# cvYouTian/Dedark-YOLO

Measured on AMD Instinct MI355X. Metric: training img/s at 640x640, higher is better.
Workload: dtype bf16

## Files before the change

dedark_yolo_amd/_C.py:

```python
import ctypes as C
import os

_HERE = os.path.dirname(os.path.abspath(__file__))
LIB_PATH = os.path.join(os.environ.get("DY_LIB_DIR") or os.path.join(_HERE, "lib"), "libdedark_yolo.so")

DY_F32, DY_BF16, DY_F16 = 0, 1, 2
ACT_NONE, ACT_SILU, ACT_LEAKY = 0, 1, 2
OPT_RULES = dict(Adam=0, Adamax=1, NAdam=2, RAdam=3, RMSProp=4)
STATS_REPLICAS = 64
BN_BWD_REPLICAS = 8

vp, i32, i64, f32, f64 = C.c_void_p, C.c_int, C.c_int64, C.c_float, C.c_double


class ConvDesc(C.Structure):
    _fields_ = [("src", vp), ("src_ld", i64), ("N", i32), ("Hs", i32), ("Ws", i32), ("Cs", i32), ("w", vp), ("dst", vp),
                ("dst_ld", i64), ("Hd", i32), ("Wd", i32), ("Cd", i32), ("KH", i32), ("KW", i32), ("stride", i32),
                ("pad", i32), ("dil", i32), ("scale", vp), ("shift", vp), ("act", i32), ("stats", vp), ("accumulate", i32),
                ("dtype", i32), ("dst_row_stride", i64), ("dst_img_stride", i64), ("KHf", i32), ("KWf", i32), ("kh0", i32),
                ("kh_step", i32), ("kw0", i32), ("kw_step", i32), ("dst_valid_channels", i32), ("dst_planar", vp),
                ("add_src", vp), ("add_src_ld", i64)]


class PackItem(C.Structure):
    _fields_ = [("w", vp), ("packed", vp), ("Cout", i32), ("Cout_pad", i32), ("Cin", i32), ("Cin_pad", i32), ("KH", i32),
                ("KW", i32), ("transposed", i32), ("dtype", i32), ("first_block", i64)]


class DetMaps(C.Structure):
    _fields_ = [("map", vp * 3), ("map_ld", i64 * 3), ("h", i32 * 3), ("w", i32 * 3), ("stride", f32 * 3), ("B", i32),
                ("nc", i32), ("n_levels", i32), ("dtype", i32)]


class DetMaps4(DetMaps):
    _fields_ = [("map3", vp), ("map_ld3", i64), ("h3", i32), ("w3", i32), ("stride3", f32)]


class AugSample(C.Structure):
    _fields_ = [("src", vp * 4), ("sh", i32 * 4), ("sw", i32 * 4), ("pitch", i64 * 4), ("rect", (i32 * 6) * 4), ("n_src", i32),
                ("canvas_h", i32), ("canvas_w", i32), ("hsv", i32), ("flipud", i32), ("fliplr", i32), ("minv", C.c_double * 6),
                ("lut", (C.c_uint8 * 256) * 3)]


class AugMixSample(C.Structure):
    _fields_ = [("a", AugSample), ("b", AugSample), ("r", C.c_double), ("r1", C.c_double), ("mix", i32)]


class SegDesc(C.Structure):
    _fields_ = [("mc", vp), ("mc_ld", i64), ("proto", vp), ("proto_ld", i64), ("B", i32), ("A", i32), ("nm", i32), ("mh", i32),
                ("mw", i32), ("target_gt_idx", vp), ("fg_mask", vp), ("target_box", vp), ("masks", vp), ("mask_dtype", i32),
                ("mask_h", i32), ("mask_w", i32), ("overlap", i32), ("gt_rows", vp), ("n_max", i32), ("img_h", f32), ("img_w", f32),
                ("pos", vp), ("npos", vp), ("dtype", i32)]


BIAS_GRAD_CHUNKS = 2048

POSE_MAX_LEVELS = 4


class PoseDesc(C.Structure):
    _fields_ = [("kpt", vp * POSE_MAX_LEVELS), ("kpt_ld", i64 * POSE_MAX_LEVELS), ("h", i32 * POSE_MAX_LEVELS), ("w", i32 * POSE_MAX_LEVELS),
                ("stride", f32 * POSE_MAX_LEVELS), ("n_levels", i32), ("B", i32), ("A", i32), ("K", i32), ("ndim", i32), ("dtype", i32),
                ("target_gt_idx", vp), ("fg_mask", vp), ("target_box", vp), ("keypoints", vp), ("n_targets", i32), ("gt_rows", vp),
                ("n_max", i32), ("img_h", f32), ("img_w", f32), ("sigma", vp), ("pos", vp), ("npos", vp)]


_SIGS = {
    "dy_version": [],
    "dy_frontend_init": [],
    "dy_conv2d_fwd": [C.POINTER(ConvDesc), vp],
    "dy_conv2d_dgrad": [C.POINTER(ConvDesc), vp],
    "dy_conv2d_wgrad": [vp, i64, i32, i32, i32, i32, vp, i64, i32, i32, i32, i32, i32, i32, i32, i32, i32, i32, vp, i64, vp,
                        i32, vp],
    "dy_conv2d_wgrad_forked": [vp, vp, i64, i32, i32, i32, i32, vp, i64, i32, i32, i32, i32, i32, i32, i32, i32, i32, i32, vp, i64,
                               vp, i32, vp],
    "dy_conv2d_bn_act_fwd": [C.POINTER(ConvDesc), i64, vp, vp, vp, vp, f32, f32, vp, i32, vp, i64, vp, i64, vp],
    "dy_bn_act_bwd": [vp, i64, vp, i64, vp, vp, i32, vp, vp, i64, vp, vp, i64, i32, i32, vp],
    "dy_conv2d_bn_act_fwd_valid": [C.POINTER(ConvDesc), i64, vp, vp, vp, vp, f32, f32, vp, i32, vp, i64, vp, i64, i32, vp],
    "dy_bn_act_bwd_valid": [vp, i64, vp, i64, vp, vp, i32, vp, vp, i64, vp, vp, i64, i32, i32, i32, vp],
    "dy_pack_weight": [vp, vp, i32, i32, i32, i32, i32, i32, i32, i32, vp],
    "dy_pack_item_blocks": [i32, i32, i32, i32],
    "dy_pack_weights_multi": [vp, i32, i64, vp],
    "dy_unpack_wgrad": [vp, vp, i32, i32, i32, i32, i32, vp],
    "dy_bn_finalize": [vp, i64, vp, vp, vp, vp, f32, f32, vp, vp, vp, vp, i32, vp],
    "dy_bn_fold_eval": [vp, vp, vp, vp, f32, vp, vp, i32, vp],
    "dy_bn_finalize_valid": [vp, i64, vp, vp, vp, vp, f32, f32, vp, vp, vp, vp, i32, i32, vp],
    "dy_bn_fold_eval_valid": [vp, vp, vp, vp, f32, vp, vp, i32, i32, vp],
    "dy_bn_act_fwd": [vp, i64, vp, vp, i32, vp, i64, vp, i64, i64, i32, i32, vp],
    "dy_bn_act_bwd_reduce": [vp, i64, vp, i64, vp, vp, vp, vp, i32, i32, vp, i64, i32, i32, vp],
    "dy_bn_act_bwd_apply": [vp, i64, vp, i64, vp, vp, vp, vp, vp, i32, i32, vp, vp, i64, vp, vp, i64, i32, i32, vp],
    "dy_bn_act_bwd_apply_valid": [vp, i64, vp, i64, vp, vp, vp, vp, vp, i32, i32, vp, vp, i64, vp, vp, i64, i32, i32, i32, vp],
    "dy_maxpool_fwd": [vp, i64, vp, i64, vp, i32, i32, i32, i32, i32, i32, i32, i32, i32, i32, vp],
    "dy_maxpool_bwd": [vp, i64, vp, vp, i64, i32, i32, i32, i32, i32, i32, i32, i32, i32, i32, i32, vp],
    "dy_upsample_nearest_fwd": [vp, i64, vp, i64, i32, i32, i32, i32, i32, i32, vp],
    "dy_upsample_nearest_bwd": [vp, i64, vp, i64, i32, i32, i32, i32, i32, i32, i32, vp],
    "dy_copy2d": [vp, i64, vp, i64, i64, i32, i32, i32, vp],
    "dy_cast": [vp, i32, vp, i32, i64, vp],
    "dy_pconv_pack": [vp, vp, i32, i32, i32, vp],
    "dy_pconv_fwd": [vp, i64, vp, i64, vp, vp, i32, i32, i32, i32, i32, i32, vp],
    "dy_pconv_dgrad": [vp, i64, vp, i64, vp, vp, i32, i32, i32, i32, i32, i32, vp, i64, i32, vp],
    "dy_pconv_wgrad": [vp, i64, vp, i64, vp, i32, i32, i32, i32, vp, i64, i32, vp],
    "dy_asff_fuse_fwd": [vp, i64, vp, i64, vp, i64, vp, i64, vp, i64, i64, i32, i32, vp],
    "dy_asff_fuse_bwd": [vp, i64, vp, i64, vp, i64, vp, i64, vp, i64, vp, i64, vp, i64, vp, i64, vp, i64, i64, i32, i32, i32,
                         i32, i32, vp],
    "dy_image_to_nhwc8": [vp, i32, i32, i32, vp, i32, i32, i32, vp],
    "dy_resize_bwd": [vp, i32, i32, i32, i32, i32, i32, vp, vp],
    "dy_filter_params_fwd": [vp, i32, vp, i32, vp],
    "dy_filter_params_bwd": [vp, i32, vp, vp, i32, vp],
    "dy_filters_pointwise_fwd": [vp, vp, vp, vp, vp, i32, i32, i32, i32, vp],
    "dy_filters_pointwise_bwd": [vp, vp, vp, vp, vp, vp, vp, i32, i32, i32, i32, i32, vp],
    "dy_usm_fwd": [vp, vp, vp, vp, vp, i32, i32, i32, i32, vp],
    "dy_usm_bwd": [vp, vp, i32, vp, vp, vp, vp, i32, i32, i32, i32, vp],
    "dy_loss_prepare_targets": [vp, vp, vp, i32, i32, i32, f32, f32, vp, vp, vp],
    "dy_loss_decode": [C.POINTER(DetMaps), vp, vp],
    "dy_tal_assign": [C.POINTER(DetMaps), vp, vp, vp, i32, vp, vp, vp, vp, vp, vp, vp, vp, vp],
    "dy_tal_assign_decoded": [vp, vp, vp, vp, vp, i32, i32, i32, i32, vp, vp, vp, vp, vp, vp, vp, vp, vp],
    "dy_chan_moments": [vp, i64, i32, i64, i32, vp, i32, vp],
    "dy_sru_fwd": [vp, i64, vp, i64, i32, i64, i32, i32, vp, vp, vp, f32, i32, vp],
    "dy_sru_bwd": [vp, i64, vp, i64, vp, i64, i32, i64, i32, i32, vp, vp, vp, f32, vp, i32, vp],
    "dy_cru_fuse_fwd": [vp, i64, vp, i64, i32, i64, i32, vp, i32, vp],
    "dy_cru_fuse_bwd": [vp, i64, vp, i64, vp, i64, i32, i64, i32, vp, vp, i32, vp],
    "dy_bbox_ciou": [vp, vp, i64, vp, vp, vp],
    "dy_bbox_iou": [vp, vp, i64, i32, i32, f32, vp, vp, vp],
    "dy_aug_resize_u8": [vp, i32, i32, i64, vp, i32, i32, i64, vp],
    "dy_aug_letterbox": [vp, i32, i32, i64, i32, i32, i32, i32, i32, i32, vp, vp],
    "dy_aug_mosaic_warp": [vp, i32, i32, i32, vp, vp],
    "dy_aug_mosaic_warp_mix": [vp, i32, i32, i32, vp, vp],
    "dy_dark_channel_prior": [vp, i32, i32, i32, vp, vp, vp],
    "dy_dfl_loss": [vp, vp, i64, vp, vp, vp],
    "dy_loss_fwd": [C.POINTER(DetMaps), vp, vp, vp, vp, vp, vp, vp],
    "dy_loss_finish": [vp, vp, f32, f32, f32, f32, i32, vp, vp, vp],
    "dy_loss_bwd": [C.POINTER(DetMaps), C.POINTER(vp), C.POINTER(i64), vp, vp, vp, vp, vp, vp, vp, f32, f32, f32, vp],
    "dy_detect_decode": [C.POINTER(DetMaps), vp, vp],
    "dy_detect_decode_rows": [C.POINTER(DetMaps), vp, i32, vp],
    "dy_detect_decode_tta": [C.POINTER(DetMaps), vp, i64, i32, i32, i32, f32, i32, f32, f32, vp],
    "dy_tta_scale_img": [vp, i32, i32, i32, i32, i32, i32, i32, i32, i32, vp, vp],
    "dy_nms_candidates": [vp, i32, i32, i32, f32, i32, vp, vp, i64, vp],
    "dy_nms_sort": [vp, vp, vp, i32, i64, vp, vp, vp],
    "dy_nms_greedy": [vp, vp, vp, i32, i32, i32, i64, C.c_double, i32, i32, f32, i32, vp, vp, vp, vp, vp, vp],
    "dy_preprocess_batch": [vp, vp, vp, f32, i32, i32, vp, i64, vp],
    "dy_sumsq": [vp, i64, vp, vp],
    "dy_sgd_step": [vp, vp, vp, vp, vp, f32, f32, f32, f32, f32, f32, f32, i32, f32, vp, f32, f32, i64, vp],
    "dy_sgd_step_scaled": [vp, vp, vp, vp, vp, f32, f32, f32, f32, f32, f32, f32, i32, f32, vp, f32, f32, vp, i64, vp],
    "dy_adamw_step_scaled": [vp, vp, vp, vp, vp, vp, f32, f32, f32, f32, f32, f32, f32, f32, f32, i32, f32, vp, f32, f32, vp, i64, vp],
    "dy_loss_scale_update": [vp, vp, f32, f32, i32, vp],
    "dy_optim_step": [i32, vp, vp, vp, vp, vp, vp, f32, f32, f32, f32, f32, f32, f64, f64, f64, f64, f32, vp, f32, f32, vp, vp, i64, vp],
    "dy_adamw_step": [vp, vp, vp, vp, vp, vp, f32, f32, f32, f32, f32, f32, f32, f32, f32, i32, f32, vp, f32, f32, i64, vp],
    "dy_ema_lerp": [vp, vp, f32, i64, vp],
    "dy_grad_accumulate": [vp, vp, i64, vp],
    "dy_stream_fork": [vp, vp],
    "dy_seg_positives": [vp, i32, i32, vp, vp, vp],
    "dy_seg_gt_rows": [vp, i32, i32, i32, vp, vp],
    "dy_seg_loss_fwd": [C.POINTER(SegDesc), f32, vp, vp, vp, vp],
    "dy_seg_loss_bwd": [C.POINTER(SegDesc), vp, f32, vp, i64, vp, i64, vp],
# ... 80 lines not shown
```

dedark_yolo_amd/csrc/bnact.hip:

```cpp
#include <stdlib.h>
#include <type_traits>
#include "dy_host.h"
#include "../../include/dedark_yolo.h"

#ifndef DY_BN_NT_FWD_MB
#define DY_BN_NT_FWD_MB 128
#endif

namespace {

constexpr int NT = 256;
template <typename T, bool NTS> __device__ inline void ld_s(const T* p, float* out) {
  if constexpr (NTS) ldvec_nt<T>(p, out); else ldvec<T>(p, out);
}
template <typename T, bool NTS> __device__ inline void st_s(T* p, const float* in) {
  if constexpr (NTS) stvec_nt<T>(p, in); else stvec<T>(p, in);
}

__global__ __launch_bounds__(256) void bn_finalize_kernel(const double* __restrict__ stats, double count, const float* __restrict__ gamma,
                                                           const float* __restrict__ beta, float* running_mean, float* running_var,
                                                           float momentum, float eps, float* scale, float* shift, float* mean_out,
                                                           float* invstd_out, int C, int Cv) {
  static_assert(DY_STATS_REPLICAS == 64, "one replica per lane");
  const int lane = threadIdx.x & 63;
  const int c = blockIdx.x * 4 + (threadIdx.x >> 6);
  if (c >= C) return;
  if (c >= Cv) {
    if (lane == 0) scale[c] = shift[c] = mean_out[c] = invstd_out[c] = 0.f;
    return;
  }
  double s1 = stats[(long)lane * 2 * C + c];
  double s2 = stats[(long)lane * 2 * C + C + c];
#pragma unroll
  for (int o = 32; o > 0; o >>= 1) {
    s1 += __shfl_xor(s1, o, 64);
    s2 += __shfl_xor(s2, o, 64);
  }
  if (lane != 0) return;
  double m = s1 / count;
  double var = s2 / count - m * m;
  if (var < 0) var = 0;
  float invstd = (float)(1.0 / sqrt(var + (double)eps));
  float g = gamma ? gamma[c] : 1.f, b = beta ? beta[c] : 0.f;
  float sc = g * invstd;
  scale[c] = sc;
  shift[c] = b - (float)m * sc;
  mean_out[c] = (float)m;
  invstd_out[c] = invstd;
  if (running_mean) {
    double unbiased = count > 1 ? var * count / (count - 1) : var;
    running_mean[c] = (1.f - momentum) * running_mean[c] + momentum * (float)m;
    running_var[c] = (1.f - momentum) * running_var[c] + momentum * (float)unbiased;
  }
}

__global__ void bn_fold_eval_kernel(const float* gamma, const float* beta, const float* rm, const float* rv, float eps,
                                    float* scale, float* shift, int C, int Cv) {
  int c = blockIdx.x * blockDim.x + threadIdx.x;
  if (c >= C) return;
  if (c >= Cv) {
    scale[c] = 0.f;
    shift[c] = 0.f;
    return;
  }
  float sc = gamma[c] / sqrtf(rv[c] + eps);
  scale[c] = sc;
  shift[c] = beta[c] - rm[c] * sc;
}

__device__ inline float fast_sigmoid(float x) { return __builtin_amdgcn_rcpf(1.0f + __expf(-x)); }
template <typename T, int ACT> __device__ inline float act_f(float u) {
  if (sizeof(T) == 4) return dy_act(ACT, u);
  if (ACT == DY_ACT_SILU) return u * fast_sigmoid(u);
  if (ACT == DY_ACT_LEAKY) return u > 0.f ? u : 0.1f * u;
  return u;
}
template <typename T, int ACT> __device__ inline float dact_f(float u) {
  if (sizeof(T) == 4) return dy_dact(ACT, u);
  if (ACT == DY_ACT_SILU) {
    const float s = fast_sigmoid(u);
    return s * (1.0f + u * (1.0f - s));
  }
  if (ACT == DY_ACT_LEAKY) return u > 0.f ? 1.0f : 0.1f;
  return 1.0f;
}
template <typename F> __device__ inline void with_act(int act, F&& f) {
  if (act == DY_ACT_SILU) f(std::integral_constant<int, DY_ACT_SILU>{});
  else if (act == DY_ACT_LEAKY) f(std::integral_constant<int, DY_ACT_LEAKY>{});
  else f(std::integral_constant<int, DY_ACT_NONE>{});
}

struct Map {
  int c, cl;
  long first, step;
  bool active;
};

template <int VE>
__device__ inline Map make_map(int C, int cgb, int rows) {
  Map m;
  const int CG = C / VE;
  const int cg_local = threadIdx.x % cgb, prow = threadIdx.x / cgb;
  const int cg = blockIdx.y * cgb + cg_local;
  m.active = prow < rows && cg < CG;
  m.c = cg * VE;
  m.cl = cg_local * VE;
  m.first = (long)blockIdx.x * rows + prow;
  m.step = (long)gridDim.x * rows;
  return m;
}


template <typename T, int U, bool NTS>
__global__ __launch_bounds__(NT) void bn_act_fwd_kernel(const T* __restrict__ z, long z_ld, const float* __restrict__ scale,
                                                         const float* __restrict__ shift, int act, const T* __restrict__ res,
                                                         long res_ld, T* __restrict__ y, long y_ld, long pixels, int C, int cgb,
                                                         int rows) {
  constexpr int VE = DT<T>::VE;
  extern __shared__ float lds[];
  const int nch = cgb * VE, c0 = blockIdx.y * nch;
  for (int i = threadIdx.x; i < nch; i += NT) {
    const int c = c0 + i;
    lds[i] = (scale && c < C) ? scale[c] : 1.f;
    lds[nch + i] = (shift && c < C) ? shift[c] : 0.f;
  }
  __syncthreads();
  const Map m = make_map<VE>(C, cgb, rows);
  if (!m.active) return;
  float sc[VE], sh[VE];
#pragma unroll
  for (int e = 0; e < VE; ++e) {
    sc[e] = lds[m.cl + e];
    sh[e] = lds[nch + m.cl + e];
  }
  with_act(act, [&](auto actc) {
    constexpr int ACT = decltype(actc)::value;
    auto loop = [&](auto resc) {
      constexpr bool RES = decltype(resc)::value;
      for (long p0 = m.first; p0 < pixels; p0 += U * m.step) {
        float v[U][VE], r[U][VE];
#pragma unroll
        for (int k = 0; k < U; ++k) {
          const long p = p0 + k * m.step;
          if (p < pixels) {
            ld_s<T, NTS>(z + p * z_ld + m.c, v[k]);
            if (RES) ld_s<T, NTS>(res + p * res_ld + m.c, r[k]);
          }
        }
#pragma unroll
        for (int k = 0; k < U; ++k) {
          const long p = p0 + k * m.step;
          if (p < pixels) {
#pragma unroll
            for (int e = 0; e < VE; ++e) {
              const float o = act_f<T, ACT>(v[k][e] * sc[e] + sh[e]);
              v[k][e] = RES ? o + r[k][e] : o;
            }
            st_s<T, NTS>(y + p * y_ld + m.c, v[k]);
          }
        }
      }
    };
    if (res) loop(std::true_type{});
    else loop(std::false_type{});
  });
}

template <typename T, int U, bool NTS>
// ... 312 lines not shown
```

dedark_yolo_amd/csrc/conv.hip:

```cpp
#include <stdlib.h>
#include "dy_host.h"
#include "conv_epilogue.h"
#include "../../include/dedark_yolo.h"
#include "conv_route.h"

namespace {

constexpr int ROWB = 144;
constexpr int NTHREADS = 256;

struct ConvP {
  const char* src;
  long src_ld;
  int N, Hs, Ws, Cs;
  const char* w;
  char* dst;
  long dst_ld;
  int Hd, Wd, Cd;
  int KH, KW, stride, pad, dil;
  const float* scale;
  const float* shift;
  int act;
  double* stats;
  int accumulate;
// ... 730 lines not shown
  const int tiles_m = dy_cdiv(p.M, BM);
  auto blocks = [&](int bn) {
    p.tiles_n = dy_cdiv(d->Cd, bn);
    p.nblk = tiles_m * p.tiles_n;
    if (p.ncls > 1) p.nblk = dy_route::number_parity_blocks(p, BM, dy_route::CLS_SEQUENTIAL);
  };
  dy_note_kernel(d->Cd <= 32 ? "conv_igemm_kernel<BN=32>" : (d->Cd <= 64 ? "conv_igemm_kernel<BN=64>" : "conv_igemm_kernel<BN=128>"));
  if (d->Cd <= 32) {
    blocks(32);
    conv_igemm_kernel<T, BM, 32, 4, 1, MODE><<<p.nblk, NTHREADS, 0, st>>>(p);
  } else if (d->Cd <= 64) {
    blocks(64);
    conv_igemm_kernel<T, BM, 64, 2, 2, MODE><<<p.nblk, NTHREADS, 0, st>>>(p);
  } else {
    blocks(128);
    conv_igemm_kernel<T, BM, 128, 2, 2, MODE><<<p.nblk, NTHREADS, 0, st>>>(p);
  }
  DY_LAUNCH_CHECK();
  return 0;
}

bool thin_eligible(const dy_conv_desc* d, int mode, bool parity_class = false) {
  static const bool off = dy_env("DY_NO_CONV_THIN") != nullptr;
  static const bool all_shapes = getenv("DY_CONV_THIN_ALL") != nullptr;
  if (off || d->dtype != DY_BF16) return false;
  if (!all_shapes && !parity_class && !(d->Cs == 16 && d->KH * d->KW > 1)) return false;
  if (!(d->Cs == 16 || d->Cs == 32 || d->Cs == 48) || d->Cd > 32 || d->Cd % 8 != 0) return false;
  if (d->KH > 3 || d->KW > 3 || d->dil != 1 || (mode == 1 && d->stride != 1)) return false;
  if ((d->src_ld * 2) % 16 != 0 || (d->dst_ld * 2) % 16 != 0 || (long)d->N * d->Hd * d->Wd < 1024) return false;
  return true;
}

int launch_thin(const dy_conv_desc* d, int mode, hipStream_t st, const dy_conv_desc* classes = nullptr, int ncls = 0) {
  ConvP p;
  dy_route::fill_parity_classes(p, classes, ncls);
  dy_route::fill_gather(p, d);
  p.tiles_n = 1;
  p.nblk = dy_cdiv(p.M, THIN_BM);
  if (p.ncls > 1) p.nblk = dy_route::number_parity_blocks(p, THIN_BM, dy_route::CLS_SEQUENTIAL);
  dy_note_kernel("conv_thin_kernel");
#define THIN(C_, M_) conv_thin_kernel<C_, M_><<<p.nblk, NTHREADS, 0, st>>>(p)
  const int c16 = d->Cs / 16;
  if (mode == 0) { if (c16 == 1) THIN(1, 0); else if (c16 == 2) THIN(2, 0); else THIN(3, 0); }
  else { if (c16 == 1) THIN(1, 1); else if (c16 == 2) THIN(2, 1); else THIN(3, 1); }
#undef THIN
  DY_LAUNCH_CHECK();
  return 0;
}

int launch_generic(const dy_conv_desc* d, int mode, hipStream_t st, const dy_conv_desc* classes = nullptr, int ncls = 0) {
  if (mode == 0)
    return d->dtype == DY_F32 ? launch_conv<float, 0>(d, st, classes, ncls)
                              : (d->dtype == DY_F16 ? launch_conv<f16_t, 0>(d, st, classes, ncls) : launch_conv<bf16_t, 0>(d, st, classes, ncls));
  return d->dtype == DY_F32 ? launch_conv<float, 1>(d, st, classes, ncls)
                            : (d->dtype == DY_F16 ? launch_conv<f16_t, 1>(d, st, classes, ncls) : launch_conv<bf16_t, 1>(d, st, classes, ncls));
}

int check_conv(const dy_conv_desc* d, const char* who) {
  DY_CHECK(d && d->src && d->w && (d->dst || d->dst_planar), "%s: null pointer", who);
  DY_CHECK(d->dtype == DY_F32 || d->dtype == DY_BF16 || d->dtype == DY_F16, "%s: bad dtype %d", who, d->dtype);
  const int ve = d->dtype == DY_F32 ? 4 : 8, es = d->dtype == DY_F32 ? 4 : 2;
  DY_CHECK(d->Cs > 0 && d->Cs % ve == 0, "%s: Cs=%d must be a positive multiple of %d", who, d->Cs, ve);
  DY_CHECK(d->src_ld >= d->Cs && (d->src_ld * es) % 16 == 0, "%s: src_ld=%ld not 16-byte aligned", who, (long)d->src_ld);
  DY_CHECK(((uintptr_t)d->src) % 16 == 0 && ((uintptr_t)d->w) % 16 == 0, "%s: src/w pointer not 16-byte aligned", who);
  DY_CHECK(d->dst_ld >= d->Cd && d->Cd > 0, "%s: dst_ld=%ld < Cd=%d", who, (long)d->dst_ld, d->Cd);
  DY_CHECK(d->N > 0 && d->Hs > 0 && d->Ws > 0 && d->Hd > 0 && d->Wd > 0, "%s: empty geometry", who);
  DY_CHECK(d->KH > 0 && d->KW > 0 && d->stride > 0 && d->dil > 0 && d->pad >= 0, "%s: bad window", who);
  DY_CHECK(d->act >= 0 && d->act <= 2, "%s: bad act", who);
  return 0;
}

enum : unsigned {
  SITE_FWD = 1,
  SITE_DGRAD_HEAD = 2,
  SITE_DGRAD = 4,
  SITE_CLASS = 8,
};

struct Route {
  bool (*eligible)(const dy_conv_desc* d, int mode);
  int (*launch)(const dy_conv_desc* d, int mode, void* stream);
  unsigned sites;
  bool fuses_add;
};

const Route kRoutes[] = {
    {dy_dense_fwd_eligible, dy_dense_fwd_launch, SITE_FWD, false},
    {dy_conv_stem_fwd_eligible, dy_conv_stem_fwd_launch, SITE_FWD, false},
    {dy_dense_dgrad_eligible, dy_dense_dgrad_launch, SITE_DGRAD_HEAD, false},
    {dy_conv_small_dgrad_eligible, dy_conv_small_dgrad_launch, SITE_DGRAD_HEAD, false},
    {dy_conv_px_eligible, dy_conv_px_launch, SITE_FWD | SITE_DGRAD, true},
    {dy_conv_v4_eligible, dy_conv_v4_launch, SITE_FWD | SITE_DGRAD | SITE_CLASS, true},
    {dy_conv_v5_eligible, dy_conv_v5_launch, SITE_FWD | SITE_DGRAD | SITE_CLASS, true},
    {dy_conv_v3_eligible, dy_conv_v3_launch, SITE_FWD | SITE_DGRAD, false},
    {dy_conv_v2_eligible, dy_conv_v2_launch, SITE_FWD | SITE_DGRAD | SITE_CLASS, false},
    {[](const dy_conv_desc* d, int mode) { return thin_eligible(d, mode); },
     [](const dy_conv_desc* d, int mode, void* stream) { return launch_thin(d, mode, (hipStream_t)stream); }, SITE_FWD | SITE_DGRAD, false},
    {[](const dy_conv_desc*, int) { return true; },
     [](const dy_conv_desc* d, int mode, void* stream) { return launch_generic(d, mode, (hipStream_t)stream); },
     SITE_FWD | SITE_DGRAD | SITE_CLASS, false},
};

const Route* pick_route(const dy_conv_desc* d, unsigned site) {
  const int mode = (site & (SITE_DGRAD_HEAD | SITE_DGRAD)) ? 1 : 0;
  for (const Route& r : kRoutes)
    if ((r.sites & site) && r.eligible(d, mode)) return &r;
  return nullptr;
}

}

extern "C" int dy_conv2d_fwd(const dy_conv_desc* d, void* stream) {
  if (int e = check_conv(d, "dy_conv2d_fwd")) return e;
  const int ho = (d->Hs + 2 * d->pad - d->dil * (d->KH - 1) - 1) / d->stride + 1;
  const int wo = (d->Ws + 2 * d->pad - d->dil * (d->KW - 1) - 1) / d->stride + 1;
  DY_CHECK(ho == d->Hd && wo == d->Wd, "dy_conv2d_fwd: dst %dx%d does not match conv output %dx%d", d->Hd, d->Wd, ho, wo);
  return pick_route(d, SITE_FWD)->launch(d, 0, stream);
}

static int dgrad_dispatch(const dy_conv_desc* d, void* stream, bool* added) {
  if (int e = check_conv(d, "dy_conv2d_dgrad")) return e;
  const int ho = (d->Hd + 2 * d->pad - d->dil * (d->KH - 1) - 1) / d->stride + 1;
  const int wo = (d->Wd + 2 * d->pad - d->dil * (d->KW - 1) - 1) / d->stride + 1;
  DY_CHECK(ho == d->Hs && wo == d->Ws, "dy_conv2d_dgrad: dz %dx%d does not match conv output %dx%d", d->Hs, d->Ws, ho, wo);
  DY_CHECK(d->stats == nullptr, "dy_conv2d_dgrad: stats unsupported");
  DY_CHECK(d->KHf == 0 && d->dst_row_stride == 0, "dy_conv2d_dgrad: tap subsets / strided destinations are forward-only");
  if (const Route* r = pick_route(d, SITE_DGRAD_HEAD)) return r->launch(d, 1, stream);
  DY_CHECK(d->dst_planar == nullptr, "dy_conv2d_dgrad: dst_planar is only supported by the direct stem kernel (bf16, 3x3 s2 p1, Cd == 8)");
  static const bool no_parity = dy_env("DY_NO_PARITY_DGRAD") != nullptr;
  if (d->stride == 2 && d->dil == 1 && !no_parity) {
    dy_conv_desc c[4];
    int nc = 0;
    bool ok = true;
    for (int ph = 0; ph < 2 && ok; ++ph)
      for (int pw = 0; pw < 2 && ok; ++pw) {
        int geo[2][4];
        for (int ax = 0; ax < 2; ++ax) {
          const int par = ax == 0 ? ph : pw, K = ax == 0 ? d->KH : d->KW, ext = ax == 0 ? d->Hd : d->Wd;
          const int first = (par + d->pad) & 1;
          const int n = first < K ? (K - 1 - first) / 2 + 1 : 0;
          const int last = first + 2 * (n - 1);
          const int omin = (par + d->pad - last) / 2;
          geo[ax][0] = n; geo[ax][1] = last; geo[ax][2] = -omin; geo[ax][3] = (ext - par + 1) / 2;
        }
        if (geo[0][3] <= 0 || geo[1][3] <= 0) continue;
        if (geo[0][0] == 0 || geo[1][0] == 0 || geo[0][2] != geo[1][2] || geo[0][2] < 0) { ok = false; break; }
        dy_conv_desc& q = c[nc++];
        q = *d;
        const long es = d->dtype == DY_F32 ? 4 : 2;
        q.dst = (char*)d->dst + ((long)ph * d->Wd + pw) * d->dst_ld * es;
        q.dst_ld = 2 * d->dst_ld;
        q.dst_row_stride = 2L * d->Wd * d->dst_ld;
        q.dst_img_stride = (long)d->Hd * d->Wd * d->dst_ld;
        q.Hd = geo[0][3]; q.Wd = geo[1][3];
        q.KHf = d->KH; q.KWf = d->KW;
        q.KH = geo[0][0]; q.KW = geo[1][0];
        q.kh0 = geo[0][1]; q.kh_step = -2; q.kw0 = geo[1][1]; q.kw_step = -2;
        q.stride = 1; q.pad = geo[0][2];
      }
    if (ok) {
      static const bool multi = !(dy_env("DY_PARITY_MULTI") && atoi(dy_env("DY_PARITY_MULTI")) == 0);
      if (multi && nc > 1) {
        dy_conv_desc r[4];
        bool all_v2 = true, none_v2 = true;
        for (int i = 0; i < nc; ++i) {
          r[i] = c[nc - 1 - i];
          const bool e2 = dy_conv_v2_eligible(&r[i], 0);
          all_v2 = all_v2 && e2;
          none_v2 = none_v2 && !e2;
        }
        const long class_tiles = dy_cdiv((long)r[0].N * r[0].Hd * r[0].Wd, 256);
        if (dy_conv_v4_classes_eligible(r, nc)) return dy_conv_v4_launch_classes(r, nc, stream);
        if (dy_conv_v5_classes_eligible(r, nc)) return dy_conv_v5_launch_classes(r, nc, stream);
        if (all_v2 && class_tiles <= 256) return dy_conv_v2_launch_classes(r, nc, stream);
        if (none_v2) {
          bool thin = true;
          for (int i = 0; i < nc; ++i) thin = thin && thin_eligible(&r[i], 0, true);
          if (thin) return launch_thin(&r[0], 0, (hipStream_t)stream, r, nc);
          if (class_tiles <= 256) return launch_generic(&r[0], 0, (hipStream_t)stream, r, nc);
        }
      }
      for (int i = nc - 1; i >= 0; --i) {
        if (int e = pick_route(&c[i], SITE_CLASS)->launch(&c[i], 0, stream)) return e;
      }
      return 0;
    }
  }
  const Route* r = pick_route(d, SITE_DGRAD);
  *added = r->fuses_add;
  return r->launch(d, 1, stream);
}

extern "C" int dy_conv2d_dgrad(const dy_conv_desc* d, void* stream) {
  bool added = false;
  if (int e = dgrad_dispatch(d, stream, &added)) return e;
  if (d->add_src && !added) {
    DY_CHECK(d->dst && d->dst_planar == nullptr, "dy_conv2d_dgrad: add_src needs an NHWC destination");
    return dy_copy2d(d->add_src, d->add_src_ld, d->dst, d->dst_ld, (int64_t)d->N * d->Hd * d->Wd, d->Cd, 1, d->dtype, stream);
  }
  return 0;
}

namespace {
template <typename T>
int launch_wgrad(WgP p, float* scratch, long scratch_elems, float* g_oihw, int Cout_real, int Cin_real, hipStream_t st) {
  constexpr int MK = 8 * DT<T>::VE;
  int bm, bn;
  bn = p.Ktot <= 32 ? 32 : (p.Ktot <= 64 ? 64 : 128);
  if (bn == 32) bm = 128;
  else if (bn == 64) bm = p.Cout <= 64 ? 64 : 128;
  else bm = p.Cout <= 32 ? 32 : (p.Cout <= 64 ? 64 : 128);
  const int tiles_c = dy_cdiv(p.Cout, bm);
  p.tiles_k = dy_cdiv(p.Ktot, bn);
  const int tiles = tiles_c * p.tiles_k;
  p.tiles = tiles;
  static const int env_blocks = dy_env("DY_WGRAD_BLOCKS") ? atoi(dy_env("DY_WGRAD_BLOCKS")) : 0;
  static const int env_steps = dy_env("DY_WGRAD_STEPS") ? atoi(dy_env("DY_WGRAD_STEPS")) : 0;
  const int min_steps = env_steps > 0 ? env_steps : 4;
  long max_splits = (p.M + (long)min_steps * MK - 1) / ((long)min_steps * MK);
  long want = ((env_blocks > 0 ? env_blocks : 2048) + tiles - 1) / tiles;
  long splits = want < max_splits ? want : max_splits;
  const long fit = scratch_elems / ((long)tiles * bm * bn);
  DY_CHECK(fit >= 1, "dy_conv2d_wgrad: scratch too small (%ld floats, need %ld)", scratch_elems, (long)tiles * bm * bn);
  if (splits > fit) splits = fit;
  if (splits < 1) splits = 1;
  if (splits > 65535) splits = 65535;
  long chunk = (p.M + splits - 1) / splits;
  chunk = (chunk + MK - 1) / MK * MK;
  splits = (p.M + chunk - 1) / chunk;
  p.chunk = chunk;
  p.part = scratch;
  dim3 grid(tiles, (unsigned)splits);
  dy_note_kernel("conv_wgrad_kernel+wgrad_reduce_kernel");
#define WG(BM_, BN_, WM_, WN_) conv_wgrad_kernel<T, BM_, BN_, WM_, WN_><<<grid, NTHREADS, 0, st>>>(p)
  if (bm == 128 && bn == 128) WG(128, 128, 2, 2);
  else if (bm == 64 && bn == 128) WG(64, 128, 1, 4);
  else if (bm == 32 && bn == 128) WG(32, 128, 1, 4);
  else if (bm == 128 && bn == 64) WG(128, 64, 4, 1);
  else if (bm == 64 && bn == 64) WG(64, 64, 2, 2);
  else WG(128, 32, 4, 1);
#undef WG
  DY_LAUNCH_CHECK();
  wgrad_reduce_kernel<<<dim3(Cout_real, dy_cdiv(p.Ktot, 32)), 256, 0, st>>>(scratch, (int)splits, tiles, p.tiles_k, bm, bn,
                                                                            Cin_real, p.Cin, p.KH, p.KW, p.Ktot, g_oihw);
  DY_LAUNCH_CHECK();
  return 0;
}

int wgrad_generic(const DyWgradArgs& a, void* stream) {
  WgP p;
  p.x = (const char*)a.x; p.x_ld = a.x_ld; p.N = a.N; p.Hi = a.Hi; p.Wi = a.Wi; p.Cin = a.Cin_pad;
  p.dz = (const char*)a.dz; p.dz_ld = a.dz_ld; p.Ho = a.Ho; p.Wo = a.Wo; p.Cout = a.Cout_pad;
  p.KH = a.KH; p.KW = a.KW; p.stride = a.stride; p.pad = a.pad; p.dil = a.dil; p.part = a.scratch;
  p.M = (long)a.N * a.Ho * a.Wo;
  p.Ktot = a.KH * a.KW * a.Cin_pad;
  p.pointwise = (a.KH == 1 && a.KW == 1 && a.stride == 1 && a.pad == 0) ? 1 : 0;
  hipStream_t st = (hipStream_t)stream;
  return a.dtype == DY_F32 ? launch_wgrad<float>(p, a.scratch, a.scratch_elems, a.g_oihw, a.Cout, a.Cin, st)
                           : (a.dtype == DY_F16 ? launch_wgrad<f16_t>(p, a.scratch, a.scratch_elems, a.g_oihw, a.Cout, a.Cin, st)
                                                : launch_wgrad<bf16_t>(p, a.scratch, a.scratch_elems, a.g_oihw, a.Cout, a.Cin, st));
}
}

extern "C" int dy_conv2d_wgrad(const void* x, int64_t x_ld, int N, int Hi, int Wi, int Cin_pad, const void* dz, int64_t dz_ld,
                               int Ho, int Wo, int Cout_pad, int KH, int KW, int stride, int pad, int dil, int Cout, int Cin,
                               float* scratch, int64_t scratch_elems, float* g_oihw, int dtype, void* stream) {
  DY_CHECK(x && dz && scratch && g_oihw, "dy_conv2d_wgrad: null pointer");
  DY_CHECK(dtype == DY_F32 || dtype == DY_BF16 || dtype == DY_F16, "dy_conv2d_wgrad: bad dtype");
  const int ve = dtype == DY_F32 ? 4 : 8, es = dtype == DY_F32 ? 4 : 2;
  DY_CHECK(Cin_pad % ve == 0 && Cout_pad % ve == 0, "dy_conv2d_wgrad: Cin=%d / Cout=%d must be multiples of %d", Cin_pad, Cout_pad, ve);
  DY_CHECK(Cout > 0 && Cout <= Cout_pad && Cin > 0 && Cin <= Cin_pad, "dy_conv2d_wgrad: bad real channel counts");
  DY_CHECK((x_ld * es) % 16 == 0 && (dz_ld * es) % 16 == 0, "dy_conv2d_wgrad: ld not 16-byte aligned");
  DY_CHECK(((uintptr_t)x) % 16 == 0 && ((uintptr_t)dz) % 16 == 0, "dy_conv2d_wgrad: pointer not 16-byte aligned");
  const int ho = (Hi + 2 * pad - dil * (KH - 1) - 1) / stride + 1, wo = (Wi + 2 * pad - dil * (KW - 1) - 1) / stride + 1;
  DY_CHECK(ho == Ho && wo == Wo, "dy_conv2d_wgrad: dz %dx%d does not match conv output %dx%d", Ho, Wo, ho, wo);
  const DyWgradArgs a = {x, x_ld, N, Hi, Wi, Cin_pad, dz, dz_ld, Ho, Wo, Cout_pad, KH, KW, stride, pad, dil, Cout, Cin,
                         scratch, scratch_elems, g_oihw, dtype};
  if (dy_dense_wgrad_eligible(a)) return dy_dense_wgrad_launch(a, stream);
  if (dy_wgrad_v3_eligible(a)) return dy_wgrad_v3_launch(a, stream);
  if (dy_wgrad_v4_eligible(a)) return dy_wgrad_v4_launch(a, stream);
  if (dy_wgrad_v2_eligible(a)) return dy_wgrad_v2_launch(a, stream);
  return wgrad_generic(a, stream);
}
// ... 67 lines not shown
```

dedark_yolo_amd/csrc/conv_epilogue.h:

```cpp
#pragma once
#include "dy_common.h"

namespace dy_epi {

template <int BM>
constexpr int pitch() { return BM * 2 + 8; }

typedef __attribute__((ext_vector_type(4))) short s16x4;
typedef __attribute__((address_space(3))) s16x4* lds_s16x4_ptr;

template <int BM, int BN>
constexpr int image_bytes() { return BN * pitch<BM>(); }

template <typename T16 = bf16_t>
__device__ inline uint32_t pack2(float a, float b) {
  if constexpr (__is_same(T16, bf16_t)) return pack_bf16x2(a, b);
  else return (uint32_t)cvt16<T16>(a) | ((uint32_t)cvt16<T16>(b) << 16);
}

template <int BM, int BN, int NW, typename T16, typename OffFn>
__device__ inline void store_image(const char* smem, int lane, int wave, long m0, int n0, long M, int Cd, int accumulate, T16* dst,
                                   OffFn off) {
  constexpr int PT = pitch<BM>();
  constexpr int UP = BM / 16, UC = BN / 32;
  const int g = lane >> 4, li = lane & 15, tq = li >> 2, tp = li & 3;
  static_assert(UP % NW == 0, "pixel tiles per wave");
#pragma unroll 2
  for (int u = 0; u < (UP / NW) * UC; ++u) {
    const int pt = wave + NW * (u / UC), ct = u % UC;
    const int cb = ct * 32 + 8 * g;
    const char* base = smem + (cb + tq) * PT + (pt * 16 + 4 * tp) * 2;
    const s16x4 lo = __builtin_amdgcn_ds_read_tr16_b64_v4i16((lds_s16x4_ptr)(base));
    const s16x4 hi = __builtin_amdgcn_ds_read_tr16_b64_v4i16((lds_s16x4_ptr)(base + 4 * PT));
    const long m = m0 + pt * 16 + li;
    const int n = n0 + cb;
    if (m < M && n < Cd) {
      u32x4 v;
      v[0] = (uint32_t)(uint16_t)lo[0] | ((uint32_t)(uint16_t)lo[1] << 16);
      v[1] = (uint32_t)(uint16_t)lo[2] | ((uint32_t)(uint16_t)lo[3] << 16);
      v[2] = (uint32_t)(uint16_t)hi[0] | ((uint32_t)(uint16_t)hi[1] << 16);
      v[3] = (uint32_t)(uint16_t)hi[2] | ((uint32_t)(uint16_t)hi[3] << 16);
      T16* o = dst + off(m) + n;
      if (n + 8 <= Cd) {
        if (accumulate) {
          float x[8], y[8];
          ldvec<T16>(o, x);
          ldvec<T16>(reinterpret_cast<const T16*>(&v), y);
#pragma unroll
          for (int e = 0; e < 8; ++e) x[e] += y[e];
          stvec<T16>(o, x);
        } else {
          *reinterpret_cast<u32x4*>(o) = v;
        }
      } else {
        const T16* e = reinterpret_cast<const T16*>(&v);
        for (int q = 0; q < 8 && n + q < Cd; ++q) {
          if (accumulate) DT<T16>::st(o + q, DT<T16>::ld(o + q) + DT<T16>::ld(e + q));
          else o[q] = e[q];
        }
      }
    }
  }
}

template <int BN>
constexpr int row_pitch() { return BN * 2 + 8; }

template <int BM, int BN>
constexpr int row_image_bytes() { return BM * row_pitch<BN>(); }

template <int BM, int BN, int NW, typename T16, typename OffFn, int RG = 64>
__device__ inline void store_rows(const char* smem, int lane, int wave, long m0, int n0, long M, int Cd, int accumulate, T16* dst, OffFn off,
                                  const T16* __restrict__ add = nullptr, long add_ld = 0) {
  constexpr int PT = row_pitch<BN>();
  constexpr int LPP = BN >= 128 ? 16 : BN / 8;
  constexpr int PPI = 64 / LPP;
  constexpr int ITERS = BM / PPI / NW;
  constexpr int HALVES = BN >= 128 ? BN / 128 : 1;
  const int pl = lane / LPP, chunk = lane % LPP;
  const bool nt = accumulate & 2;
  accumulate &= 1;
#pragma unroll 2
  for (int u = 0; u < ITERS; ++u) {
    const int px = PPI * (wave + NW * u) + pl;
    if (RG < 64 && (px & 63) >= RG) continue;
    const long m = RG < 64 ? m0 + (px >> 6) * RG + (px & 63) : m0 + px;
#pragma unroll
    for (int h = 0; h < HALVES; ++h) {
      const int c = 128 * h + 8 * chunk;
      const uint2 lo = *reinterpret_cast<const uint2*>(smem + px * PT + c * 2);
      const uint2 hi = *reinterpret_cast<const uint2*>(smem + px * PT + c * 2 + 8);
      const int n = n0 + c;
      if (m < M && n < Cd) {
        u32x4 v = {lo.x, lo.y, hi.x, hi.y};
        T16* o = dst + off(m) + n;
        if (n + 8 <= Cd) {
          if (accumulate || add) {
            float x[8], y[8];
            ldvec<T16>(reinterpret_cast<const T16*>(&v), y);
            if (accumulate) {
              ldvec<T16>(o, x);
#pragma unroll
              for (int e = 0; e < 8; ++e) y[e] += x[e];
            }
            if (add) {
              ldvec<T16>(add + m * add_ld + n, x);
#pragma unroll
              for (int e = 0; e < 8; ++e) y[e] += x[e];
            }
            if (nt) {
              u32x4 w;
              stvec<T16>(reinterpret_cast<T16*>(&w), y);
              asm volatile("global_store_dwordx4 %0, %1, off nt" ::"v"(o), "v"(w) : "memory");
            } else {
              stvec<T16>(o, y);
            }
          } else if (nt) {
            asm volatile("global_store_dwordx4 %0, %1, off nt" ::"v"(o), "v"(v) : "memory");
          } else {
            *reinterpret_cast<u32x4*>(o) = v;
          }
        } else {
          const T16* e = reinterpret_cast<const T16*>(&v);
          for (int q = 0; q < 8 && n + q < Cd; ++q) {
            float t = DT<T16>::ld(e + q);
            if (accumulate) t += DT<T16>::ld(o + q);
            if (add) t += DT<T16>::ld(add + m * add_ld + n + q);
            DT<T16>::st(o + q, t);
          }
        }
      }
    }
  }
}

template <int BM, int BN, int WM, int WN, int TM, int TN, typename T16, typename OffFn>
__device__ inline void store_tile(char* smem, f32x16 (&acc)[TM][TN], int wm, int wn, int lane, int wave, long m0, int n0, long M, int Cd,
                                  const float* scale, const float* shift, int act, int accumulate, T16* dst, OffFn off,
                                  float (&csum)[TN], float (&csq)[TN]) {
  constexpr int PT = pitch<BM>();
  static_assert(BM / WM == 32 * TM && BN / WN == 32 * TN, "wave tiling");
  const int cl = lane & 31, hh = lane >> 5;
#pragma unroll
  for (int j = 0; j < TN; ++j) { csum[j] = 0.f; csq[j] = 0.f; }
  __builtin_amdgcn_s_barrier();
#pragma unroll
  for (int j = 0; j < TN; ++j) {
    const int col = wn * (BN / WN) + j * 32 + cl;
    const int n = n0 + col;
    const bool nok = n < Cd;
    const float sc = (nok && scale) ? scale[n] : 1.f;
    const float sf = (nok && shift) ? shift[n] : 0.f;
#pragma unroll
    for (int i = 0; i < TM; ++i) {
      const int row0 = wm * (BM / WM) + i * 32 + 4 * hh;
      const long mrem = M - (m0 + row0);
#pragma unroll
      for (int rq = 0; rq < 4; ++rq) {
        float v[4];
#pragma unroll
        for (int e = 0; e < 4; ++e) {
          const float a = acc[i][j][4 * rq + e];
          if (nok && 8 * rq + e < mrem) {
            csum[j] += a;
// ... 18 lines not shown
```

dedark_yolo_amd/csrc/conv_route.h:

```cpp
#pragma once
#include "dy_common.h"
#include "../../include/dedark_yolo.h"

namespace dy_route {

__device__ inline int xcd_remap(int bid, int nblk) {
  int q = nblk >> 3, r = nblk & 7, x = bid & 7;
  int base = (x < r) ? x * (q + 1) : r * (q + 1) + (x - r) * q;
  return base + (bid >> 3);
}

template <typename P>
__device__ inline long dst_offset(const P& p, long m) {
  if (p.dst_row == 0) return m * p.dst_ld;
  const long HWd = (long)p.Hd * p.Wd;
  const long img = m / HWd;
  const int rem = (int)(m - img * HWd);
  const int oh = rem / p.Wd, ow = rem - oh * p.Wd;
  return img * p.dst_img + (long)oh * p.dst_row + (long)ow * p.dst_ld;
}

template <typename P>
inline void fill_weight_taps(P& p, const dy_conv_desc* d) {
  if (d->KHf > 0) {
    p.kh0 = d->kh0; p.khs = d->kh_step; p.kw0 = d->kw0; p.kws = d->kw_step; p.KWf = d->KWf;
    p.w_row = (long)d->KHf * d->KWf * d->Cs;
  } else {
    p.kh0 = 0; p.khs = 1; p.kw0 = 0; p.kws = 1; p.KWf = d->KW;
    p.w_row = (long)d->KH * d->KW * d->Cs;
  }
}

template <typename P>
inline void fill_dst_strides(P& p, const dy_conv_desc* d) {
  p.dst_row = d->dst_row_stride;
  p.dst_img = d->dst_img_stride ? d->dst_img_stride : (long)d->Hd * d->dst_row_stride;
}

template <typename P>
inline void fill_gather(P& p, const dy_conv_desc* d) {
  p.src = (const char*)d->src; p.src_ld = d->src_ld; p.N = d->N; p.Hs = d->Hs; p.Ws = d->Ws; p.Cs = d->Cs;
  p.w = (const char*)d->w; p.dst = (char*)d->dst; p.dst_ld = d->dst_ld; p.Hd = d->Hd; p.Wd = d->Wd; p.Cd = d->Cd;
  p.KH = d->KH; p.KW = d->KW; p.stride = d->stride; p.pad = d->pad; p.dil = d->dil;
  p.scale = d->scale; p.shift = d->shift; p.act = d->act; p.stats = d->stats; p.accumulate = d->accumulate;
  p.M = (long)d->N * d->Hd * d->Wd;
  p.Ktot = d->KH * d->KW * d->Cs;
  static const int ablate = dy_env("DY_ABLATE") ? atoi(dy_env("DY_ABLATE")) : 0;
  p.ablate = ablate;
  fill_dst_strides(p, d);
  fill_weight_taps(p, d);
}

template <typename P>
inline void fill_taps_extents(P& p, const dy_conv_desc* d, int mode) {
  p.src = (const char*)d->src; p.w = (const char*)d->w; p.dst = (char*)d->dst;
  p.src_ld = d->src_ld; p.dst_ld = d->dst_ld;
  p.src_bytes = (unsigned)((((long)d->N * d->Hs * d->Ws - 1) * d->src_ld + d->Cs) * 2);
  p.Hs = d->Hs; p.Ws = d->Ws; p.Cs = d->Cs; p.Hd = d->Hd; p.Wd = d->Wd; p.Cd = d->Cd;
  p.KH = d->KH; p.KW = d->KW;
  if (mode == 0) {
    p.stride = d->stride; p.dh0 = -d->pad; p.dhs = d->dil; p.dw0 = -d->pad; p.dws = d->dil;
  } else {
    p.stride = 1; p.dh0 = d->pad; p.dhs = -d->dil; p.dw0 = d->pad; p.dws = -d->dil;
  }
  fill_weight_taps(p, d);
  p.w_bytes = (unsigned)((long)d->Cd * p.w_row * 2);
  {
    const int dh_lo = p.dhs < 0 ? p.dh0 + p.dhs * (p.KH - 1) : p.dh0, dw_lo = p.dws < 0 ? p.dw0 + p.dws * (p.KW - 1) : p.dw0;
    const long lo = ((long)dh_lo * p.Ws + dw_lo) * p.src_ld * 2;
    p.a_min = lo < 0 ? (int)lo : 0;
  }
  p.scale = d->scale; p.shift = d->shift; p.act = d->act; p.stats = d->stats; p.accumulate = d->accumulate;
  if ((long)d->N * d->Hd * d->Wd * d->Cd * 2 > (128L << 20)) p.accumulate |= 2;
  p.M = (long)d->N * d->Hd * d->Wd;
  p.add_src = mode == 1 ? (const char*)d->add_src : nullptr; p.add_src_ld = d->add_src_ld;
  fill_dst_strides(p, d);
}

template <typename P>
inline void fill_parity_classes(P& p, const dy_conv_desc* classes, int ncls) {
  p.ncls = ncls > 1 ? ncls : 0;
  for (int c = 0; c < p.ncls; ++c) {
    const dy_conv_desc& q = classes[c];
    DyParityCls& k = p.cls[c];
    k.dst = (char*)q.dst; k.M = (long)q.N * q.Hd * q.Wd; k.Hd = q.Hd; k.Wd = q.Wd; k.KH = q.KH; k.KW = q.KW; k.pad = q.pad;
    k.kh0 = q.kh0; k.kw0 = q.kw0; k.Ktot = q.KH * q.KW * q.Cs; k.blk0 = 0; k._r = 0;
  }
}

enum ClsOrder { CLS_SEQUENTIAL, CLS_XCD_SLOTS };
template <typename P>
inline int number_parity_blocks(P& p, int bm, ClsOrder order) {
  int next = 0;
  for (int c = 0; c < p.ncls; ++c) {
    DyParityCls& k = p.cls[c];
    const int tiles = dy_cdiv(k.M, bm) * p.tiles_n;
    k.blk0 = next;
    k._r = order == CLS_XCD_SLOTS ? dy_cdiv(tiles, 8) : 0;
    next += order == CLS_XCD_SLOTS ? k._r : tiles;
  }
  return order == CLS_XCD_SLOTS ? 8 * next : next;
}

inline bool dma_extents_ok(const dy_conv_desc* d, int KH, int KW, int dil) {
  const long src_bytes = (((long)d->N * d->Hs * d->Ws - 1) * d->src_ld + d->Cs) * 2;
  const long w_row = d->KHf > 0 ? (long)d->KHf * d->KWf * d->Cs : (long)d->KH * d->KW * d->Cs;
  const long w_bytes = (long)d->Cd * w_row * 2;
  const long halo = ((long)KH * dil * d->Ws + (long)KW * dil) * d->src_ld * 2;
  return src_bytes + halo <= 0x7fffffffL && w_bytes <= 0x3fffffffL;
}

inline bool parity_classes_uniform(const dy_conv_desc* c, int ncls) {
  const dy_conv_desc* d = &c[0];
  for (int i = 0; i < ncls; ++i) {
    const dy_conv_desc& q = c[i];
    if (q.src != d->src || q.w != d->w || q.Cs != d->Cs || q.Cd != d->Cd || q.dtype != d->dtype || q.stride != 1 || q.dil != 1 || q.KHf != d->KHf ||
        q.KWf != d->KWf || q.kh_step != d->kh_step || q.kw_step != d->kw_step || q.dst_ld != d->dst_ld || q.dst_row_stride != d->dst_row_stride ||
        q.dst_img_stride != d->dst_img_stride || q.src_ld != d->src_ld || q.accumulate != d->accumulate || q.scale || q.shift || q.stats ||
        q.act != DY_ACT_NONE)
      return false;
    if ((q.dst_ld * 2) % 16 != 0 || ((uintptr_t)q.dst) % 16 != 0 || (q.src_ld * 2) % 16 != 0) return false;
  }
  return true;
}

}

bool dy_dense_fwd_eligible(const dy_conv_desc* d, int mode);
int dy_dense_fwd_launch(const dy_conv_desc* d, int mode, void* stream);
bool dy_dense_dgrad_eligible(const dy_conv_desc* d, int mode);
int dy_dense_dgrad_launch(const dy_conv_desc* d, int mode, void* stream);
bool dy_conv_stem_fwd_eligible(const dy_conv_desc* d, int mode);
int dy_conv_stem_fwd_launch(const dy_conv_desc* d, int mode, void* stream);
bool dy_conv_small_dgrad_eligible(const dy_conv_desc* d, int mode);
int dy_conv_small_dgrad_launch(const dy_conv_desc* d, int mode, void* stream);
bool dy_conv_px_eligible(const dy_conv_desc* d, int mode);
int dy_conv_px_launch(const dy_conv_desc* d, int mode, void* stream);
bool dy_conv_v4_eligible(const dy_conv_desc* d, int mode);
int dy_conv_v4_launch(const dy_conv_desc* d, int mode, void* stream);
bool dy_conv_v4_classes_eligible(const dy_conv_desc* classes, int ncls);
int dy_conv_v4_launch_classes(const dy_conv_desc* classes, int ncls, void* stream);
bool dy_conv_v5_eligible(const dy_conv_desc* d, int mode);
int dy_conv_v5_launch(const dy_conv_desc* d, int mode, void* stream);
bool dy_conv_v5_classes_eligible(const dy_conv_desc* classes, int ncls);
int dy_conv_v5_launch_classes(const dy_conv_desc* classes, int ncls, void* stream);
bool dy_conv_v3_eligible(const dy_conv_desc* d, int mode);
int dy_conv_v3_launch(const dy_conv_desc* d, int mode, void* stream);
bool dy_conv_v2_eligible(const dy_conv_desc* d, int mode);
int dy_conv_v2_launch(const dy_conv_desc* d, int mode, void* stream);
int dy_conv_v2_launch_classes(const dy_conv_desc* classes, int ncls, void* stream);
bool dy_conv_prefers_256(const dy_conv_desc* d);

struct DyWgradArgs {
  const void* x;
  long x_ld;
  int N, Hi, Wi, Cin_pad;
  const void* dz;
  long dz_ld;
  int Ho, Wo, Cout_pad, KH, KW, stride, pad, dil, Cout, Cin;
  float* scratch;
  long scratch_elems;
  float* g_oihw;
  int dtype;
};
bool dy_dense_wgrad_eligible(const DyWgradArgs& a);
int dy_dense_wgrad_launch(const DyWgradArgs& a, void* stream);
bool dy_wgrad_v3_eligible(const DyWgradArgs& a);
int dy_wgrad_v3_launch(const DyWgradArgs& a, void* stream);
bool dy_wgrad_v4_eligible(const DyWgradArgs& a);
int dy_wgrad_v4_launch(const DyWgradArgs& a, void* stream);
bool dy_wgrad_v2_eligible(const DyWgradArgs& a);
int dy_wgrad_v2_launch(const DyWgradArgs& a, void* stream);
```

dedark_yolo_amd/csrc/conv_v4.hip:

```cpp
#include <stdlib.h>
#include <type_traits>
#include "dy_common.h"
#include "conv_epilogue.h"
#include "../../include/dedark_yolo.h"
#include "conv_route.h"

namespace v4 {

constexpr int BM = 256, BN = 256, BK = 64;
constexpr int HALF = 128 * 128;
constexpr int OFF_A0 = 0, OFF_A1 = HALF, OFF_B0 = 2 * HALF, OFF_B1 = 3 * HALF, BUF = 4 * HALF;
constexpr unsigned B_ROW_OOB = 0x40000000u;

typedef __attribute__((address_space(3))) void* lds_ptr_t;
typedef __attribute__((ext_vector_type(8))) __bf16 bf16x8;

struct P {
  const char* src;
  const char* w;
  char* dst;
  unsigned src_bytes, w_bytes;
  long src_ld, dst_ld, dst_row, dst_img;
  int Hs, Ws, Cs, Hd, Wd, Cd;
  int stride;
  int KH, KW;
  int dh0, dhs, dw0, dws;
  int kh0, khs, kw0, kws, KWf;
  long w_row;
  const float* scale;
  const float* shift;
  int act;
  double* stats;
  int accumulate;
  long M;
  int a_min;
  int nk;
  int tiles_n, nblk;
  int n_full, rb_tail;
  const char* add_src;
  long add_src_ld;
  int ncls;
  DyParityCls cls[4];
};

using dy_route::xcd_remap;
using dy_route::dst_offset;

template <int ABL, typename T, int RB>
__device__ __forceinline__ void conv_tile(const P& p, char* smem, const long m0, const int n0, const int tile_m) {
  constexpr int RG = 16 * RB;
  const int tid = threadIdx.x, lane = tid & 63;
  const int wave = __builtin_amdgcn_readfirstlane(tid >> 6);
  const int wr = wave >> 2, wc = wave & 3;

  unsigned nrec_a = p.src_bytes - p.a_min, nrec_b = p.w_bytes;

  const int lrow = lane >> 3, slot = lane & 7;
  const int chunk = slot ^ ((4 * wave + (lane >> 4)) & 7);
  unsigned a_off[4], a_pad[4], b_off[4];
  {
    const DyTileWalk walk(m0, p.Hd, p.Wd);
#pragma unroll
    for (int i = 0; i < 4; ++i) {
      const int rl = 128 * (i >> 1) + 8 * (wave + 8 * (i & 1)) + lrow;
      const int r = RB == 4 ? rl : (rl >> 6) * RG + (rl & 63);
      const bool ok = (RB == 4 || (rl & 63) < RG) && m0 + r < p.M;
      int img, oh, ow;
      walk.at(r, img, oh, ow);
      const int sh0 = oh * p.stride, sw0 = ow * p.stride;
      a_off[i] = (unsigned)((((long)img * p.Hs + sh0) * p.Ws + sw0) * p.src_ld * 2 + chunk * 16);
      unsigned wb = 0, mk = 0;
      for (int tw = 0; tw < p.KW; ++tw) {
        const int sw = sw0 + p.dw0 + p.dws * tw;
        if (sw >= 0 && sw < p.Ws) wb |= 1u << tw;
      }
      for (int th = 0; th < p.KH; ++th) {
        const int sh = sh0 + p.dh0 + p.dhs * th;
        if (ok && sh >= 0 && sh < p.Hs) mk |= wb << (th * p.KW);
      }
      a_pad[i] = __builtin_amdgcn_alignbit(~mk, ~mk, 1);
      const int n = n0 + 128 * (i >> 1) + 8 * (wave + 8 * (i & 1)) + lrow;
      b_off[i] = n < p.Cd ? (unsigned)((long)n * p.w_row * 2 + chunk * 16) : B_ROW_OOB;
    }
  }
  const int ntaps = p.KH * p.KW;
  int vtap_a, vtap_b;
  {
    const int t = lane < ntaps ? lane : 0;
    const int th = t / p.KW, tw = t - th * p.KW;
    vtap_a = ((p.dh0 + p.dhs * th) * p.Ws + p.dw0 + p.dws * tw) * (int)p.src_ld * 2 - p.a_min;
    vtap_b = (int)((((long)((p.kh0 + p.khs * th) * p.KWf + p.kw0 + p.kws * tw)) * p.Cs) * 2);
  }
  int sk = 0, s_tap = 0, s_ci2 = 0;
  int a_koff = __builtin_amdgcn_readlane(vtap_a, 0);
  int b_koff = __builtin_amdgcn_readlane(vtap_b, 0);
  auto advance = [&]() {
    ++sk;
    const bool wrap = s_tap + 1 == ntaps;
    s_tap = wrap ? 0 : s_tap + 1;
    s_ci2 += wrap ? 2 * BK : 0;
    a_koff = __builtin_amdgcn_readlane(vtap_a, s_tap) + s_ci2;
    b_koff = __builtin_amdgcn_readlane(vtap_b, s_tap) + s_ci2;
    const int rot = wrap ? (33 - ntaps) & 31 : 1;
#pragma unroll
    for (int i = 0; i < 4; ++i) a_pad[i] = __builtin_amdgcn_alignbit(a_pad[i], a_pad[i], rot);
    if (sk >= p.nk) { nrec_a = 0; nrec_b = 0; a_koff = 0; b_koff = 0; }
  };
  if (p.nk < 1) { nrec_a = 0; nrec_b = 0; a_koff = 0; b_koff = 0; }
  bool in_loop = false;
  auto stage_a = [&](int buf, int h) {
    if ((ABL & 1) && in_loop) return;
    if (ABL & 16) return;
    const __amdgpu_buffer_rsrc_t rs = __builtin_amdgcn_make_buffer_rsrc((void*)(p.src + p.a_min), 0, nrec_a, 0x00020000);
#pragma unroll
    for (int j = 0; j < 2; ++j) {
      const int i = 2 * h + j;
      const unsigned v = (a_pad[i] & 0x80000000u) | a_off[i];
      __builtin_amdgcn_raw_ptr_buffer_load_lds(rs, (lds_ptr_t)(smem + buf * BUF + (h ? OFF_A1 : OFF_A0) + (wave + 8 * j) * 1024), 16,
                                               (int)v, a_koff, 0, 0);
    }
  };
  auto stage_b = [&](int buf, int h) {
    if ((ABL & 1) && in_loop) return;
    if (ABL & 32) return;
    const __amdgpu_buffer_rsrc_t rs = __builtin_amdgcn_make_buffer_rsrc((void*)p.w, 0, nrec_b, 0x00020000);
#pragma unroll
    for (int j = 0; j < 2; ++j) {
      const int i = 2 * h + j;
      __builtin_amdgcn_raw_ptr_buffer_load_lds(rs, (lds_ptr_t)(smem + buf * BUF + (h ? OFF_B1 : OFF_B0) + (wave + 8 * j) * 1024), 16,
                                               (int)b_off[i], b_koff, 0, 0);
    }
// ... 111 lines not shown
    read_a(b, 1);
    __builtin_amdgcn_sched_barrier(0);
    stage_a(b, 0);
    __builtin_amdgcn_sched_barrier(0);
    asm volatile("s_waitcnt vmcnt(10)" ::: "memory");
    __builtin_amdgcn_s_barrier();
    stamp(2, 0);
    mma(1, 1, b ^ 1, nothing);
    stamp(2, 1);
    if (!(ABL & 2048)) __builtin_amdgcn_s_barrier();
    stamp(2, 2);
    read_b(b ^ 1, 0, b ^ 1);
    __builtin_amdgcn_sched_barrier(0);
    stage_b(b, 1);
    __builtin_amdgcn_sched_barrier(0);
    asm volatile("s_waitcnt vmcnt(6)" ::: "memory");
    if (!(ABL & 2048)) __builtin_amdgcn_s_barrier();
    stamp(3, 0);
    mma(1, 0, b, nothing);
    stamp(3, 1);
    __builtin_amdgcn_s_barrier();
  };

  stamp(0, -1);
  for (int kt = 0; kt < p.nk; kt += 2) {
    kstep(std::integral_constant<int, 0>{});
    if (kt + 1 < p.nk) kstep(std::integral_constant<int, 1>{});
  }
  if ((ABL & 512) && blockIdx.x == 0 && lane == 0 && (wave == 0 || wave == 4)) {
    unsigned long long* o = reinterpret_cast<unsigned long long*>(p.stats) + (wave ? 12 : 0);
    for (int i = 0; i < 4; ++i)
      for (int j = 0; j < 3; ++j) o[3 * i + j] = t_sum[i][j];
  }
  if (!(ABL & 8) && wr == 0) __builtin_amdgcn_s_barrier();
  asm volatile("s_waitcnt vmcnt(0)" ::: "memory");
  __builtin_amdgcn_s_barrier();

  constexpr int PT = dy_epi::row_pitch<BN>();
  const int cl = lane & 15, g = lane >> 4;
  const bool plain = !p.scale && !p.shift && p.act == DY_ACT_NONE;
#pragma unroll
  for (int bh = 0; bh < 2; ++bh)
#pragma unroll
    for (int j = 0; j < 2; ++j) {
      const int c0 = 128 * bh + 32 * wc + 16 * j + 4 * g;
      if (plain) {
#pragma unroll
        for (int ah = 0; ah < 2; ++ah)
#pragma unroll
          for (int i = 0; i < RB; ++i) {
            const int px = 128 * ah + 64 * wr + 16 * i + cl;
            uint2 w2 = {dy_epi::pack2<T>(acc[ah][bh][i][j][0], acc[ah][bh][i][j][1]), dy_epi::pack2<T>(acc[ah][bh][i][j][2], acc[ah][bh][i][j][3])};
            *reinterpret_cast<uint2*>(smem + px * PT + c0 * 2) = w2;
          }
      } else {
        float sc[4], sf[4];
#pragma unroll
        for (int e = 0; e < 4; ++e) {
          const int n = n0 + c0 + e;
          const bool nok = n < p.Cd;
          sc[e] = (nok && p.scale) ? p.scale[n] : 1.f;
          sf[e] = (nok && p.shift) ? p.shift[n] : 0.f;
        }
#pragma unroll
        for (int ah = 0; ah < 2; ++ah)
#pragma unroll
          for (int i = 0; i < RB; ++i) {
            const int px = 128 * ah + 64 * wr + 16 * i + cl;
            float v[4];
#pragma unroll
            for (int e = 0; e < 4; ++e) {
              float u = acc[ah][bh][i][j][e] * sc[e] + sf[e];
              if (p.act == DY_ACT_SILU) u = u * dy_sigmoid(u);
              else if (p.act == DY_ACT_LEAKY) u = u > 0.f ? u : 0.1f * u;
              v[e] = u;
            }
            uint2 w2 = {dy_epi::pack2<T>(v[0], v[1]), dy_epi::pack2<T>(v[2], v[3])};
            *reinterpret_cast<uint2*>(smem + px * PT + c0 * 2) = w2;
          }
      }
    }
  __syncthreads();
  auto off_fn = [&](long m) { return dst_offset(p, m); };
  if (!(ABL & 64))
    dy_epi::store_rows<BM, BN, 8, T, decltype(off_fn), RG>(smem, lane, wave, m0, n0, p.M, p.Cd, p.accumulate, reinterpret_cast<T*>(p.dst), off_fn,
                                                           reinterpret_cast<const T*>(p.add_src), p.add_src_ld);
  if (p.stats && !(ABL & 512)) {
    __syncthreads();
    float* red = reinterpret_cast<float*>(smem);
#pragma unroll
    for (int bh = 0; bh < 2; ++bh)
#pragma unroll
      for (int j = 0; j < 2; ++j)
#pragma unroll
        for (int e = 0; e < 4; ++e) {
          float s1 = 0.f, s2 = 0.f;
#pragma unroll
          for (int ah = 0; ah < 2; ++ah)
#pragma unroll
            for (int i = 0; i < RB; ++i) {
              const float a = acc[ah][bh][i][j][e];
              s1 += a;
              s2 += a * a;
            }
          s1 = row16_sum(s1);
          s2 = row16_sum(s2);
          if (cl == 0) {
            const int col = 128 * bh + 32 * wc + 16 * j + 4 * g + e;
            red[(wr * BN + col) * 2] = s1;
            red[(wr * BN + col) * 2 + 1] = s2;
          }
        }
    __syncthreads();
    if (tid < BN) {
      const int n = n0 + tid;
      if (n < p.Cd) {
        const float s1 = red[tid * 2] + red[(BN + tid) * 2];
        const float s2 = red[tid * 2 + 1] + red[(BN + tid) * 2 + 1];
        double* st = p.stats + (long)(tile_m % DY_STATS_REPLICAS) * 2 * p.Cd;
        atomic_add_f64(st + n, (double)s1);
        atomic_add_f64(st + p.Cd + n, (double)s2);
      }
    }
  }
}

template <int ABL, typename T = bf16_t>
__global__ __launch_bounds__(512) void conv_kernel(const P p) {
  extern __shared__ __attribute__((aligned(16))) char smem[];
  if (p.ncls > 1) {
    const int x = blockIdx.x & 7, i = (int)blockIdx.x >> 3;
    int c = 0;
#pragma unroll
    for (int k = 1; k < 4; ++k)
      if (k < p.ncls && i >= p.cls[k].blk0) c = k;
    const DyParityCls& k = p.cls[c];
    const int tile = x * k._r + (i - k.blk0);
    const int tiles = (int)((k.M + BM - 1) / BM) * p.tiles_n;
    if (tile >= tiles) return;
    P q = p;
    q.dst = k.dst; q.M = k.M; q.Hd = k.Hd; q.Wd = k.Wd; q.KH = k.KH; q.KW = k.KW;
    q.dh0 = -k.pad; q.dw0 = -k.pad; q.kh0 = k.kh0; q.kw0 = k.kw0;
    q.nk = k.Ktot / BK;
    q.a_min = -(k.pad * p.Ws + k.pad) * (int)p.src_ld * 2;
    const int tile_m = tile / p.tiles_n, tile_n = tile - tile_m * p.tiles_n;
    conv_tile<ABL, T, 4>(q, smem, (long)tile_m * BM, tile_n * BN, tile_m);
    return;
  }
  const bool tail = (int)blockIdx.x >= p.n_full;
  const int bid = tail ? p.n_full + xcd_remap(blockIdx.x - p.n_full, p.nblk - p.n_full) : xcd_remap(blockIdx.x, p.n_full);
  const int tile_m = bid / p.tiles_n, tile_n = bid - tile_m * p.tiles_n;
  const int n0 = tile_n * BN;
  if (!tail) {
    conv_tile<ABL, T, 4>(p, smem, (long)tile_m * BM, n0, tile_m);
  } else {
    const int full_m = p.n_full / p.tiles_n;
    const long m0 = (long)full_m * BM + (long)(tile_m - full_m) * 64 * p.rb_tail;
    if (p.rb_tail == 3) conv_tile<ABL, T, 3>(p, smem, m0, n0, tile_m);
    else conv_tile<ABL, T, 2>(p, smem, m0, n0, tile_m);
  }
}

}

static int v4_variant(const dy_conv_desc* d, int mode) {
  if (d->dtype != DY_BF16 && d->dtype != DY_F16) return 0;
  if (!(d->Cs % 64 == 0 && d->KH * d->KW <= 25)) return 0;
  if (mode == 1 && d->stride != 1) return 0;
  if ((d->src_ld * 2) % 16 != 0 || (d->dst_ld * 2) % 16 != 0 || ((uintptr_t)d->dst) % 16 != 0) return 0;
  if (!dy_route::dma_extents_ok(d, d->KH, d->KW, d->dil)) return 0;
  const long tiles_m = ((long)d->N * d->Hd * d->Wd + 255) / 256;
  const long t256 = (d->Cd + 255) / 256;
  static const long min_k = dy_env("DY_V4_MINK") ? atol(dy_env("DY_V4_MINK")) : 512;
  if (d->Cd >= 192 && t256 * 256 * 4 <= (long)d->Cd * 5 && tiles_m * t256 >= 192 && (long)d->KH * d->KW * d->Cs >= min_k) return 256;
  return 0;
}

static int v4_cus() {
  static int n = 0;
  if (!n) {
    int dev = 0;
    if (hipGetDevice(&dev) != hipSuccess || hipDeviceGetAttribute(&n, hipDeviceAttributeMultiprocessorCount, dev) != hipSuccess || n <= 0) n = 256;
  }
  return n;
}

static void v4_split(long M, int tiles_n, int& n_full, int& rb_tail, int& nblk) {
  const int cus = v4_cus();
  const long tiles_m = (M + v4::BM - 1) / v4::BM;
  const long T = tiles_m * tiles_n;
  n_full = (int)T;
  rb_tail = 4;
  nblk = (int)T;
  static const char* force = dy_env("DY_V4_TAIL");
  if (force && atoi(force) == 0) return;
  if (T <= cus || T % cus == 0) return;
  const long full_blocks = (T / cus) * cus;
  const long full_m = full_blocks / tiles_n;
  if (full_m * tiles_n != full_blocks) return;
  const long rows_left = M - full_m * v4::BM;
  const double cost[5] = {0, 0, 0.75, 0.92, 1.0};
  double best = 1e9;
  int best_rb = 4;
  for (int rb = 4; rb >= 2; --rb) {
    if (force && atoi(force) != rb && rb != 4) continue;
    const long t = ((rows_left + 64 * rb - 1) / (64 * rb)) * tiles_n;
    const double c = (double)((t + cus - 1) / cus) * cost[rb];
    if (c < best - 1e-9) { best = c; best_rb = rb; }
  }
  if (force && atoi(force) >= 2 && atoi(force) <= 3) best_rb = atoi(force);
  if (best_rb == 4) return;
  n_full = (int)full_blocks;
  rb_tail = best_rb;
  nblk = (int)(full_blocks + ((rows_left + 64 * best_rb - 1) / (64 * best_rb)) * tiles_n);
}

template <int ABL, typename T = bf16_t>
static int v4_launch(const dy_conv_desc* d, int mode, void* stream, int force_variant = 0, const dy_conv_desc* classes = nullptr, int ncls = 0) {
  const int variant = force_variant ? force_variant : (ncls > 1 ? 256 : v4_variant(d, mode));
  DY_CHECK(variant != 0, "conv_v4: problem not eligible");
  DY_CHECK((long)d->N * d->Hd * d->Wd < (1L << 31), "conv_v4: too many output pixels");
  v4::P p;
  dy_route::fill_taps_extents(p, d, mode);
  p.nk = d->KH * d->KW * d->Cs / v4::BK;
  p.tiles_n = dy_cdiv(d->Cd, variant);
  v4_split(p.M, p.tiles_n, p.n_full, p.rb_tail, p.nblk);
  DY_CHECK(ncls <= 1 || (ncls <= 4 && mode == 0), "conv_v4: at most 4 forward-style classes");
  dy_route::fill_parity_classes(p, classes, ncls);
  if (p.ncls > 1) {
    for (int c = 0; c < p.ncls; ++c) DY_CHECK(p.cls[c].M < (1L << 31), "conv_v4: too many output pixels");
    p.nblk = dy_route::number_parity_blocks(p, v4::BM, dy_route::CLS_XCD_SLOTS);
    p.n_full = p.nblk; p.rb_tail = 4;
  }
  constexpr int EPI256 = dy_epi::row_image_bytes<256, 256>();
  constexpr int SH256 = 2 * v4::BUF > EPI256 ? 2 * v4::BUF : EPI256;
  static_assert(SH256 <= 160 * 1024, "LDS budget");
  static bool configured = false;
  if (!configured) {
    hipError_t e = hipFuncSetAttribute(reinterpret_cast<const void*>(&v4::conv_kernel<ABL, T>), hipFuncAttributeMaxDynamicSharedMemorySize, SH256);
    if (e != hipSuccess) {
      dy_set_error("conv_v4: hipFuncSetAttribute failed: %s", hipGetErrorString(e));
      return 3;
    }
    configured = true;
  }
  dy_note_kernel("v4::conv_kernel");
  v4::conv_kernel<ABL, T><<<p.nblk, 512, SH256, (hipStream_t)stream>>>(p);
  DY_LAUNCH_CHECK();
  return 0;
}

#ifndef DY_V4_DIAG_BUILD
bool dy_conv_v4_eligible(const dy_conv_desc* d, int mode) {
  static const bool off = dy_env("DY_NO_CONV_V4") != nullptr;
  return !off && v4_variant(d, mode) != 0;
}

int dy_conv_v4_launch(const dy_conv_desc* d, int mode, void* stream) {
  return d->dtype == DY_F16 ? v4_launch<0, f16_t>(d, mode, stream) : v4_launch<0, bf16_t>(d, mode, stream);
}

bool dy_conv_v4_classes_eligible(const dy_conv_desc* c, int ncls) {
  static const bool off = dy_env("DY_NO_CONV_V4") != nullptr || (dy_env("DY_V4_CLASSES") && atoi(dy_env("DY_V4_CLASSES")) == 0);
  if (off || ncls < 2 || ncls > 4) return false;
  const dy_conv_desc* d = &c[0];
  if (d->dtype != DY_BF16 && d->dtype != DY_F16) return false;
  if (!(d->Cs % 64 == 0 && d->KHf > 0 && d->KHf * d->KWf <= 25 && d->stride == 1)) return false;
  if (!dy_route::dma_extents_ok(d, d->KHf, d->KWf, 1) || !dy_route::parity_classes_uniform(c, ncls)) return false;
  const long t256 = (d->Cd + 255) / 256;
  if (!(d->Cd >= 192 && t256 * 256 * 4 <= (long)d->Cd * 5)) return false;
  long tiles = 0, kmax = 0;
  for (int i = 0; i < ncls; ++i) {
    const dy_conv_desc& q = c[i];
    tiles += (((long)q.N * q.Hd * q.Wd + 255) / 256) * t256;
    const long k = (long)q.KH * q.KW * q.Cs;
    kmax = k > kmax ? k : kmax;
  }
  return tiles >= 192 && kmax >= 512;
}

int dy_conv_v4_launch_classes(const dy_conv_desc* c, int ncls, void* stream) {
  return c[0].dtype == DY_F16 ? v4_launch<0, f16_t>(&c[0], 0, stream, 0, c, ncls) : v4_launch<0, bf16_t>(&c[0], 0, stream, 0, c, ncls);
}
#endif
```

dedark_yolo_amd/csrc/conv_v5.hip:

```cpp
#include <stdlib.h>
#include <type_traits>
#include "dy_common.h"
#include "conv_epilogue.h"
#include "../../include/dedark_yolo.h"
#include "conv_route.h"

namespace v5 {

constexpr int BM = 256, BK = 32;
constexpr int A_BYTES = BM * 64, NSTAGE = 3;
constexpr unsigned B_ROW_OOB = 0x40000000u;

typedef __attribute__((address_space(3))) void* lds_ptr_t;
typedef __attribute__((ext_vector_type(8))) __bf16 bf16x8;

__device__ unsigned long long g_stamps[16];

__device__ inline void stamp(int ablate, int nblk, int i) {
  if ((ablate & 32) && threadIdx.x == 0 && (blockIdx.x == 0 || (int)blockIdx.x == (nblk / 8) * 7)) {
    unsigned long long t;
    asm volatile("s_memtime %0\n\ts_waitcnt lgkmcnt(0)" : "=s"(t)::"memory");
    g_stamps[(blockIdx.x == 0 ? 0 : 8) + i] = t;
  }
}

struct P {
  const char* src;
  const char* w;
  char* dst;
  unsigned src_bytes, w_bytes;
  long src_ld, dst_ld, dst_row, dst_img;
  int Hs, Ws, Cs, Hd, Wd, Cd;
  int stride;
  int KH, KW;
  int dh0, dhs, dw0, dws;
  int kh0, khs, kw0, kws, KWf;
  long w_row;
  const float* scale;
  const float* shift;
  int act;
  double* stats;
  int accumulate;
  long M;
  int a_min;
  int nk;
  int tiles_n, nblk;
  const char* add_src;
  long add_src_ld;
  int ablate;
  int ncls;
  DyParityCls cls[4];
};

using dy_route::xcd_remap;
using dy_route::dst_offset;

template <int BN, typename T, int MB>
__device__ __forceinline__ void epilogue(const P& p, f32x4 (&acc)[MB][4], char* smem, int tid, int lane, int wave, int wm, int wn, long m0,
                                         int n0, int tile_m) {
  constexpr int WN = BN / 64, WM = 4 / WN;
  constexpr int PT = dy_epi::row_pitch<BN>();
  const int cl = lane & 15, g = lane >> 4;
  const bool plain = !p.scale && !p.shift && p.act == DY_ACT_NONE;
#pragma unroll
  for (int j = 0; j < 4; ++j) {
    const int c0 = 64 * wn + 16 * j + 4 * g;
    if (plain) {
#pragma unroll
      for (int i = 0; i < MB; ++i) {
        const int px = 16 * MB * wm + 16 * i + cl;
        uint2 w2 = {dy_epi::pack2<T>(acc[i][j][0], acc[i][j][1]), dy_epi::pack2<T>(acc[i][j][2], acc[i][j][3])};
        *reinterpret_cast<uint2*>(smem + px * PT + c0 * 2) = w2;
      }
    } else {
      float sc[4], sf[4];
#pragma unroll
      for (int e = 0; e < 4; ++e) {
        const int n = n0 + c0 + e;
        const bool nok = n < p.Cd;
        sc[e] = (nok && p.scale) ? p.scale[n] : 1.f;
        sf[e] = (nok && p.shift) ? p.shift[n] : 0.f;
      }
#pragma unroll
      for (int i = 0; i < MB; ++i) {
        const int px = 16 * MB * wm + 16 * i + cl;
        float v[4];
#pragma unroll
        for (int e = 0; e < 4; ++e) {
          float u = acc[i][j][e] * sc[e] + sf[e];
          if (p.act == DY_ACT_SILU) u = u * dy_sigmoid(u);
          else if (p.act == DY_ACT_LEAKY) u = u > 0.f ? u : 0.1f * u;
          v[e] = u;
        }
        uint2 w2 = {dy_epi::pack2<T>(v[0], v[1]), dy_epi::pack2<T>(v[2], v[3])};
        *reinterpret_cast<uint2*>(smem + px * PT + c0 * 2) = w2;
      }
    }
  }
  __syncthreads();
  stamp(DY_ABLATE_OF(p), p.nblk, 3);
  dy_epi::store_rows<BM, BN, 4>(smem, lane, wave, m0, n0, p.M, p.Cd, p.accumulate, reinterpret_cast<T*>(p.dst),
                                [&](long m) { return dst_offset(p, m); }, reinterpret_cast<const T*>(p.add_src), p.add_src_ld);
  stamp(DY_ABLATE_OF(p), p.nblk, 4);
  if (p.stats) {
    __syncthreads();
    float* red = reinterpret_cast<float*>(smem);
#pragma unroll
    for (int j = 0; j < 4; ++j)
#pragma unroll
      for (int e = 0; e < 4; ++e) {
        float s1 = 0.f, s2 = 0.f;
#pragma unroll
        for (int i = 0; i < MB; ++i) {
          const float a = acc[i][j][e];
          s1 += a;
          s2 += a * a;
        }
        s1 = row16_sum(s1);
        s2 = row16_sum(s2);
        if (cl == 0) {
          const int col = 64 * wn + 16 * j + 4 * g + e;
          red[(wm * BN + col) * 2] = s1;
          red[(wm * BN + col) * 2 + 1] = s2;
        }
      }
    __syncthreads();
    if (tid < BN) {
      const int n = n0 + tid;
      if (n < p.Cd) {
        float s1 = 0.f, s2 = 0.f;
#pragma unroll
        for (int w = 0; w < WM; ++w) {
          s1 += red[(w * BN + tid) * 2];
          s2 += red[(w * BN + tid) * 2 + 1];
        }
        double* st = p.stats + (long)(tile_m % DY_STATS_REPLICAS) * 2 * p.Cd;
        atomic_add_f64(st + n, (double)s1);
        atomic_add_f64(st + p.Cd + n, (double)s2);
      }
    }
  }
}

template <int BN, typename T = bf16_t, bool SLIM = false>
__global__ __launch_bounds__(256, SLIM ? 4 : 2) void conv_kernel(const P pk) {
  constexpr int WN = BN / 64, WM = 4 / WN, MB = BM / WM / 16, NB = 4, STAGE = A_BYTES + BN * 64, B_LD = BN / 64;
  extern __shared__ __attribute__((aligned(16))) char smem[];
  const int tid = threadIdx.x, lane = tid & 63;
  const int wave = __builtin_amdgcn_readfirstlane(tid >> 6);
  const int wm = wave / WN, wn = wave % WN;
  P p = pk;
  int bid;
  if (pk.ncls > 1) {
    const int x = blockIdx.x & 7, i = (int)blockIdx.x >> 3;
    int c = 0;
#pragma unroll
    for (int k = 1; k < 4; ++k)
      if (k < pk.ncls && i >= pk.cls[k].blk0) c = k;
    const DyParityCls& k = pk.cls[c];
    bid = x * k._r + (i - k.blk0);
    if (bid >= (int)((k.M + BM - 1) / BM) * pk.tiles_n) return;
    p.dst = k.dst; p.M = k.M; p.Hd = k.Hd; p.Wd = k.Wd; p.KH = k.KH; p.KW = k.KW;
    p.dh0 = -k.pad; p.dw0 = -k.pad; p.kh0 = k.kh0; p.kw0 = k.kw0;
    p.nk = k.Ktot / BK;
    p.a_min = -(k.pad * pk.Ws + k.pad) * (int)pk.src_ld * 2;
  } else {
    bid = xcd_remap(blockIdx.x, p.nblk);
  }
  stamp(DY_ABLATE_OF(p), p.nblk, 0);
  const int tile_m = bid / p.tiles_n, tile_n = bid - tile_m * p.tiles_n;
  const long m0 = (long)tile_m * BM;
  const int n0 = tile_n * BN;

  unsigned nrec_a = p.nk > 0 ? p.src_bytes - p.a_min : 0, nrec_b = p.nk > 0 ? p.w_bytes : 0;

  const int lrow = lane >> 2, slot = lane & 3;
  const int chunk = slot ^ ((lane & 32) ? 3 : 0);
  unsigned a_off[4], a_pad[4], b_off[B_LD];
  {
    const DyTileWalk walk(m0, p.Hd, p.Wd);
#pragma unroll
    for (int j = 0; j < 4; ++j) {
      const int r = 16 * (wave + 4 * j) + lrow;
      const bool ok = m0 + r < p.M;
      int img, oh, ow;
// ... 90 lines not shown
#pragma unroll
    for (int i = 0; i < MB; ++i) {
#pragma unroll
      for (int j = 0; j < NB; ++j)
        acc[i][j] = mfma_16x16x32<T>(bfr[j], afr[i], acc[i][j]);
      if (i == 0) mid();
    }
    __builtin_amdgcn_s_setprio(0);
  };
  auto nothing = []() {};
  auto walk = [&]() { advance(); };
  stamp(DY_ABLATE_OF(p), p.nblk, 1);
  if constexpr (BN >= 128) {
    issue(0);
    advance();
    issue(STAGE);
    advance();
    int cur = 0, fill = 2 * STAGE;
    for (int kt = 0; kt < p.nk; ++kt) {
      if ((DY_ABLATE_OF(p) & 64) || kt + 1 >= p.nk) asm volatile("s_waitcnt vmcnt(0)" ::: "memory");
      else
      asm volatile("s_waitcnt vmcnt(%0)" ::"n"(4 + B_LD) : "memory");
      __builtin_amdgcn_s_barrier();
      __builtin_amdgcn_sched_barrier(0);
      if (sk < p.nk) issue(fill);
      __builtin_amdgcn_sched_barrier(0);
      compute(cur, walk);
      __builtin_amdgcn_sched_barrier(0);
      cur = cur == 2 * STAGE ? 0 : cur + STAGE;
      fill = fill == 2 * STAGE ? 0 : fill + STAGE;
    }
  } else if constexpr (SLIM) {
    issue(0);
    advance();
    int cur = 0;
    for (int kt = 0; kt < p.nk; ++kt) {
      asm volatile("s_waitcnt vmcnt(0)" ::: "memory");
      __builtin_amdgcn_s_barrier();
      __builtin_amdgcn_sched_barrier(0);
      if (sk < p.nk) issue(cur ? 0 : STAGE);
      __builtin_amdgcn_sched_barrier(0);
      compute(cur, walk);
      __builtin_amdgcn_sched_barrier(0);
      cur = cur ? 0 : STAGE;
    }
  } else {
    issue(0);
    advance();
    issue(STAGE);
    advance();
    int cur = 0;
    for (int kt = 0; kt < p.nk; kt += 2) {
      asm volatile("s_waitcnt vmcnt(0)" ::: "memory");
      __builtin_amdgcn_s_barrier();
      __builtin_amdgcn_sched_barrier(0);
      const int nxt = cur ^ (2 * STAGE);
      if (sk < p.nk) {
        issue(nxt);
        advance();
        issue(nxt + STAGE);
      } else {
        advance();
      }
      __builtin_amdgcn_sched_barrier(0);
      compute(cur, walk);
      compute(cur + STAGE, nothing);
      __builtin_amdgcn_sched_barrier(0);
      cur = nxt;
    }
  }
  asm volatile("s_waitcnt vmcnt(0)" ::: "memory");
  __builtin_amdgcn_s_barrier();
  stamp(DY_ABLATE_OF(p), p.nblk, 2);

  epilogue<BN, T, MB>(p, acc, smem, tid, lane, wave, wm, wn, m0, n0, tile_m);
#ifdef DY_DIAG
  asm volatile("s_waitcnt vmcnt(0)" ::: "memory");
#endif
  stamp(DY_ABLATE_OF(p), p.nblk, 5);
}

constexpr int BAND_BYTES = 17 * 1024;

template <int BN, typename T = bf16_t, int NBAND_ = (BN == 64 ? 3 : 2)>
__global__ __launch_bounds__(256, (BN == 64 && NBAND_ == 2) ? 3 : 2) void band_kernel(const P p) {
  constexpr int WN = BN / 64, WM = 4 / WN, MB = BM / WM / 16, B_LD = BN / 64, B_BYTES = BN * 64;
  constexpr int NBAND = NBAND_, DB = 3 * (NBAND - 1), NBBUF = DB + 1;
  constexpr int OFF_B = NBAND * BAND_BYTES, OFF_ZERO = OFF_B + NBBUF * B_BYTES;
  constexpr int N0 = (DB - 1) * B_LD + 5 * (NBAND - 2), N1 = (DB - 1) * B_LD + 5 * (NBAND - 1);
  extern __shared__ __attribute__((aligned(16))) char smem[];
  const int tid = threadIdx.x, lane = tid & 63;
  const int wave = __builtin_amdgcn_readfirstlane(tid >> 6);
  const int wm = wave / WN, wn = wave % WN;
  const int bid = xcd_remap(blockIdx.x, p.nblk);
  stamp(DY_ABLATE_OF(p), p.nblk, 0);
  const int tile_m = bid / p.tiles_n, tile_n = bid - tile_m * p.tiles_n;
  const long m0 = (long)tile_m * BM;
  const int n0 = tile_n * BN;

  if (tid < 16) reinterpret_cast<unsigned*>(smem + OFF_ZERO)[tid] = 0u;

  const int lrow = lane >> 2, slot = lane & 3;
  const int chunk = slot ^ ((lane & 16) ? 2 : 0);
  const bool tail_lane = (lane >> 4) == wave;
  unsigned a_off[5], b_off[B_LD];
#pragma unroll
  for (int j = 0; j < 5; ++j) {
    const int brow = j < 4 ? 16 * (wave + 4 * j) + lrow : 256 + lrow;
    a_off[j] = (unsigned)((m0 - 1 + brow) * p.src_ld * 2 + chunk * 16);
  }
#pragma unroll
  for (int j = 0; j < B_LD; ++j) {
    const int n = n0 + 16 * (wave + 4 * j) + lrow;
    b_off[j] = n < p.Cd ? (unsigned)((long)n * p.w_row * 2 + chunk * 16) : B_ROW_OOB;
  }
  const int ng = p.nk / 3;
  int ga_n = 0, ga_th = 0, ga_ci = 0;
  auto issue_band = [&](int base) {
    const bool live = ga_n < ng && !(DY_ABLATE_OF(p) & 2);
    const unsigned koff = (unsigned)((p.dh0 + p.dhs * ga_th) * p.Ws * (int)p.src_ld * 2 + ga_ci * 2);
    const __amdgpu_buffer_rsrc_t rs = __builtin_amdgcn_make_buffer_rsrc((void*)p.src, 0, live ? p.src_bytes : 0u, 0x00020000);
#pragma unroll
    for (int j = 0; j < 4; ++j)
      __builtin_amdgcn_raw_ptr_buffer_load_lds(rs, (lds_ptr_t)(smem + base + (wave + 4 * j) * 1024), 16, (int)(a_off[j] + koff), 0, 0, 0);
    if (tail_lane)
      __builtin_amdgcn_raw_ptr_buffer_load_lds(rs, (lds_ptr_t)(smem + base + 16 * 1024), 16, (int)(a_off[4] + koff), 0, 0, 0);
    ++ga_n;
    if (++ga_th == 3) { ga_th = 0; ga_ci += BK; }
  };
  int kb = 0, kb_tp = 0, kb_ci = 0;
  auto issue_b = [&](int base) {
    const bool live = kb < p.nk && !(DY_ABLATE_OF(p) & 4);
    const int koff = live ? (int)(((long)kb_tp * p.Cs + kb_ci) * 2) : 0;
    const __amdgpu_buffer_rsrc_t rs = __builtin_amdgcn_make_buffer_rsrc((void*)p.w, 0, live ? p.w_bytes : 0u, 0x00020000);
#pragma unroll
    for (int j = 0; j < B_LD; ++j)
      __builtin_amdgcn_raw_ptr_buffer_load_lds(rs, (lds_ptr_t)(smem + base + (wave + 4 * j) * 1024), 16, (int)b_off[j], koff, 0, 0);
    ++kb;
    if (++kb_tp == 9) { kb_tp = 0; kb_ci += BK; }
  };

  const int fr = lane & 15, fq = lane >> 4;
  const int r0 = 16 * MB * wm + fr;
  int a_rd[3];
#pragma unroll
  for (int tw = 0; tw < 3; ++tw) {
    const int brow = r0 + 1 + p.dw0 + p.dws * tw;
    a_rd[tw] = brow * 64 + ((fq ^ ((brow & 4) ? 2 : 0)) * 16);
  }
  const int b_rd = (64 * wn + fr) * 64 + ((fq ^ ((fr & 4) ? 2 : 0)) * 16);
  unsigned tm[3] = {0u, 0u, 0u};
  {
    const long m = m0 + r0;
    int img, h, w;
    DyTileWalk(m0, p.Hd, p.Wd).at(r0, img, h, w);
#pragma unroll
    for (int i = 0; i < MB; ++i) {
      const bool ok = m + 16 * i < p.M;
#pragma unroll
      for (int th = 0; th < 3; ++th) {
        const bool hv = (unsigned)(h + p.dh0 + p.dhs * th) < (unsigned)p.Hs;
#pragma unroll
        for (int tw = 0; tw < 3; ++tw) {
          const bool wv = (unsigned)(w + p.dw0 + p.dws * tw) < (unsigned)p.Ws;
          if (ok && hv && wv) tm[th] |= 1u << (8 * tw + i);
        }
      }
// ... 17 lines not shown
    if (DY_ABLATE_OF(p) & 16) {
#pragma unroll
      for (int j = 0; j < 4; ++j) bfr[j] = u32x4{0x3f803f80u + (unsigned)b_base, 0x3f803f80u, 0x3f803f80u, 0x3f803f80u};
#pragma unroll
      for (int i = 0; i < MB; ++i) afr[i] = u32x4{0x3f803f80u, 0x3f803f80u + (bits & 1u), 0x3f803f80u, 0x3f803f80u};
    } else {
#pragma unroll
      for (int j = 0; j < 4; ++j) bfr[j] = *reinterpret_cast<const u32x4*>(smem + b_base + b_rd + 1024 * j);
#pragma unroll
      for (int i = 0; i < MB; ++i) {
        const int sel = ((bits >> i) & 1u) ? av : OFF_ZERO - 1024 * i;
        afr[i] = *reinterpret_cast<const u32x4*>(smem + sel + 1024 * i);
      }
    }
    if (DY_ABLATE_OF(p) & 8) {
#pragma unroll
      for (int i = 0; i < MB; ++i) acc[i][0][0] += __builtin_bit_cast(float, afr[i][0] ^ bfr[i & 3][1]);
      return;
    }
    __builtin_amdgcn_s_setprio(1);
#pragma unroll
    for (int i = 0; i < MB; ++i)
#pragma unroll
      for (int j = 0; j < 4; ++j) acc[i][j] = mfma_16x16x32<T>(bfr[j], afr[i], acc[i][j]);
    __builtin_amdgcn_s_setprio(0);
  };
  stamp(DY_ABLATE_OF(p), p.nblk, 1);

  int band_fill = 0, b_fill = 0;
#pragma unroll
  for (int s = 0; s < DB; ++s) {
    if (s % 3 == 0) {
      issue_band(band_fill);
      band_fill += BAND_BYTES;
    }
    issue_b(OFF_B + b_fill);
    b_fill += B_BYTES;
  }
  int band_cur = 0, b_cur = 0, th = 0;
  auto next_b = [&]() {
    b_cur = b_cur == DB * B_BYTES ? 0 : b_cur + B_BYTES;
    b_fill = b_fill == DB * B_BYTES ? 0 : b_fill + B_BYTES;
  };
  auto group = [&](auto tailc) {
    constexpr bool tail = decltype(tailc)::value;
    const unsigned tmc = th == 0 ? tm[0] : (th == 1 ? tm[1] : tm[2]);
    asm volatile("s_waitcnt vmcnt(%0)" ::"n"(N0) : "memory");
    __builtin_amdgcn_s_barrier();
    __builtin_amdgcn_sched_barrier(0);
    if constexpr (!tail) {
      issue_band(band_fill);
      issue_b(OFF_B + b_fill);
    }
    __builtin_amdgcn_sched_barrier(0);
    compute(band_cur, OFF_B + b_cur, tmc, a_rd[0]);
    __builtin_amdgcn_sched_barrier(0);
    next_b();
    asm volatile("s_waitcnt vmcnt(%0)" ::"n"(tail ? B_LD : N1) : "memory");
    __builtin_amdgcn_s_barrier();
    __builtin_amdgcn_sched_barrier(0);
    if constexpr (!tail) issue_b(OFF_B + b_fill);
    __builtin_amdgcn_sched_barrier(0);
    compute(band_cur, OFF_B + b_cur, tmc >> 8, a_rd[1]);
    __builtin_amdgcn_sched_barrier(0);
    next_b();
    asm volatile("s_waitcnt vmcnt(%0)" ::"n"(tail ? 0 : N1) : "memory");
    __builtin_amdgcn_s_barrier();
    __builtin_amdgcn_sched_barrier(0);
    if constexpr (!tail) issue_b(OFF_B + b_fill);
    __builtin_amdgcn_sched_barrier(0);
    compute(band_cur, OFF_B + b_cur, tmc >> 16, a_rd[2]);
    __builtin_amdgcn_sched_barrier(0);
    next_b();
    band_cur = band_cur == (NBAND - 1) * BAND_BYTES ? 0 : band_cur + BAND_BYTES;
    band_fill = band_fill == (NBAND - 1) * BAND_BYTES ? 0 : band_fill + BAND_BYTES;
    th = th == 2 ? 0 : th + 1;
  };
  constexpr bool peel = NBAND == 2;
  for (int g = 0; g < ng - (peel ? 1 : 0); ++g) group(std::false_type{});
  if (peel) group(std::true_type{});
  asm volatile("s_waitcnt vmcnt(0)" ::: "memory");
  __builtin_amdgcn_s_barrier();
  stamp(DY_ABLATE_OF(p), p.nblk, 2);
  epilogue<BN, T, MB>(p, acc, smem, tid, lane, wave, wm, wn, m0, n0, tile_m);
#ifdef DY_DIAG
  asm volatile("s_waitcnt vmcnt(0)" ::: "memory");
#endif
  stamp(DY_ABLATE_OF(p), p.nblk, 5);
}


}

extern "C" int dy_debug_conv5_stamps(unsigned long long* out) {
  return hipMemcpyFromSymbol(out, HIP_SYMBOL(v5::g_stamps), sizeof(unsigned long long) * 16) == hipSuccess ? 0 : 1;
}

bool dy_conv_v5_eligible(const dy_conv_desc* d, int mode) {
  static const bool off = dy_env("DY_NO_CONV_V5") != nullptr;
  if (off || (d->dtype != DY_BF16 && d->dtype != DY_F16)) return false;
  if (!(d->Cs % 32 == 0 && d->KH * d->KW <= 25)) return false;
  if (mode == 1 && d->stride != 1) return false;
  if ((d->src_ld * 2) % 16 != 0 || (d->dst_ld * 2) % 16 != 0 || ((uintptr_t)d->dst) % 16 != 0) return false;
  const long M = (long)d->N * d->Hd * d->Wd;
  if (!(dy_route::dma_extents_ok(d, d->KH, d->KW, d->dil) && M < (1L << 31))) return false;
  const long tiles_m = (M + 255) / 256;
  const long tn = (d->Cd + 127) / 128;
  if (d->Cd >= 96 && tn * 128 * 4 <= (long)d->Cd * 5 && tiles_m * tn >= 256) return true;
  return d->Cd >= 48 && d->Cd <= 64 && tiles_m >= 256;
}

static int v5_launch(const dy_conv_desc* d, int mode, void* stream, const dy_conv_desc* classes, int ncls);

int dy_conv_v5_launch(const dy_conv_desc* d, int mode, void* stream) { return v5_launch(d, mode, stream, nullptr, 0); }

bool dy_conv_v5_classes_eligible(const dy_conv_desc* c, int ncls) {
  static const bool off = dy_env("DY_NO_CONV_V5") != nullptr || (dy_env("DY_V5_CLASSES") && atoi(dy_env("DY_V5_CLASSES")) == 0);
  if (off || ncls < 2 || ncls > 4) return false;
  const dy_conv_desc* d = &c[0];
  if (d->dtype != DY_BF16 && d->dtype != DY_F16) return false;
  if (!(d->Cs % 32 == 0 && d->KHf > 0 && d->KHf * d->KWf <= 25 && d->stride == 1)) return false;
  if (!dy_route::dma_extents_ok(d, d->KHf, d->KWf, 1) || !dy_route::parity_classes_uniform(c, ncls)) return false;
  const long tn = (d->Cd + 127) / 128;
  const bool wide = d->Cd >= 96 && tn * 128 * 4 <= (long)d->Cd * 5, narrow = d->Cd >= 48 && d->Cd <= 64;
  if (!wide && !narrow) return false;
  long tiles = 0;
  for (int i = 0; i < ncls; ++i) {
    const dy_conv_desc& q = c[i];
    if ((long)q.N * q.Hd * q.Wd >= (1L << 31)) return false;
    tiles += (((long)q.N * q.Hd * q.Wd + 255) / 256) * (wide ? tn : 1);
  }
  return tiles >= 256;
}

int dy_conv_v5_launch_classes(const dy_conv_desc* c, int ncls, void* stream) { return v5_launch(&c[0], 0, stream, c, ncls); }

static int v5_launch(const dy_conv_desc* d, int mode, void* stream, const dy_conv_desc* classes, int ncls) {
  v5::P p;
  dy_route::fill_taps_extents(p, d, mode);
  p.nk = d->KH * d->KW * d->Cs / v5::BK;
  static const int ablate = dy_env("DY_ABLATE") ? atoi(dy_env("DY_ABLATE")) : 0;
  p.ablate = ablate;
  const int bn = d->Cd <= 64 ? 64 : 128;
  p.tiles_n = dy_cdiv(d->Cd, bn);
  p.nblk = dy_cdiv(p.M, v5::BM) * p.tiles_n;
  DY_CHECK(ncls <= 1 || (ncls <= 4 && mode == 0), "conv_v5: at most 4 forward-style classes");
  dy_route::fill_parity_classes(p, classes, ncls);
  if (p.ncls > 1) p.nblk = dy_route::number_parity_blocks(p, v5::BM, dy_route::CLS_XCD_SLOTS);
  constexpr int RING128 = v5::NSTAGE * (v5::A_BYTES + 128 * 64), EPI128 = dy_epi::row_image_bytes<v5::BM, 128>();
  constexpr int RING64 = 4 * (v5::A_BYTES + 64 * 64), EPI64 = dy_epi::row_image_bytes<v5::BM, 64>();
  constexpr int SH128 = RING128 > EPI128 ? RING128 : EPI128, SH64 = RING64 > EPI64 ? RING64 : EPI64;
  constexpr int RING64S = 2 * (v5::A_BYTES + 64 * 64), SH64S = RING64S > EPI64 ? RING64S : EPI64;
  static_assert(4 * SH64S <= 160 * 1024, "four blocks per CU");
  static const bool slim64 = !(dy_env("DY_CONV64_SLIM") && atoi(dy_env("DY_CONV64_SLIM")) == 0);
  constexpr int BAND128 = 2 * v5::BAND_BYTES + 4 * 128 * 64 + 64, BAND64 = 3 * v5::BAND_BYTES + 7 * 64 * 64 + 64;
  constexpr int SB128 = BAND128 > EPI128 ? BAND128 : EPI128, SB64 = BAND64 > EPI64 ? BAND64 : EPI64;
  constexpr int BAND64S = 2 * v5::BAND_BYTES + 4 * 64 * 64 + 64, SB64S = BAND64S > EPI64 ? BAND64S : EPI64;
  static_assert(3 * SB64S <= 160 * 1024, "three blocks per CU");
  static const int band64_nband = dy_env("DY_BAND64_NBAND") ? atoi(dy_env("DY_BAND64_NBAND")) : 2;
  static_assert(2 * SH128 <= 160 * 1024 && 2 * SH64 <= 160 * 1024 && 2 * SB128 <= 160 * 1024 && 2 * SB64 <= 160 * 1024, "two blocks per CU");
  static const bool no_band = dy_env("DY_NO_CONV_BAND") != nullptr;
  const bool band = ncls <= 1 && !no_band && d->KH == 3 && d->KW == 3 && d->stride == 1 && d->pad == 1 && d->dil == 1 && d->KHf <= 0 && d->Hs == d->Hd &&
                    d->Ws == d->Wd && d->Ws >= 16;
  static bool configured = false;
  if (!configured) {
    hipError_t e = hipFuncSetAttribute(reinterpret_cast<const void*>(&v5::conv_kernel<128, bf16_t>), hipFuncAttributeMaxDynamicSharedMemorySize, SH128);
    if (e == hipSuccess) e = hipFuncSetAttribute(reinterpret_cast<const void*>(&v5::conv_kernel<64, bf16_t>), hipFuncAttributeMaxDynamicSharedMemorySize, SH64);
    if (e == hipSuccess) e = hipFuncSetAttribute(reinterpret_cast<const void*>(&v5::conv_kernel<128, f16_t>), hipFuncAttributeMaxDynamicSharedMemorySize, SH128);
    if (e == hipSuccess) e = hipFuncSetAttribute(reinterpret_cast<const void*>(&v5::conv_kernel<64, f16_t>), hipFuncAttributeMaxDynamicSharedMemorySize, SH64);
    if (e == hipSuccess) e = hipFuncSetAttribute(reinterpret_cast<const void*>(&v5::conv_kernel<64, bf16_t, true>), hipFuncAttributeMaxDynamicSharedMemorySize, SH64S);
    if (e == hipSuccess) e = hipFuncSetAttribute(reinterpret_cast<const void*>(&v5::conv_kernel<64, f16_t, true>), hipFuncAttributeMaxDynamicSharedMemorySize, SH64S);
    if (e == hipSuccess) e = hipFuncSetAttribute(reinterpret_cast<const void*>(&v5::band_kernel<128, bf16_t>), hipFuncAttributeMaxDynamicSharedMemorySize, SB128);
    if (e == hipSuccess) e = hipFuncSetAttribute(reinterpret_cast<const void*>(&v5::band_kernel<64, bf16_t>), hipFuncAttributeMaxDynamicSharedMemorySize, SB64);
    if (e == hipSuccess) e = hipFuncSetAttribute(reinterpret_cast<const void*>(&v5::band_kernel<128, f16_t>), hipFuncAttributeMaxDynamicSharedMemorySize, SB128);
    if (e == hipSuccess) e = hipFuncSetAttribute(reinterpret_cast<const void*>(&v5::band_kernel<64, f16_t>), hipFuncAttributeMaxDynamicSharedMemorySize, SB64);
    if (e == hipSuccess) e = hipFuncSetAttribute(reinterpret_cast<const void*>(&v5::band_kernel<64, bf16_t, 2>), hipFuncAttributeMaxDynamicSharedMemorySize, SB64S);
    if (e == hipSuccess) e = hipFuncSetAttribute(reinterpret_cast<const void*>(&v5::band_kernel<64, f16_t, 2>), hipFuncAttributeMaxDynamicSharedMemorySize, SB64S);
    if (e != hipSuccess) {
      dy_set_error("conv_v5: hipFuncSetAttribute failed: %s", hipGetErrorString(e));
      return 3;
    }
    configured = true;
  }
  const bool f16 = d->dtype == DY_F16;
  if (band && bn == 128) {
    dy_note_kernel("v5::band_kernel<128>");
    if (f16) v5::band_kernel<128, f16_t><<<p.nblk, 256, SB128, (hipStream_t)stream>>>(p);
    else v5::band_kernel<128, bf16_t><<<p.nblk, 256, SB128, (hipStream_t)stream>>>(p);
  } else if (band && band64_nband == 2) {
    dy_note_kernel("v5::band_kernel<64>");
    if (f16) v5::band_kernel<64, f16_t, 2><<<p.nblk, 256, SB64S, (hipStream_t)stream>>>(p);
    else v5::band_kernel<64, bf16_t, 2><<<p.nblk, 256, SB64S, (hipStream_t)stream>>>(p);
  } else if (band) {
    dy_note_kernel("v5::band_kernel<64>");
    if (f16) v5::band_kernel<64, f16_t><<<p.nblk, 256, SB64, (hipStream_t)stream>>>(p);
    else v5::band_kernel<64, bf16_t><<<p.nblk, 256, SB64, (hipStream_t)stream>>>(p);
  } else if (bn == 128) {
    dy_note_kernel("v5::conv_kernel<128>");
    if (f16) v5::conv_kernel<128, f16_t><<<p.nblk, 256, SH128, (hipStream_t)stream>>>(p);
    else v5::conv_kernel<128, bf16_t><<<p.nblk, 256, SH128, (hipStream_t)stream>>>(p);
  } else if (slim64) {
    dy_note_kernel("v5::conv_kernel<64>");
    if (f16) v5::conv_kernel<64, f16_t, true><<<p.nblk, 256, SH64S, (hipStream_t)stream>>>(p);
    else v5::conv_kernel<64, bf16_t, true><<<p.nblk, 256, SH64S, (hipStream_t)stream>>>(p);
  } else {
    dy_note_kernel("v5::conv_kernel<64>");
    if (f16) v5::conv_kernel<64, f16_t><<<p.nblk, 256, SH64, (hipStream_t)stream>>>(p);
    else v5::conv_kernel<64, bf16_t><<<p.nblk, 256, SH64, (hipStream_t)stream>>>(p);
  }
  DY_LAUNCH_CHECK();
  return 0;
}
```

dedark_yolo_amd/csrc/dy_common.h:

```cpp
#pragma once
#include <hip/hip_runtime.h>
#include <stdint.h>
#include <stdio.h>

#define DY_F32 0
#define DY_BF16 1
#define DY_F16 2

#include <stdlib.h>
#ifdef DY_DIAG
#define DY_ABLATE_OF(p) ((p).ablate)
static inline const char* dy_env(const char* name) { return getenv(name); }
#else
#define DY_ABLATE_OF(p) 0
static inline const char* dy_env(const char*) { return nullptr; }
#endif

#define DY_ACT_NONE 0
#define DY_ACT_SILU 1
#define DY_ACT_LEAKY 2

typedef uint16_t bf16_t;
typedef _Float16 f16_t;
typedef __attribute__((ext_vector_type(4))) float f32x4;
// ... 97 lines not shown
    out[2 * i] = __builtin_bit_cast(float, v[i] << 16);
    out[2 * i + 1] = __builtin_bit_cast(float, v[i] & 0xffff0000u);
  }
}
template <> __device__ inline void ldvec<f16_t>(const f16_t* p, float* out) {
  const f16x8 v = *reinterpret_cast<const f16x8*>(p);
#pragma unroll
  for (int i = 0; i < 8; ++i) out[i] = (float)v[i];
}
template <typename T> __device__ inline void stvec(T* p, const float* in);
template <> __device__ inline void stvec<float>(float* p, const float* in) {
  f32x4 v = {in[0], in[1], in[2], in[3]};
  *reinterpret_cast<f32x4*>(p) = v;
}
__device__ inline uint32_t pack_bf16x2(float lo, float hi) {
  typedef __attribute__((ext_vector_type(2))) float f32x2_;
  typedef __attribute__((ext_vector_type(2))) __bf16 bf16x2_;
  return __builtin_bit_cast(uint32_t, __builtin_convertvector(f32x2_{lo, hi}, bf16x2_));
}
template <> __device__ inline void stvec<bf16_t>(bf16_t* p, const float* in) {
  u32x4 v;
#pragma unroll
  for (int i = 0; i < 4; ++i) v[i] = pack_bf16x2(in[2 * i], in[2 * i + 1]);
  *reinterpret_cast<u32x4*>(p) = v;
}

template <> __device__ inline void stvec<f16_t>(f16_t* p, const float* in) {
  f16x8 v;
#pragma unroll
  for (int i = 0; i < 8; ++i) v[i] = (f16_t)in[i];
  *reinterpret_cast<f16x8*>(p) = v;
}

template <typename T> __device__ inline void ldvec_nt(const T* p, float* out) {
  if constexpr (sizeof(T) == 4) {
    const f32x4 v = __builtin_nontemporal_load(reinterpret_cast<const f32x4*>(p));
    out[0] = v[0]; out[1] = v[1]; out[2] = v[2]; out[3] = v[3];
  } else {
    const u32x4 v = __builtin_nontemporal_load(reinterpret_cast<const u32x4*>(p));
    if constexpr (__is_same(T, f16_t)) {
      const f16x8 h = __builtin_bit_cast(f16x8, v);
#pragma unroll
      for (int i = 0; i < 8; ++i) out[i] = (float)h[i];
    } else {
#pragma unroll
      for (int i = 0; i < 4; ++i) {
        out[2 * i] = __builtin_bit_cast(float, v[i] << 16);
        out[2 * i + 1] = __builtin_bit_cast(float, v[i] & 0xffff0000u);
      }
    }
  }
}
template <typename T> __device__ inline void stvec_nt(T* p, const float* in) {
  if constexpr (sizeof(T) == 4) {
    const f32x4 v = {in[0], in[1], in[2], in[3]};
    __builtin_nontemporal_store(v, reinterpret_cast<f32x4*>(p));
  } else {
    u32x4 v;
    if constexpr (__is_same(T, f16_t)) {
      f16x8 h;
#pragma unroll
      for (int i = 0; i < 8; ++i) h[i] = (f16_t)in[i];
      v = __builtin_bit_cast(u32x4, h);
    } else {
#pragma unroll
      for (int i = 0; i < 4; ++i) v[i] = pack_bf16x2(in[2 * i], in[2 * i + 1]);
    }
    __builtin_nontemporal_store(v, reinterpret_cast<u32x4*>(p));
  }
}

__host__ __device__ inline float dy_sigmoid(float x) { return 1.0f / (1.0f + expf(-x)); }
__host__ __device__ inline float dy_act(int act, float u) {
  if (act == DY_ACT_SILU) return u * dy_sigmoid(u);
  if (act == DY_ACT_LEAKY) return u > 0.f ? u : 0.1f * u;
  return u;
}
__host__ __device__ inline float dy_dact(int act, float u) {
  if (act == DY_ACT_SILU) {
    float s = dy_sigmoid(u);
    return s * (1.0f + u * (1.0f - s));
  }
  if (act == DY_ACT_LEAKY) return u > 0.f ? 1.0f : 0.1f;
  return 1.0f;
}

struct DyTileWalk {
  int img0, oh0, ow0, Hd, Wd;
  float inv_h, inv_w;
  __device__ inline DyTileWalk(long m0, int Hd_, int Wd_) : Hd(Hd_), Wd(Wd_) {
    const unsigned HWd = (unsigned)(Hd_ * Wd_);
    const unsigned mm = (unsigned)m0;
    const unsigned img = mm / HWd;
    const unsigned rem = mm - img * HWd;
    const unsigned oh = rem / (unsigned)Wd_;
    img0 = (int)img;
    oh0 = (int)oh;
    ow0 = (int)(rem - oh * (unsigned)Wd_);
    inv_h = 1.0f / (float)Hd_;
    inv_w = 1.0f / (float)Wd_;
  }
  __device__ inline void at(int r, int& img, int& oh, int& ow) const {
    const int x = ow0 + r;
    const int q = (int)(((float)x + 0.5f) * inv_w);
    ow = x - q * Wd;
    const int y = oh0 + q;
    const int q2 = (int)(((float)y + 0.5f) * inv_h);
    oh = y - q2 * Hd;
    img = img0 + q2;
  }
};

__device__ inline float row16_sum(float v) {
  v += __builtin_bit_cast(float, __builtin_amdgcn_update_dpp(0, __builtin_bit_cast(int, v), 0xB1, 0xf, 0xf, true));
  v += __builtin_bit_cast(float, __builtin_amdgcn_update_dpp(0, __builtin_bit_cast(int, v), 0x4E, 0xf, 0xf, true));
  v += __builtin_bit_cast(float, __builtin_amdgcn_update_dpp(0, __builtin_bit_cast(int, v), 0x141, 0xf, 0xf, true));
  v += __builtin_bit_cast(float, __builtin_amdgcn_update_dpp(0, __builtin_bit_cast(int, v), 0x140, 0xf, 0xf, true));
  return v;
}
__device__ inline float wave_sum(float v) {
#pragma unroll
  for (int o = 32; o > 0; o >>= 1) v += __shfl_xor(v, o, 64);
  return v;
}
__device__ inline float wave_max(float v) {
#pragma unroll
  for (int o = 32; o > 0; o >>= 1) v = fmaxf(v, __shfl_xor(v, o, 64));
  return v;
}
__device__ inline float block_sum(float v, float* sm) {
  v = wave_sum(v);
  int lane = threadIdx.x & 63, w = threadIdx.x >> 6, nw = (blockDim.x + 63) >> 6;
  __syncthreads();
  if (lane == 0) sm[w] = v;
  __syncthreads();
  float r = 0.f;
  for (int i = 0; i < nw; ++i) r += sm[i];
  return r;
}

__device__ inline void atomic_add_f64(double* p, double v) { unsafeAtomicAdd(p, v); }
__device__ inline void atomic_add_f32(float* p, float v) { unsafeAtomicAdd(p, v); }
```

dedark_yolo_amd/nn/modules.py:

```python
import ctypes as C
import math
import os

import torch
import torch.nn as nn

from .. import ops
from .._C import ACT_LEAKY, ACT_NONE, ACT_SILU, call
from ..ops import as_nhwc, conv_backward, conv_forward, copy2d, empty_nhwc, ld_of, ptr, stream

__all__ = ("Conv", "Concat", "Bottleneck", "C2", "C2f", "PConv", "PconvBottleneck", "PconvBottleneck_n", "FasterC2f", "FasterC2f_N", "SPPF", "Upsample", "AsffTribeLevel", "AsffDoubLevel", "MFRU", "SCConv", "RFBblock", "DFL", "Detect",
           "AsffDetect", "Proto", "Segment", "Pose", "Classify",
           "lowlight_recovery", "ExtractParameters2", "autopad")


def autopad(k, p=None, d=1):
    if d > 1:
        k = d * (k - 1) + 1 if isinstance(k, int) else [d * (x - 1) + 1 for x in k]
    if p is None:
        p = k // 2 if isinstance(k, int) else [x // 2 for x in k]
    return p


class Tape:
# ... 22 lines not shown
        ctx.out_meta = [(outs.shape, outs.dtype, outs.device)]
        return outs

    @staticmethod
    def backward(ctx, *gouts):
        gouts = [g if g is not None else torch.zeros(m[0], dtype=m[1], device=m[2]) for g, m in zip(gouts, ctx.out_meta)]
        module, tape = ctx.module, ctx.tape
        if getattr(module, "_planar_grad_ok", False) and all(g.is_contiguous() and g.dtype == m[1] for g, m in zip(gouts, ctx.out_meta)):
            pass
        else:
            gouts = [as_nhwc(g, m[1]) for g, m in zip(gouts, ctx.out_meta)]
        gins = module._bwd(tape, *gouts, needs=list(ctx.needs_input_grad[3:3 + ctx.n_in]))
        if not isinstance(gins, (list, tuple)):
            gins = (gins,)
        assert not tape.stack, f"{type(module).__name__}: unbalanced tape"
        cb = module.__dict__.get("_dy_after_backward")
        if cb is not None:
            cb()
        pg = [tape.pgrads.get(p) for p in module._plist]
        return (None, None, None, *gins, *pg)


class DyModule(nn.Module):
    in_dtype = None

    def _params(self):
        pl = self.__dict__.get("_plist")
        if pl is None:
            pl = [p for p in self.parameters() if p.requires_grad]
            self.__dict__["_plist"] = pl
        return pl

    def forward(self, x, *extra, out=None):
        xs = list(x) if isinstance(x, (list, tuple)) else [x]
        xs = [self._adapt(t) for t in xs]
        pl = self._params()
        if torch.is_grad_enabled() and (any(t.requires_grad for t in xs) or any(p.requires_grad for p in pl)):
            return self._wrap(_ModuleFn.apply(self, len(xs), out, *xs, *pl))
        with torch.no_grad():
            return self._wrap(self._fwd(None, *xs) if out is None else self._fwd(None, *xs, out=out))

    def _adapt(self, t):
        return as_nhwc(t, self.in_dtype)

    def _wrap(self, out):
        return list(out) if isinstance(out, tuple) else out

    def train(self, mode=True):
        self.__dict__.pop("_plist", None)
        return super().train(mode)


def _act_code(act):
    if act is True or isinstance(act, nn.SiLU):
        return ACT_SILU
    if isinstance(act, nn.LeakyReLU):
        if abs(act.negative_slope - 0.1) > 1e-12:
            raise NotImplementedError("only LeakyReLU(0.1) is implemented in the HIP epilogue")
        return ACT_LEAKY
    if act is False or act is None or isinstance(act, nn.Identity):
        return ACT_NONE
    raise NotImplementedError(f"activation {act!r} has no HIP epilogue")


class Conv(DyModule):
    default_act = nn.SiLU()

    def __init__(self, c1, c2, k=1, s=1, p=None, g=1, d=1, act=True):
        super().__init__()
        if g != 1:
            raise NotImplementedError("grouped convolution is outside the Dedark-YOLO hot path")
        self.conv = nn.Conv2d(c1, c2, k, s, autopad(k, p, d), groups=g, dilation=d, bias=False)
        self.bn = nn.BatchNorm2d(c2)
        self.act = self.default_act if act is True else act if isinstance(act, nn.Module) else nn.Identity()
        self._act = _act_code(self.act)

    def _fwd(self, tape, x, out=None, residual=None):
        c = self.conv
        return conv_forward(tape, x, c.weight, None, self.bn, self._act, c.stride[0], c.padding[0], c.dilation[0],
                            self.training, out=out, residual=residual)

    _takes_into = True

    def _bwd(self, tape, dy, needs=(True,), dx_out=None, accumulate=False, add_src=None, into=None):
        if into is not None and into[0] is not None:
            conv_backward(tape, dy, need_dx=True, dx_out=into[0], accumulate=True)
            return None
        return conv_backward(tape, dy, need_dx=needs[0], dx_out=dx_out, accumulate=accumulate, add_src=add_src)


class AddConv(nn.Module):

    def __init__(self, in_ch, out_ch, ksize, stride):
        super().__init__()
        self.conv = nn.Conv2d(in_ch, out_ch, ksize, stride, (ksize - 1) // 2, bias=False)
        self.batch_norm = nn.BatchNorm2d(out_ch)
        self.leaky = nn.LeakyReLU(0.1)

    def _fwd(self, tape, x, training, out=None):
        c = self.conv
        return conv_forward(tape, x, c.weight, None, self.batch_norm, ACT_LEAKY, c.stride[0], c.padding[0], 1, training, out=out)


def plain_conv_fwd(tape, m, x, act=ACT_NONE, out=None):
    return conv_forward(tape, x, m.weight, m.bias, None, act, m.stride[0], m.padding[0], m.dilation[0], False, out=out)


class Concat(DyModule):

    def __init__(self, dimension=1):
        super().__init__()
        if dimension != 1:
            raise NotImplementedError("Concat: only channel concat is on the hot path")
        self.d = dimension

    @staticmethod
    def _in_place(xs, tot):
        t0 = xs[0]
        if ld_of(t0) != tot or t0.dim() != 4:
            return None
        es, base, o = t0.element_size(), t0.data_ptr(), 0
        for t in xs:
            if (t.dtype != t0.dtype or tuple(t.shape[2:]) != tuple(t0.shape[2:]) or t.shape[0] != t0.shape[0] or ld_of(t) != tot
                    or t.stride() != t0.stride() or t.data_ptr() != base + o * es
                    or t.untyped_storage().data_ptr() != t0.untyped_storage().data_ptr()):
                return None
            o += t.shape[1]
        return torch.as_strided(t0, (t0.shape[0], tot, t0.shape[2], t0.shape[3]), t0.stride(), t0.storage_offset())

    def _fwd(self, tape, *xs):
        B, _, H, W = xs[0].shape
        tot = sum(t.shape[1] for t in xs)
        whole = self._in_place(xs, tot)
        if whole is not None:
            if tape is not None:
                tape.push([t.shape[1] for t in xs])
            return whole
        out = empty_nhwc(B, tot, H, W, xs[0].dtype, xs[0].device)
        o = 0
        for t in xs:
            copy2d(t, out[:, o:o + t.shape[1]])
            o += t.shape[1]
        if tape is not None:
            tape.push([t.shape[1] for t in xs])
        return out

    def _bwd(self, tape, dy, needs=None):
        sizes = tape.pop()
        outs, o = [], 0
        for c in sizes:
            outs.append(dy[:, o:o + c])
            o += c
        return outs


class Upsample(DyModule):

    def __init__(self, size=None, scale_factor=None, mode="nearest"):
        super().__init__()
        if size is not None or mode != "nearest" or int(scale_factor) != scale_factor:
            raise NotImplementedError("Upsample: integer nearest-neighbour scale only")
        self.scale_factor = int(scale_factor)
        self.mode = mode

    def _fwd(self, tape, x, out=None):
        return ops.upsample_fwd(x, self.scale_factor, out=out)

    _takes_into = True

    def _bwd(self, tape, dy, needs=None, into=None):
        if into is not None and into[0] is not None:
            ops.upsample_bwd(dy, self.scale_factor, dx_out=into[0], accumulate=True)
            return None
        return ops.upsample_bwd(dy, self.scale_factor)


class Bottleneck(DyModule):

    def __init__(self, c1, c2, shortcut=True, g=1, k=(3, 3), e=0.5):
        super().__init__()
        c_ = int(c2 * e)
        self.cv1 = Conv(c1, c_, k[0], 1)
        self.cv2 = Conv(c_, c2, k[1], 1, g=g)
        self.add = shortcut and c1 == c2

    def _fwd(self, tape, x, out=None):
        t = self.cv1._fwd(tape, x)
        return self.cv2._fwd(tape, t, out=out, residual=x if self.add else None)

    def _bwd(self, tape, dy, needs=(True,), dx_out=None, accumulate=False):
        dt = self.cv2._bwd(tape, dy)
        return self.cv1._bwd(tape, dt, dx_out=dx_out, accumulate=accumulate, add_src=dy if self.add else None)


class C2(DyModule):

    def __init__(self, c1, c2, n=1, shortcut=True, g=1, e=0.5):
        super().__init__()
        self.c = int(c2 * e)
        self.cv1 = Conv(c1, 2 * self.c, 1, 1)
        self.cv2 = Conv(2 * self.c, c2, 1)
        self.m = nn.Sequential(*(Bottleneck(self.c, self.c, shortcut, g, k=((3, 3), (3, 3)), e=1.0) for _ in range(n)))

    def _fwd(self, tape, x, out=None):
        c, n = self.c, len(self.m)
        B, _, H, W = x.shape
        Y = empty_nhwc(B, 2 * c, H, W, x.dtype, x.device)
        Z = empty_nhwc(B, 2 * c, H, W, x.dtype, x.device)
        self.cv1._fwd(tape, x, out=Y)
        t = Y[:, :c]
        for i, m in enumerate(self.m):
            t = m._fwd(tape, t, out=Z[:, :c] if i == n - 1 else None)
        copy2d(Y[:, c:], Z[:, c:])
        return self.cv2._fwd(tape, Z, out=out)

    def _bwd(self, tape, dy, needs=(True,)):
        c, n = self.c, len(self.m)
        dZ = self.cv2._bwd(tape, dy)
        B, _, H, W = dZ.shape
        dY = empty_nhwc(B, 2 * c, H, W, dZ.dtype, dZ.device)
        copy2d(dZ[:, c:], dY[:, c:])
        g = dZ[:, :c]
        for i in reversed(range(n)):
            g = self.m[i]._bwd(tape, g, dx_out=dY[:, :c] if i == 0 else None)
        return self.cv1._bwd(tape, dY, needs=needs)


class C2f(DyModule):

    def __init__(self, c1, c2, n=1, shortcut=False, g=1, e=0.5):
        super().__init__()
        self.c = int(c2 * e)
        self.cv1 = Conv(c1, 2 * self.c, 1, 1)
        self.cv2 = Conv((2 + n) * self.c, c2, 1)
        self.m = nn.ModuleList(Bottleneck(self.c, self.c, shortcut, g, k=((3, 3), (3, 3)), e=1.0) for _ in range(n))

    def _fwd(self, tape, x, out=None):
        c, n = self.c, len(self.m)
        B, _, H, W = x.shape
        Y = empty_nhwc(B, (2 + n) * c, H, W, x.dtype, x.device)
        self.cv1._fwd(tape, x, out=Y[:, :2 * c])
        for i, m in enumerate(self.m):
            m._fwd(tape, Y[:, (1 + i) * c:(2 + i) * c], out=Y[:, (2 + i) * c:(3 + i) * c])
        return self.cv2._fwd(tape, Y, out=out)

    def _bwd(self, tape, dy, needs=(True,)):
        c, n = self.c, len(self.m)
        dY = self.cv2._bwd(tape, dy)
        for i in reversed(range(n)):
            self.m[i]._bwd(tape, dY[:, (2 + i) * c:(3 + i) * c], dx_out=dY[:, (1 + i) * c:(2 + i) * c], accumulate=True)
        return self.cv1._bwd(tape, dY[:, :2 * c], needs=needs)


class PConv(DyModule):

    def __init__(self, dim, n_div, forward="split_cat"):
        super().__init__()
        if forward != "split_cat":
            raise NotImplementedError("PConv: only the split_cat forward is implemented")
        self.dim_conv3 = dim // n_div
        self.dim_untouched = dim - self.dim_conv3
        self.patial_conv3 = nn.Conv2d(self.dim_conv3, self.dim_conv3, 3, 1, 1, bias=False)

    def _fwd(self, tape, x, out=None):
        return ops.pconv_forward(tape, x, self.patial_conv3.weight, out=out)

    def _bwd(self, tape, dy, needs=(True,), dx_out=None, accumulate=False, add_src=None):
        return ops.pconv_backward(tape, dy, dx_out=dx_out, accumulate=accumulate, add_src=add_src)


class _PconvBottleneckBase(DyModule):

    def _last(self):
        raise NotImplementedError

    def _fwd(self, tape, x, out=None):
        fb = self.fasterblock
        t = fb[1]._fwd(tape, fb[0]._fwd(tape, x))
        y = conv_forward(tape, t, self._last().weight, None, None, ACT_NONE, 1, 0, 1, False, out=out)
        if self.add:
            copy2d(x, y, accumulate=True)
            ops.emu_round(y)
        return y

    def _bwd(self, tape, dy, needs=(True,), dx_out=None, accumulate=False):
        fb = self.fasterblock
        du = conv_backward(tape, dy)
        dt = fb[1]._bwd(tape, du)
        return fb[0]._bwd(tape, dt, dx_out=dx_out, accumulate=accumulate, add_src=dy if self.add else None)


class PconvBottleneck(_PconvBottleneckBase):

    def __init__(self, c1, c2, shortcut=True, g=1, k=(3, 3), e=0.5):
        super().__init__()
        if g != 1:
            raise NotImplementedError("grouped convolution is outside the Dedark-YOLO hot path")
        c_ = int(c2 * e)
        self.fasterblock = nn.Sequential(PConv(dim=c1, n_div=4), Conv(c1=c1, c2=c_, k=3, s=1, p=1))
        self.conv = nn.Conv2d(c_, c2, 1, 1, autopad(1, None, 1), groups=g, bias=False)
        self.add = shortcut and c1 == c2

    def _last(self):
        return self.conv


class PconvBottleneck_n(_PconvBottleneckBase):

    def __init__(self, c1, c2, shortcut=True, g=1, k=(3, 3), e=0.5):
        super().__init__()
        if g != 1:
            raise NotImplementedError("grouped convolution is outside the Dedark-YOLO hot path")
        c_ = int(c2 * e)
        self.fasterblock = nn.Sequential(PConv(dim=c1, n_div=4), Conv(c1=c1, c2=2 * c_, k=1, s=1),
                                         nn.Conv2d(2 * c_, c2, 1, 1, autopad(1, None, 1), groups=g, bias=False))
        self.add = shortcut and c1 == c2

    def _last(self):
        return self.fasterblock[2]


class FasterC2f_N(C2f):

    def __init__(self, c1, c2, n=1, shortcut=False, g=1, e=0.5):
        super().__init__(c1, c2, n, shortcut, g, e)
        self.m = nn.ModuleList(PconvBottleneck_n(self.c, self.c, shortcut, g=g, k=((3, 3), (3, 3)), e=1.0) for _ in range(n))


class FasterC2f(C2f):

    def __init__(self, c1, c2, n=1, shortcut=False, g=1, e=0.5):
        super().__init__(c1, c2, n, shortcut, g, e)
        self.m = nn.ModuleList(PconvBottleneck(self.c, self.c, shortcut, g, k=((3, 3), (3, 3)), e=1.0) for _ in range(n))
# ... 914 lines not shown
```

dedark_yolo_amd/ops.py:

```python
import ctypes as C
import math
import os

import torch

from . import _C
from ._C import ACT_LEAKY, ACT_NONE, ACT_SILU, ConvDesc, DetMaps, DetMaps4, call

_compute_dtype = torch.float32
_pack_generation = 0
_weights_epoch = 0


def set_compute_dtype(dt):
    global _compute_dtype
    if dt not in (torch.float32, torch.bfloat16, torch.float16):
        raise ValueError(f"dedark_yolo_amd: unsupported compute dtype {dt}")
    _compute_dtype = dt


def get_compute_dtype():
    return _compute_dtype


# ... 203 lines not shown
class PackPlan:

    def __init__(self):
        self.sig = None
        self.table = None
        self.n_blocks = 0
        self.entries = []

    def _collect(self, model):
        ent = []
        _extra_pack_views[:] = [r for r in _extra_pack_views if r() is not None]
        for w in list(model.parameters()) + [r() for r in _extra_pack_views]:
            cache = w.__dict__.get("_dy_pack")
            if not cache or w.dtype != torch.float32 or not w.is_contiguous() or w.dim() != 4:
                continue
            for key, (tag, out) in cache.items():
                ent.append((w, key, out))
        return ent

    def repack(self, model):
        key = (id(model), _pack_generation)
        if key != getattr(self, "_ent_key", None):
            self._ent = self._collect(model)
            self._ent_sig = tuple((w.data_ptr(), out.data_ptr(), k) for w, k, out in self._ent)
            self._ent_key = key
        ent = self._ent
        if not ent:
            return
        sig = self._ent_sig
        if any(w.data_ptr() != sg[0] for (w, _, _), sg in zip(ent[:4], sig[:4])):
            self._ent_key = None
            return self.repack(model)
        if sig != self.sig:
            items = (_C.PackItem * len(ent))()
            blk = 0
            lib = _C.lib()
            for it, (w, (cout_pad, cin_pad, transposed, dtype), out) in zip(items, ent):
                Co, Ci, KH, KW = w.shape
                it.w, it.packed = w.data_ptr(), out.data_ptr()
                it.Cout, it.Cout_pad, it.Cin, it.Cin_pad, it.KH, it.KW = Co, cout_pad, Ci, cin_pad, KH, KW
                it.transposed, it.dtype, it.first_block = int(transposed), dt_id(dtype), blk
                blk += lib.dy_pack_item_blocks(cout_pad, cin_pad, KH, KW)
            raw = torch.frombuffer(bytearray(bytes(items)), dtype=torch.uint8)
            self.table = raw.to(ent[0][0].device)
            self.n_blocks, self.sig = blk, sig
        call("dy_pack_weights_multi", ptr(self.table), len(ent), self.n_blocks, stream())
        for w, key, out in ent:
            w.__dict__["_dy_pack"][key] = ((_weights_epoch, w._version), out)


def _padded_vec(v, n):
    if v is None:
        return None
    v = v.detach()
    if v.numel() == n and v.dtype == torch.float32:
        return v
    out = torch.zeros(n, dtype=torch.float32, device=v.device)
    out[:v.numel()] = v
    return out


def bn_fold(bn, cout_pad):
    tag = (_weights_epoch, bn.weight._version, bn.bias._version, bn.running_mean._version, bn.running_var._version,
           bn.weight.data_ptr(), bn.running_mean.data_ptr(), cout_pad)
    hit = bn.__dict__.get("_dy_fold")
    if hit is not None and hit[0] == tag:
        return hit[1]
    aff = hit[1] if (hit is not None and hit[1].shape[1] == cout_pad and hit[1].device == bn.weight.device) else \
        torch.empty((2, cout_pad), dtype=torch.float32, device=bn.weight.device)
    call("dy_bn_fold_eval_valid", ptr(bn.weight), ptr(bn.bias), ptr(bn.running_mean), ptr(bn.running_var), float(bn.eps),
         ptr(aff[0]), ptr(aff[1]), cout_pad, bn.weight.numel(), stream())
    bn.__dict__["_dy_fold"] = (tag, aff)
    return aff


def bn_fold_is_current(bn):
    hit = bn.__dict__.get("_dy_fold")
    return hit is not None and hit[0][:7] == (_weights_epoch, bn.weight._version, bn.bias._version, bn.running_mean._version,
                                               bn.running_var._version, bn.weight.data_ptr(), bn.running_mean.data_ptr())


class ConvCtx:
    __slots__ = ("x", "z", "aff", "weight", "bias", "bn", "act", "k", "stride", "pad", "dil", "cout", "cout_pad", "cin_pad",
                 "has_bn", "y", "owner", "shared")


def _conv_desc(src, w, dst, N, Hs, Ws, Cs, Hd, Wd, Cd, KH, KW, stride, pad, dil, scale, shift, act, stats, accumulate, dtype):
    if dst is not None:
        dptr, dld = dst.data_ptr(), ld_of(dst)
    else:
        dptr, dld = None, Cd
    return ConvDesc(src.data_ptr(), ld_of(src), N, Hs, Ws, Cs, w.data_ptr(), dptr, dld, Hd, Wd, Cd, KH, KW, stride, pad, dil,
                    None if scale is None else scale.data_ptr(), None if shift is None else shift.data_ptr(), act,
                    None if stats is None else stats.data_ptr(), 1 if accumulate else 0, dt_id(dtype))


_bn_pending = {}


def flush_bn_counters():
    for bn, n in _bn_pending.items():
        bn.num_batches_tracked += n
    _bn_pending.clear()


def conv_forward(tape, x, weight, bias=None, bn=None, act=ACT_NONE, stride=1, pad=0, dil=1, training=False, out=None,
                 residual=None, owner=None, shared=False):
    dtype = x.dtype
    B, Cin, H, W = x.shape
    Cout, Cw, KH, KW = weight.shape
    if Cw != Cin:
        raise RuntimeError(f"conv: weight expects {Cw} input channels, got {Cin}")
    ve = vec_elems(dtype)
    cin_pad = padded_channels(x)
    cout_pad = round_up(Cout, ve)
    Ho = (H + 2 * pad - dil * (KH - 1) - 1) // stride + 1
    Wo = (W + 2 * pad - dil * (KW - 1) - 1) // stride + 1
    wp = _pack(weight, cout_pad, cin_pad, False, dtype)
    dev = x.device
    has_bn = bn is not None
    batch_stats = has_bn and training
    ctx = None
    if tape is not None:
        ctx = ConvCtx()
        ctx.x, ctx.weight, ctx.bias, ctx.bn, ctx.act = x, weight, bias, bn, act
        ctx.owner = owner if owner is not None else weight
        ctx.shared = shared
        ctx.k, ctx.stride, ctx.pad, ctx.dil = (KH, KW), stride, pad, dil
        ctx.cout, ctx.cout_pad, ctx.cin_pad, ctx.has_bn = Cout, cout_pad, cin_pad, has_bn
    if batch_stats:
        z = empty_nhwc(B, cout_pad, Ho, Wo, dtype, dev)
        stats = arena.alloc(2 * cout_pad * _C.STATS_REPLICAS, dev)
        d = _conv_desc(x, wp, z, B, H, W, cin_pad, Ho, Wo, cout_pad, KH, KW, stride, pad, dil, None, None, ACT_NONE, stats,
                       False, dtype)
        aff = torch.empty((4, cout_pad), dtype=torch.float32, device=dev)
        pa, sa = aff.data_ptr(), 4 * cout_pad
        pixels = B * Ho * Wo
        _bn_pending[bn] = _bn_pending.get(bn, 0) + 1
        bn.__dict__.pop("_dy_fold", None)
        y = out if out is not None else empty_nhwc(B, cout_pad, Ho, Wo, dtype, dev)
        st = stream()
        rp, rld = (residual.data_ptr(), ld_of(residual)) if residual is not None else (None, 0)
        bp = bn._parameters
        if _C._prof is None and _emulate_storage is None:
            call("dy_conv2d_bn_act_fwd_valid", C.byref(d), pixels, ptr(bp["weight"]), ptr(bp["bias"]), ptr(bn.running_mean), ptr(bn.running_var),
                 float(bn.momentum), float(bn.eps), pa, act, rp, rld, y.data_ptr(), ld_of(y), Cout, st)
        else:
            _C.set_meta(kind="conv_fwd", shape=f"{Cin}->{Cout} k{KH} s{stride} in {B}x{H}x{W}", dtype=str(dtype), flops=2.0 * pixels * Cout * KH * KW * Cin,
                        bytes=float((B * H * W * Cin + pixels * Cout + Cout * KH * KW * Cin) * x.element_size()))
            call("dy_conv2d_fwd", C.byref(d), st)
            emu_round(z)
            call("dy_bn_finalize_valid", ptr(stats), pixels, ptr(bn.weight), ptr(bn.bias), ptr(bn.running_mean),
                 ptr(bn.running_var), float(bn.momentum), float(bn.eps), pa, pa + sa, pa + 2 * sa, pa + 3 * sa, cout_pad, Cout, st)
            _C.set_meta(kind="bn_act_fwd", shape=f"{cout_pad}ch {B}x{Ho}x{Wo}", dtype=str(dtype), flops=0.0,
                        bytes=float(pixels * cout_pad * x.element_size() * (3 if residual is not None else 2)))
            call("dy_bn_act_fwd", ptr(z), ld_of(z), pa, pa + sa, act, rp, rld, ptr(y), ld_of(y), pixels, cout_pad, dt_id(dtype), st)
            emu_round(y)
        if ctx is not None:
            ctx.z, ctx.aff, ctx.y = z, aff, None
    else:
        if has_bn:
            aff = bn_fold(bn, cout_pad)
            scale, shift = aff[0], aff[1]
        else:
            scale, shift = None, _padded_vec(bias, cout_pad)
        direct = residual is None
        y = out if (out is not None and direct) else empty_nhwc(B, cout_pad, Ho, Wo, dtype, dev)
        d = _conv_desc(x, wp, y, B, H, W, cin_pad, Ho, Wo, cout_pad, KH, KW, stride, pad, dil, scale, shift, act, None, False,
                       dtype)
        _C._prof is not None and _C.set_meta(kind="conv_fwd", shape=f"{Cin}->{Cout} k{KH} s{stride} in {B}x{H}x{W}", dtype=str(dtype), flops=2.0 * B * Ho * Wo * Cout * KH * KW * Cin,
                    bytes=float((B * H * W * Cin + B * Ho * Wo * Cout + Cout * KH * KW * Cin) * x.element_size()))
        call("dy_conv2d_fwd", C.byref(d), stream())
        if not direct:
            tgt = out if out is not None else y
            if tgt is not y:
                call("dy_copy2d", ptr(y), ld_of(y), ptr(tgt), ld_of(tgt), B * Ho * Wo, cout_pad, 0, dt_id(dtype), stream())
            call("dy_copy2d", ptr(residual), ld_of(residual), ptr(tgt), ld_of(tgt), B * Ho * Wo, cout_pad, 1, dt_id(dtype),
                 stream())
            y = tgt
        emu_round(y)
        if ctx is not None:
            if has_bn:
                raise RuntimeError("conv: gradients through an eval-mode BatchNorm are not supported")
            ctx.z, ctx.aff, ctx.y = None, None, y
    if tape is not None:
        tape.push(ctx)
    return y if cout_pad == Cout else y[:, :Cout]


def _add_pgrad(tape, p, g):
    if p is None or not p.requires_grad:
        return
    if p in tape.pgrads:
        tape.pgrads[p] = tape.pgrads[p] + g
    else:
        tape.pgrads[p] = g


_wg_scratch = {}


def wgrad_scratch(device, elems=32 << 20, tag=0):
    t = _wg_scratch.get((device, tag))
    if t is None or t.numel() < elems:
        t = torch.empty(elems, dtype=torch.float32, device=device)
        _wg_scratch[(device, tag)] = t
    return t


class _WgradSide:
    GROUP = 8

# ... 6 lines not shown
        self.free_events = []
        self.cb_queued = False


_wg_side = _WgradSide()


def enable_wgrad_stream(on=True):
    _wg_side.on = bool(on) and os.environ.get("DY_WGRAD_STREAM", "1") != "0"


def wgrad_stream_enabled():
    return bool(_wg_side.on)


def wgrad_side_stream(device=None):
    s = _wg_side
    if not s.on:
        return None
    if s.stream is None:
        prio = int(os.environ.get("DY_WGRAD_PRIO", "0"))
        s.stream = torch.cuda.Stream(device=device, priority=prio)
        s.raw = s.stream.cuda_stream
    return s.stream


def _side_wait_main(side=None):
    call("dy_stream_fork", stream(), _wg_side.raw)


def _wg_track(x, dz):
    s = _wg_side
    s.cur.append((x, dz))
    if len(s.cur) < s.GROUP or torch.cuda.is_current_stream_capturing():
        return
    ev = s.free_events.pop() if s.free_events else torch.cuda.Event()
    ev.record(s.stream)
    s.groups.append((ev, s.cur))
    s.cur = []
    while s.groups and s.groups[0][0].query():
        s.free_events.append(s.groups.pop(0)[0])


def wgrad_pending():
    return bool(_wg_side.cur or _wg_side.groups)


def wgrad_join():
    s = _wg_side
    if s.cur or s.groups:
        call("dy_stream_fork", s.raw, stream())
        s.free_events.extend(g[0] for g in s.groups)
        s.groups.clear()
        s.cur = []
    s.cb_queued = False


_branch = {"on": False, "streams": [], "by_device": {}}


def enable_branch_streams(on=True):
    _branch["on"] = bool(on) and os.environ.get("DY_BRANCH_STREAMS", "1") != "0"


def branch_streams(n, device):
    if not _branch["on"] or n <= 0:
        return None
    dev = torch.device(device)
    key = dev.index if dev.index is not None else torch.cuda.current_device()
    mine = _branch["by_device"].setdefault(key, [])
    while len(mine) < n:
        s = torch.cuda.Stream(device=device)
        mine.append(s)
        _branch["streams"].append(s)
    return mine[:n]


def _grad_dst(p):
    if p is not None and p.requires_grad and getattr(p, "_dy_direct", False) and p.grad is not None:
        return p.grad
    return None


def conv_backward(tape, dy, need_dx=True, dx_out=None, accumulate=False, add_src=None):
    ctx = tape.pop()
    x = ctx.x
    dtype = x.dtype
    dev = x.device
    B, Cin, H, W = x.shape
    KH, KW = ctx.k
    Cout, cout_pad, cin_pad = ctx.cout, ctx.cout_pad, ctx.cin_pad
    Ho, Wo = dy.shape[2], dy.shape[3]
    if cout_pad != Cout:
        if padded_channels(dy) != cout_pad:
            raise RuntimeError("conv_backward: gradient view lacks zero padding")
    pixels = B * Ho * Wo
    did = dt_id(dtype)
    st = stream()
    _grad_dst = (lambda p: None) if getattr(ctx, "shared", False) else globals()["_grad_dst"]
    if ctx.has_bn:
        aff, z, bn = ctx.aff, ctx.z, ctx.bn
        sums = arena.alloc(2 * cout_pad * _C.BN_BWD_REPLICAS, dev)
        pa, sa = aff.data_ptr(), 4 * cout_pad
        dz = empty_nhwc(B, cout_pad, Ho, Wo, dtype, dev)
        gw_, gb_ = _grad_dst(bn.weight), _grad_dst(bn.bias)
        direct = gw_ is not None and gb_ is not None
        if not direct:
            dgb = torch.empty((2, Cout), dtype=torch.float32, device=dev)
            gw_, gb_ = dgb[0], dgb[1]
        if _C._prof is None or _emulate_storage is not None:
            call("dy_bn_act_bwd_valid", dy.data_ptr(), ld_of(dy), z.data_ptr(), ld_of(z), pa, ptr(bn._parameters["weight"]), ctx.act,
                 sums.data_ptr(), dz.data_ptr(), ld_of(dz), gw_.data_ptr(), gb_.data_ptr(), pixels, cout_pad, Cout, did, st)
        else:
            _C.set_meta(kind="bn_act_bwd_reduce", shape=f"{cout_pad}ch {pixels}px", dtype=str(dtype), flops=0.0, bytes=float(pixels * cout_pad * x.element_size() * 2))
            call("dy_bn_act_bwd_reduce", ptr(dy), ld_of(dy), ptr(z), ld_of(z), pa, pa + sa, pa + 2 * sa, pa + 3 * sa,
                 ctx.act, 1, ptr(sums), pixels, cout_pad, did, st)
            _C.set_meta(kind="bn_act_bwd_apply", shape=f"{cout_pad}ch {pixels}px", dtype=str(dtype), flops=0.0, bytes=float(pixels * cout_pad * x.element_size() * 3))
            call("dy_bn_act_bwd_apply_valid", ptr(dy), ld_of(dy), ptr(z), ld_of(z), pa, pa + sa, pa + 2 * sa, pa + 3 * sa,
                 ptr(bn.weight), ctx.act, 1, ptr(sums), ptr(dz), ld_of(dz), ptr(gw_), ptr(gb_), pixels, cout_pad, Cout, did, st)
        emu_round(dz)
        if not direct:
            _add_pgrad(tape, bn.weight, gw_)
            _add_pgrad(tape, bn.bias, gb_)
    else:
        y = ctx.y
        need_bias = ctx.bias is not None and ctx.bias.requires_grad
        if ctx.act == ACT_NONE and not need_bias:
            dz = dy
        else:
            sums = arena.alloc(2 * cout_pad * _C.BN_BWD_REPLICAS, dev)
            call("dy_bn_act_bwd_reduce", ptr(dy), ld_of(dy), ptr(y), ld_of(y), None, None, None, None, ctx.act, 0, ptr(sums),
                 pixels, cout_pad, did, st)
            gb_ = _grad_dst(ctx.bias) if (need_bias and cout_pad == Cout) else None
            db = gb_ if gb_ is not None else torch.empty(cout_pad, dtype=torch.float32, device=dev)
            if ctx.act == ACT_NONE:
                dz = dy
                call("dy_bn_act_bwd_apply_valid", ptr(dy), ld_of(dy), ptr(y), ld_of(y), None, None, None, None, None, ctx.act, 0,
                     ptr(sums), ptr(dy), ld_of(dy), None, ptr(db), 0, cout_pad, Cout, did, st)
            else:
                dz = empty_nhwc(B, cout_pad, Ho, Wo, dtype, dev)
                call("dy_bn_act_bwd_apply_valid", ptr(dy), ld_of(dy), ptr(y), ld_of(y), None, None, None, None, None, ctx.act, 0,
                     ptr(sums), ptr(dz), ld_of(dz), None, ptr(db), pixels, cout_pad, Cout, did, st)
                emu_round(dz)
            if need_bias and gb_ is None:
                gd = _grad_dst(ctx.bias)
                if gd is not None:
                    gd.copy_(db[:Cout])
                else:
                    _add_pgrad(tape, ctx.bias, db[:Cout])
    if ctx.owner.requires_grad:
        gd = _grad_dst(ctx.owner)
        gw = gd if gd is not None else torch.empty(ctx.weight.shape, dtype=torch.float32, device=dev)
        side = wgrad_side_stream(dev) if gd is not None else None
        st_w = st
        if side is not None:
            if _C._prof is not None:
                _side_wait_main()
            if not _wg_side.cb_queued:
                try:
                    torch.autograd.Variable._execution_engine.queue_callback(wgrad_join)
                    _wg_side.cb_queued = True
                except RuntimeError:
                    pass
            st_w = side.cuda_stream
        scratch = wgrad_scratch(dev, tag=st_w)
        _C._prof is not None and _C.set_meta(kind="conv_wgrad", shape=f"{Cin}->{Cout} k{KH} s{ctx.stride} in {B}x{H}x{W}", dtype=str(dtype), flops=2.0 * pixels * Cout * KH * KW * Cin,
                    bytes=float((B * H * W * Cin + pixels * Cout) * x.element_size() + Cout * KH * KW * Cin * 4))
        wargs = (ptr(x), ld_of(x), B, H, W, cin_pad, ptr(dz), ld_of(dz), Ho, Wo, cout_pad, KH, KW, ctx.stride, ctx.pad, ctx.dil, Cout, Cin,
                 ptr(scratch), scratch.numel(), ptr(gw), did)
        if side is not None and _C._prof is not None:
            with torch.cuda.stream(side):
                call("dy_conv2d_wgrad", *wargs, st_w)
        elif side is not None:
            call("dy_conv2d_wgrad_forked", st, *wargs, st_w)
        else:
            call("dy_conv2d_wgrad", *wargs, st_w)
        if side is not None:
            _wg_track(x, dz)
        if gd is None:
            _add_pgrad(tape, ctx.owner, gw.view(ctx.owner.shape))
    if not need_dx:
        return None
    wt = _pack(ctx.weight, cout_pad, cin_pad, True, dtype)
    planar = (dx_out is None and add_src is None and dtype in (torch.bfloat16, torch.float16) and cin_pad == 8 and Cin <= 4 and (KH, KW) == (3, 3) and ctx.stride == 2
              and ctx.pad == 1 and ctx.dil == 1 and cout_pad in (16, 32, 64) and os.environ.get("DY_NO_CONV_SMALL") is None)
    if planar:
        dxp = torch.empty((B, Cin, H, W), dtype=dtype, device=dev)
        d = _conv_desc(dz, wt, None, B, Ho, Wo, cout_pad, H, W, cin_pad, KH, KW, ctx.stride, ctx.pad, ctx.dil, None, None, ACT_NONE,
                       None, False, dtype)
        d.dst_valid_channels = Cin
        d.dst_planar = dxp.data_ptr()
        _C._prof is not None and _C.set_meta(kind="conv_dgrad", shape=f"{Cin}->{Cout} k{KH} s{ctx.stride} in {B}x{H}x{W} (planar)", dtype=str(dtype),
                    flops=2.0 * pixels * Cout * KH * KW * Cin, bytes=float((B * H * W * Cin + pixels * Cout) * x.element_size()))
        call("dy_conv2d_dgrad", C.byref(d), st)
        return dxp
    if dx_out is None:
        dxb = empty_nhwc(B, cin_pad, H, W, dtype, dev)
        accumulate = False
    else:
        dxb = dx_out
        if padded_channels(dxb) != cin_pad:
            raise RuntimeError("conv_backward: dx_out view too narrow")
    d = _conv_desc(dz, wt, dxb, B, Ho, Wo, cout_pad, H, W, cin_pad, KH, KW, ctx.stride, ctx.pad, ctx.dil, None, None, ACT_NONE,
                   None, accumulate, dtype)
    d.dst_valid_channels = Cin
    if add_src is not None:
        if tuple(add_src.shape) != (B, Cin, H, W) or add_src.dtype != dtype or padded_channels(add_src) != cin_pad:
            raise RuntimeError("conv_backward: add_src must be an NHWC view of dx's shape and dtype")
        d.add_src, d.add_src_ld = add_src.data_ptr(), ld_of(add_src)
    _C._prof is not None and _C.set_meta(kind="conv_dgrad", shape=f"{Cin}->{Cout} k{KH} s{ctx.stride} in {B}x{H}x{W}", dtype=str(dtype), flops=2.0 * pixels * Cout * KH * KW * Cin,
                bytes=float((B * H * W * Cin * (2 if accumulate else 1) + pixels * Cout + Cout * KH * KW * Cin) * x.element_size()))
    call("dy_conv2d_dgrad", C.byref(d), st)
    emu_round(dxb)
    if dx_out is not None:
        return dx_out
    return dxb if cin_pad == Cin else dxb[:, :Cin]


def _nhwc_like(B, Cc, H, W, dtype, device):
    Cp = round_up(Cc, vec_elems(dtype))
    if Cp == Cc:
        return empty_nhwc(B, Cc, H, W, dtype, device)
    return zeros_nhwc(B, Cp, H, W, dtype, device)[:, :Cc]


def _pconv_packed(weight, w32, transposed, dtype):
    c3 = weight.shape[0]
    if dtype == torch.float32 or c3 < 16:
        return None
    cache = weight.__dict__.setdefault("_dy_pconv_pack", {})
    key, tag = (bool(transposed), dtype), (_weights_epoch, weight._version, weight.data_ptr())
    hit = cache.get(key)
    if hit is not None and hit[0] == tag:
        return hit[1]
    out = hit[1] if hit is not None else torch.empty(9 * ((c3 + 31) // 32) * ((c3 + 15) // 16) * 512, dtype=dtype, device=weight.device)
    call("dy_pconv_pack", ptr(w32), ptr(out), c3, 1 if transposed else 0, dt_id(dtype), stream())
    cache[key] = (tag, out)
    return out


def pconv_forward(tape, x, weight, out=None):
    B, Cc, H, W = x.shape
    c3 = weight.shape[0]
    if tuple(weight.shape) != (c3, c3, 3, 3) or c3 > Cc:
        raise RuntimeError(f"pconv: weight {tuple(weight.shape)} does not fit {Cc} channels")
    y = out if out is not None else _nhwc_like(B, Cc, H, W, x.dtype, x.device)
    w32 = weight.detach()
    if w32.dtype != torch.float32 or not w32.is_contiguous():
        w32 = w32.float().contiguous()
    es = x.element_size()
    _C._prof is not None and _C.set_meta(kind="pconv_fwd", shape=f"{c3}/{Cc} k3 in {B}x{H}x{W}", dtype=str(x.dtype),
                                         flops=2.0 * B * H * W * c3 * 9 * c3, bytes=float(2 * B * H * W * Cc * es + 9 * c3 * c3 * 4))
    wp = _pconv_packed(weight, w32, False, x.dtype)
    call("dy_pconv_fwd", ptr(x), ld_of(x), ptr(y), ld_of(y), ptr(w32), ptr(wp), B, H, W, Cc, c3, dt_id(x.dtype), stream())
    emu_round(y)
    if tape is not None:
        tape.push((x, weight))
    return y


def pconv_backward(tape, dy, dx_out=None, accumulate=False, add_src=None):
    x, weight = tape.pop()
    B, Cc, H, W = x.shape
    c3 = weight.shape[0]
    dtype, dev, st = x.dtype, x.device, stream()
    es = x.element_size()
    if tuple(dy.shape) != (B, Cc, H, W) or dy.dtype != dtype:
        raise RuntimeError("pconv_backward: gradient does not match the forward's output")
    if weight.requires_grad:
        gd = _grad_dst(weight)
        gw = gd if gd is not None else torch.empty(weight.shape, dtype=torch.float32, device=dev)
        scratch = wgrad_scratch(dev, tag=st)
        _C._prof is not None and _C.set_meta(kind="pconv_wgrad", shape=f"{c3}/{Cc} k3 in {B}x{H}x{W}", dtype=str(dtype),
                                             flops=2.0 * B * H * W * c3 * 9 * c3, bytes=float(2 * B * H * W * c3 * es + 9 * c3 * c3 * 4))
        call("dy_pconv_wgrad", ptr(x), ld_of(x), ptr(dy), ld_of(dy), ptr(gw), B, H, W, c3, ptr(scratch), scratch.numel(), dt_id(dtype), st)
        if gd is None:
            _add_pgrad(tape, weight, gw)
    if dx_out is None:
        dx, accumulate = _nhwc_like(B, Cc, H, W, dtype, dev), False
    else:
        dx = dx_out
    if add_src is not None and (tuple(add_src.shape) != (B, Cc, H, W) or add_src.dtype != dtype):
        raise RuntimeError("pconv_backward: add_src must be an NHWC view of dx's shape and dtype")
    w32 = weight.detach()
    if w32.dtype != torch.float32 or not w32.is_contiguous():
        w32 = w32.float().contiguous()
    n_rw = 2 + (1 if accumulate else 0) + (1 if add_src is not None else 0)
    _C._prof is not None and _C.set_meta(kind="pconv_dgrad", shape=f"{c3}/{Cc} k3 in {B}x{H}x{W}", dtype=str(dtype),
                                         flops=2.0 * B * H * W * c3 * 9 * c3, bytes=float(n_rw * B * H * W * Cc * es + 9 * c3 * c3 * 4))
    wp = _pconv_packed(weight, w32, True, dtype)
    call("dy_pconv_dgrad", ptr(dy), ld_of(dy), ptr(dx), ld_of(dx), ptr(w32), ptr(wp), B, H, W, Cc, c3, 1 if accumulate else 0,
         ptr(add_src), 0 if add_src is None else ld_of(add_src), dt_id(dtype), st)
    emu_round(dx)
    return dx

# ... 256 lines not shown
```

include/dedark_yolo.h:

```cpp
#ifndef DEDARK_YOLO_H
#define DEDARK_YOLO_H
#include <stddef.h>
#include <stdint.h>
#ifdef __cplusplus
extern "C" {
#endif

#define DY_F32 0
#define DY_BF16 1
#define DY_F16 2
#define DY_ACT_NONE 0
#define DY_ACT_SILU 1
#define DY_ACT_LEAKY 2
#define DY_STATS_REPLICAS 64
#define DY_BN_BWD_REPLICAS 8

const char* dy_last_error(void);
int dy_version(void);
const char* dy_last_kernel(void);
void dy_clear_last_kernel(void);

typedef struct {
  const void* src;
  int64_t src_ld;
  int N, Hs, Ws, Cs;
  const void* w;
  void* dst;
  int64_t dst_ld;
  int Hd, Wd, Cd;
  int KH, KW, stride, pad, dil;
  const float* scale;
  const float* shift;
  int act;
  double* stats;
  int accumulate;
  int dtype;
  int64_t dst_row_stride;
  int64_t dst_img_stride;
  int KHf, KWf;
  int kh0, kh_step;
  int kw0, kw_step;
  int dst_valid_channels;
  void* dst_planar;
  const void* add_src;
  int64_t add_src_ld;
} dy_conv_desc;

int dy_conv2d_fwd(const dy_conv_desc* d, void* stream);
int dy_conv2d_dgrad(const dy_conv_desc* d, void* stream);
int dy_conv2d_wgrad(const void* x, int64_t x_ld, int N, int Hi, int Wi, int Cin_pad, const void* dz, int64_t dz_ld, int Ho,
                    int Wo, int Cout_pad, int KH, int KW, int stride, int pad, int dil, int Cout, int Cin, float* scratch,
                    int64_t scratch_elems, float* g_oihw, int dtype, void* stream);
int dy_pack_weight(const float* w_oihw, void* packed, int Cout, int Cout_pad, int Cin, int Cin_pad, int KH, int KW,
                   int transposed, int dtype, void* stream);
typedef struct {
  const float* w;
  void* packed;
  int Cout, Cout_pad, Cin, Cin_pad, KH, KW, transposed, dtype;
  int64_t first_block;
} dy_pack_item;
int64_t dy_pack_item_blocks(int Cout_pad, int Cin_pad, int KH, int KW);
int dy_pack_weights_multi(const dy_pack_item* items_dev, int n_items, int64_t n_blocks, void* stream);
int dy_unpack_wgrad(const float* dw_packed, float* g_oihw, int Cout, int Cin, int Cin_pad, int KH, int KW, void* stream);

int dy_bn_finalize(const double* stats, int64_t count, const float* gamma, const float* beta, float* running_mean,
                   float* running_var, float momentum, float eps, float* scale, float* shift, float* mean, float* invstd,
                   int C, void* stream);
int dy_bn_fold_eval(const float* gamma, const float* beta, const float* running_mean, const float* running_var, float eps,
                    float* scale, float* shift, int C, void* stream);
int dy_bn_finalize_valid(const double* stats, int64_t count, const float* gamma, const float* beta, float* running_mean,
                         float* running_var, float momentum, float eps, float* scale, float* shift, float* mean, float* invstd,
                         int C, int C_valid, void* stream);
int dy_bn_fold_eval_valid(const float* gamma, const float* beta, const float* running_mean, const float* running_var, float eps,
                          float* scale, float* shift, int C, int C_valid, void* stream);
int dy_bn_act_fwd(const void* z, int64_t z_ld, const float* scale, const float* shift, int act, const void* residual,
                  int64_t res_ld, void* y, int64_t y_ld, int64_t pixels, int C, int dtype, void* stream);
int dy_bn_act_bwd_reduce(const void* dy, int64_t dy_ld, const void* z, int64_t z_ld, const float* scale,
                         const float* shift, const float* mean, const float* invstd, int act, int has_bn, double* sums,
                         int64_t pixels, int C, int dtype, void* stream);
int dy_bn_act_bwd_apply(const void* dy, int64_t dy_ld, const void* z, int64_t z_ld, const float* scale, const float* shift,
                        const float* mean, const float* invstd, const float* gamma, int act, int has_bn,
                        const double* sums, void* dz, int64_t dz_ld, float* dgamma, float* dbeta, int64_t pixels, int C,
                        int dtype, void* stream);
int dy_bn_act_bwd_apply_valid(const void* dy, int64_t dy_ld, const void* z, int64_t z_ld, const float* scale, const float* shift,
                              const float* mean, const float* invstd, const float* gamma, int act, int has_bn,
                              const double* sums, void* dz, int64_t dz_ld, float* dgamma, float* dbeta, int64_t pixels, int C,
                              int C_valid, int dtype, void* stream);

int dy_maxpool_fwd(const void* x, int64_t x_ld, void* y, int64_t y_ld, uint8_t* argmax, int N, int H, int W, int C, int k,
                   int stride, int pad, int Ho, int Wo, int dtype, void* stream);
int dy_maxpool_bwd(const void* dy, int64_t dy_ld, const uint8_t* argmax, void* dx, int64_t dx_ld, int N, int H, int W, int C,
                   int k, int stride, int pad, int Ho, int Wo, int accumulate, int dtype, void* stream);
int dy_upsample_nearest_fwd(const void* x, int64_t x_ld, void* y, int64_t y_ld, int N, int H, int W, int C, int scale,
                            int dtype, void* stream);
int dy_upsample_nearest_bwd(const void* dy, int64_t dy_ld, void* dx, int64_t dx_ld, int N, int H, int W, int C, int scale,
                            int accumulate, int dtype, void* stream);
int dy_copy2d(const void* src, int64_t src_ld, void* dst, int64_t dst_ld, int64_t pixels, int C, int accumulate, int dtype,
              void* stream);
int dy_cast(const void* src, int src_dtype, void* dst, int dst_dtype, int64_t n, void* stream);

int dy_pconv_pack(const float* w, void* wp, int c3, int transposed, int dtype, void* stream);
int dy_pconv_fwd(const void* x, int64_t x_ld, void* y, int64_t y_ld, const float* w, const void* wp, int N, int H, int W, int C, int c3,
                 int dtype, void* stream);
int dy_pconv_dgrad(const void* dy, int64_t dy_ld, void* dx, int64_t dx_ld, const float* w, const void* wp, int N, int H, int W, int C,
                   int c3, int accumulate, const void* add_src, int64_t add_ld, int dtype, void* stream);
int dy_pconv_wgrad(const void* x, int64_t x_ld, const void* dy, int64_t dy_ld, float* dw, int N, int H, int W, int c3, float* scratch,
                   int64_t scratch_elems, int dtype, void* stream);
int dy_asff_fuse_fwd(const void* x0, int64_t ld0, const void* x1, int64_t ld1, const void* x2, int64_t ld2,
                     const void* logits, int64_t ldl, void* out, int64_t ldo, int64_t pixels, int C, int dtype, void* stream);
int dy_asff_fuse_bwd(const void* dout, int64_t lddo, const void* x0, int64_t ld0, const void* x1, int64_t ld1,
                     const void* x2, int64_t ld2, const void* logits, int64_t ldl, void* dx0, int64_t ldd0, void* dx1,
                     int64_t ldd1, void* dx2, int64_t ldd2, void* dlogits, int64_t lddl, int64_t pixels, int C,
                     int acc0, int acc1, int acc2, int dtype, void* stream);

int dy_image_to_nhwc8(const float* x, int B, int H, int W, void* y, int Ho, int Wo, int dtype, void* stream);
int dy_resize_bwd(const float* dy_nhwc, int dy_ld, int B, int H, int W, int Ho, int Wo, float* dx, void* stream);
int dy_filter_params_fwd(const float* feat, int feat_ld, float* params, int B, void* stream);
int dy_filter_params_bwd(const float* feat, int feat_ld, const double* dparams, float* dfeat, int B, void* stream);
int dy_filters_pointwise_fwd(const float* x, const float* params, const float* A, const float* IcA, float* s4, int B,
                             int H, int W, int fast_math, void* stream);
int dy_usm_fwd(const float* s4, const float* params, float* out_nchw, void* out_nhwc8, float* hp, int B, int H, int W,
               int dtype, void* stream);
int dy_usm_bwd(const float* dout_nchw, const void* dout_nhwc, int dout_ld, const float* hp, const float* params, float* ds4,
               double* dparams, int B, int H, int W, int dtype, void* stream);
int dy_filters_pointwise_bwd(const float* x, const float* params, const float* A, const float* IcA, const float* ds4,
                             float* dx, double* dparams, int B, int H, int W, int accumulate, int fast_math, void* stream);

typedef struct {
  const void* map[3];
  int64_t map_ld[3];
  int h[3], w[3];
  float stride[3];
// ... 210 lines not shown
```

Baseline: 1017.

## Fuse next layer's BatchNorm backward reduction into conv dgrad epilogue

Adds a conv dgrad entry point that, when the producing layer has BatchNorm, computes the BN-backward per-channel sums (sum of dy*dact and sum of dy*dact*xhat) inside the v4/v5 conv epilogue while the gradient tile is still in registers. The results are accumulated into replicated double sums with atomics, and the later BN backward uses an apply-only kernel. This removes one full read pass over dx and z for the separate reduction kernel in bottleneck and C2f blocks. In exchange the epilogue carries more registers and LDS, adds atomics, and needs extra kernel instantiations.

```diff
diff --git a/dedark_yolo_amd/_C.py b/dedark_yolo_amd/_C.py
--- a/dedark_yolo_amd/_C.py
+++ b/dedark_yolo_amd/_C.py
@@ -22,6 +22,10 @@
                 ("add_src", vp), ("add_src_ld", i64)]
 
 
+class BnReduce(C.Structure):
+    _fields_ = [("z", vp), ("z_ld", i64), ("aff", vp), ("act", i32), ("sums", vp)]
+
+
 class PackItem(C.Structure):
     _fields_ = [("w", vp), ("packed", vp), ("Cout", i32), ("Cout_pad", i32), ("Cin", i32), ("Cin_pad", i32), ("KH", i32),
                 ("KW", i32), ("transposed", i32), ("dtype", i32), ("first_block", i64)]
@@ -70,6 +74,7 @@
     "dy_frontend_init": [],
     "dy_conv2d_fwd": [C.POINTER(ConvDesc), vp],
     "dy_conv2d_dgrad": [C.POINTER(ConvDesc), vp],
+    "dy_conv2d_dgrad_bnreduce": [C.POINTER(ConvDesc), C.POINTER(BnReduce), vp],
     "dy_conv2d_wgrad": [vp, i64, i32, i32, i32, i32, vp, i64, i32, i32, i32, i32, i32, i32, i32, i32, i32, i32, vp, i64, vp,
                         i32, vp],
     "dy_conv2d_wgrad_forked": [vp, vp, i64, i32, i32, i32, i32, vp, i64, i32, i32, i32, i32, i32, i32, i32, i32, i32, i32, vp, i64,
diff --git a/dedark_yolo_amd/csrc/bnact.hip b/dedark_yolo_amd/csrc/bnact.hip
--- a/dedark_yolo_amd/csrc/bnact.hip
+++ b/dedark_yolo_amd/csrc/bnact.hip
@@ -68,22 +68,6 @@
   shift[c] = beta[c] - rm[c] * sc;
 }
 
-__device__ inline float fast_sigmoid(float x) { return __builtin_amdgcn_rcpf(1.0f + __expf(-x)); }
-template <typename T, int ACT> __device__ inline float act_f(float u) {
-  if (sizeof(T) == 4) return dy_act(ACT, u);
-  if (ACT == DY_ACT_SILU) return u * fast_sigmoid(u);
-  if (ACT == DY_ACT_LEAKY) return u > 0.f ? u : 0.1f * u;
-  return u;
-}
-template <typename T, int ACT> __device__ inline float dact_f(float u) {
-  if (sizeof(T) == 4) return dy_dact(ACT, u);
-  if (ACT == DY_ACT_SILU) {
-    const float s = fast_sigmoid(u);
-    return s * (1.0f + u * (1.0f - s));
-  }
-  if (ACT == DY_ACT_LEAKY) return u > 0.f ? 1.0f : 0.1f;
-  return 1.0f;
-}
 template <typename F> __device__ inline void with_act(int act, F&& f) {
   if (act == DY_ACT_SILU) f(std::integral_constant<int, DY_ACT_SILU>{});
   else if (act == DY_ACT_LEAKY) f(std::integral_constant<int, DY_ACT_LEAKY>{});
diff --git a/dedark_yolo_amd/csrc/conv.hip b/dedark_yolo_amd/csrc/conv.hip
--- a/dedark_yolo_amd/csrc/conv.hip
+++ b/dedark_yolo_amd/csrc/conv.hip
@@ -836,6 +836,7 @@
   int (*launch)(const dy_conv_desc* d, int mode, void* stream);
   unsigned sites;
   bool fuses_add;
+  bool (*fuses_bnr)(const dy_conv_desc* d);
 };
 
 const Route kRoutes[] = {
@@ -844,8 +845,8 @@
     {dy_dense_dgrad_eligible, dy_dense_dgrad_launch, SITE_DGRAD_HEAD, false},
     {dy_conv_small_dgrad_eligible, dy_conv_small_dgrad_launch, SITE_DGRAD_HEAD, false},
     {dy_conv_px_eligible, dy_conv_px_launch, SITE_FWD | SITE_DGRAD, true},
-    {dy_conv_v4_eligible, dy_conv_v4_launch, SITE_FWD | SITE_DGRAD | SITE_CLASS, true},
-    {dy_conv_v5_eligible, dy_conv_v5_launch, SITE_FWD | SITE_DGRAD | SITE_CLASS, true},
+    {dy_conv_v4_eligible, dy_conv_v4_launch, SITE_FWD | SITE_DGRAD | SITE_CLASS, true, dy_conv_v4_fuses_bnr},
+    {dy_conv_v5_eligible, dy_conv_v5_launch, SITE_FWD | SITE_DGRAD | SITE_CLASS, true, dy_conv_v5_fuses_bnr},
     {dy_conv_v3_eligible, dy_conv_v3_launch, SITE_FWD | SITE_DGRAD, false},
     {dy_conv_v2_eligible, dy_conv_v2_launch, SITE_FWD | SITE_DGRAD | SITE_CLASS, false},
     {[](const dy_conv_desc* d, int mode) { return thin_eligible(d, mode); },
@@ -953,6 +954,33 @@
     return dy_copy2d(d->add_src, d->add_src_ld, d->dst, d->dst_ld, (int64_t)d->N * d->Hd * d->Wd, d->Cd, 1, d->dtype, stream);
   }
   return 0;
+}
+
+thread_local const dy_bn_reduce* dy_bnr_pending = nullptr;
+
+extern "C" int dy_conv2d_dgrad_bnreduce(const dy_conv_desc* d, const dy_bn_reduce* r, void* stream) {
+  if (int e = check_conv(d, "dy_conv2d_dgrad_bnreduce")) return e;
+  DY_CHECK(r && r->z && r->aff && r->sums, "dy_conv2d_dgrad_bnreduce: null pointer");
+  DY_CHECK(d->dst && d->dst_planar == nullptr && d->stats == nullptr, "dy_conv2d_dgrad_bnreduce: needs an NHWC destination and no statistics");
+  DY_CHECK(r->act >= 0 && r->act <= 2, "dy_conv2d_dgrad_bnreduce: bad act");
+  if (int e = dy_check_view("dy_conv2d_dgrad_bnreduce(z)", r->z, r->z_ld, d->Cd, d->dtype)) return e;
+  static const bool off = dy_env("DY_NO_BN_FUSE") != nullptr;
+  bool fuse = !off && d->dtype != DY_F32 && d->stride == 1 && d->KHf == 0 && d->dst_row_stride == 0 && pick_route(d, SITE_DGRAD_HEAD) == nullptr;
+  if (fuse) {
+    const Route* rt = pick_route(d, SITE_DGRAD);
+    fuse = rt->fuses_bnr && rt->fuses_bnr(d);
+  }
+  if (fuse) {
+    dy_bnr_pending = r;
+    const int e = dy_conv2d_dgrad(d, stream);
+    dy_bnr_pending = nullptr;
+    return e;
+  }
+  if (int e = dy_conv2d_dgrad(d, stream)) return e;
+  const float* a = r->aff;
+  const long C = d->Cd;
+  return dy_bn_act_bwd_reduce(d->dst, d->dst_ld, r->z, r->z_ld, a, a + C, a + 2 * C, a + 3 * C, r->act, 1, r->sums, (int64_t)d->N * d->Hd * d->Wd,
+                              d->Cd, d->dtype, stream);
 }
 
 namespace {
diff --git a/dedark_yolo_amd/csrc/conv_epilogue.h b/dedark_yolo_amd/csrc/conv_epilogue.h
--- a/dedark_yolo_amd/csrc/conv_epilogue.h
+++ b/dedark_yolo_amd/csrc/conv_epilogue.h
@@ -1,5 +1,7 @@
 #pragma once
+#include <type_traits>
 #include "dy_common.h"
+#include "../../include/dedark_yolo.h"
 
 namespace dy_epi {
 
@@ -69,17 +71,155 @@
 template <int BM, int BN>
 constexpr int row_image_bytes() { return BM * row_pitch<BN>(); }
 
-template <int BM, int BN, int NW, typename T16, typename OffFn, int RG = 64>
+struct BnReduce {
+  const char* z;
+  long z_ld;
+  const float* aff;
+  int act;
+  double* sums;
+};
+
+template <int BN>
+constexpr int bnr_halves() { return BN >= 128 ? BN / 128 : 1; }
+template <int BN, int NW>
+constexpr int bnr_lds_bytes() { return NW * BN * 2 * 4; }
+
+template <int BM, int BN, int NW, typename T16, typename OffFn, int RG = 64, bool BNR = false>
 __device__ inline void store_rows(const char* smem, int lane, int wave, long m0, int n0, long M, int Cd, int accumulate, T16* dst, OffFn off,
-                                  const T16* __restrict__ add = nullptr, long add_ld = 0) {
+                                  const T16* __restrict__ add = nullptr, long add_ld = 0, const BnReduce* bnr = nullptr, int tile_m = 0) {
   constexpr int PT = row_pitch<BN>();
   constexpr int LPP = BN >= 128 ? 16 : BN / 8;
   constexpr int PPI = 64 / LPP;
   constexpr int ITERS = BM / PPI / NW;
-  constexpr int HALVES = BN >= 128 ? BN / 128 : 1;
+  constexpr int HALVES = bnr_halves<BN>();
   const int pl = lane / LPP, chunk = lane % LPP;
   const bool nt = accumulate & 2;
   accumulate &= 1;
+  if constexpr (BNR) {
+    float sc[HALVES][8], sh[HALVES][8], mu[HALVES][8], is[HALVES][8], s1[HALVES][8], s2[HALVES][8];
+#pragma unroll
+    for (int h = 0; h < HALVES; ++h) {
+      const int n = n0 + 128 * h + 8 * chunk;
+      const bool nok = n < Cd;
+#pragma unroll
+      for (int e = 0; e < 8; ++e) {
+        sc[h][e] = nok ? bnr->aff[n + e] : 0.f;
+        sh[h][e] = nok ? bnr->aff[Cd + n + e] : 0.f;
+        mu[h][e] = nok ? bnr->aff[2 * Cd + n + e] : 0.f;
+        is[h][e] = nok ? bnr->aff[3 * Cd + n + e] : 0.f;
+        s1[h][e] = 0.f;
+        s2[h][e] = 0.f;
+      }
+    }
+    const T16* zp = reinterpret_cast<const T16*>(bnr->z);
+    constexpr bool PRE = HALVES == 1;
+    constexpr int UNR = PRE ? ITERS : 1;
+    u32x4 zraw[PRE ? ITERS : 1][HALVES];
+#pragma unroll
+    for (int u = 0; u < (PRE ? ITERS : 0); ++u) {
+      const int px = PPI * (wave + NW * u) + pl;
+      const long m = RG < 64 ? m0 + (px >> 6) * RG + (px & 63) : m0 + px;
+      const bool rok = !(RG < 64 && (px & 63) >= RG) && m < M;
+#pragma unroll
+      for (int h = 0; h < HALVES; ++h) {
+        const int n = n0 + 128 * h + 8 * chunk;
+        zraw[u][h] = (rok && n < Cd) ? *reinterpret_cast<const u32x4*>(zp + m * bnr->z_ld + n) : u32x4{0u, 0u, 0u, 0u};
+      }
+    }
+    auto rows = [&](auto actc) {
+      constexpr int ACT = decltype(actc)::value;
+#pragma unroll UNR
+      for (int u = 0; u < ITERS; ++u) {
+        const int px = PPI * (wave + NW * u) + pl;
+        if (RG < 64 && (px & 63) >= RG) continue;
+        const long m = RG < 64 ? m0 + (px >> 6) * RG + (px & 63) : m0 + px;
+        if (m >= M) continue;
+        const long o0 = off(m);
+        float zz[HALVES][8], xa[HALVES][8], xb[HALVES][8];
+        bool ok[HALVES];
+#pragma unroll
+        for (int h = 0; h < HALVES; ++h) {
+          const int n = n0 + 128 * h + 8 * chunk;
+          ok[h] = n < Cd;
+          if (ok[h]) {
+            if (accumulate) ldvec<T16>(dst + o0 + n, xa[h]);
+            if (add) ldvec<T16>(add + m * add_ld + n, xb[h]);
+          }
+          if constexpr (PRE) ldvec<T16>(reinterpret_cast<const T16*>(&zraw[u][h]), zz[h]);
+          else if (ok[h]) ldvec<T16>(zp + m * bnr->z_ld + n, zz[h]);
+        }
+#pragma unroll
+        for (int h = 0; h < HALVES; ++h) {
+          if (!ok[h]) continue;
+          const int c = 128 * h + 8 * chunk;
+          const uint2 lo = *reinterpret_cast<const uint2*>(smem + px * PT + c * 2);
+          const uint2 hi = *reinterpret_cast<const uint2*>(smem + px * PT + c * 2 + 8);
+          u32x4 v = {lo.x, lo.y, hi.x, hi.y};
+          T16* o = dst + o0 + n0 + c;
+          float g[8];
+          ldvec<T16>(reinterpret_cast<const T16*>(&v), g);
+          if (accumulate || add) {
+            if (accumulate) {
+#pragma unroll
+              for (int e = 0; e < 8; ++e) g[e] += xa[h][e];
+            }
+            if (add) {
+#pragma unroll
+              for (int e = 0; e < 8; ++e) g[e] += xb[h][e];
+            }
+            stvec<T16>(reinterpret_cast<T16*>(&v), g);
+            ldvec<T16>(reinterpret_cast<const T16*>(&v), g);
+          }
+          if (nt) asm volatile("global_store_dwordx4 %0, %1, off nt" ::"v"(o), "v"(v) : "memory");
+          else *reinterpret_cast<u32x4*>(o) = v;
+#pragma unroll
+          for (int e = 0; e < 8; ++e) {
+            const float ge = g[e] * dact_f<T16, ACT>(zz[h][e] * sc[h][e] + sh[h][e]);
+            s1[h][e] += ge;
+            s2[h][e] += ge * ((zz[h][e] - mu[h][e]) * is[h][e]);
+          }
+        }
+      }
+    };
+    if (bnr->act == DY_ACT_SILU) rows(std::integral_constant<int, DY_ACT_SILU>{});
+    else if (bnr->act == DY_ACT_LEAKY) rows(std::integral_constant<int, DY_ACT_LEAKY>{});
+    else rows(std::integral_constant<int, DY_ACT_NONE>{});
+#pragma unroll
+    for (int h = 0; h < HALVES; ++h)
+#pragma unroll
+      for (int e = 0; e < 8; ++e) {
+#pragma unroll
+        for (int o = 32; o >= LPP; o >>= 1) {
+          s1[h][e] += __shfl_xor(s1[h][e], o, 64);
+          s2[h][e] += __shfl_xor(s2[h][e], o, 64);
+        }
+      }
+    float* red = reinterpret_cast<float*>(const_cast<char*>(smem) + row_image_bytes<BM, BN>());
+    if (pl == 0) {
+#pragma unroll
+      for (int h = 0; h < HALVES; ++h)
+#pragma unroll
+        for (int e = 0; e < 8; ++e) {
+          const int c = 128 * h + 8 * chunk + e;
+          red[(wave * BN + c) * 2] = s1[h][e];
+          red[(wave * BN + c) * 2 + 1] = s2[h][e];
+        }
+    }
+    __syncthreads();
+    const int tid = wave * 64 + lane;
+    if (tid < BN && n0 + tid < Cd) {
+      float t1 = 0.f, t2 = 0.f;
+#pragma unroll
+      for (int w = 0; w < NW; ++w) {
+        t1 += red[(w * BN + tid) * 2];
+        t2 += red[(w * BN + tid) * 2 + 1];
+      }
+      double* st = bnr->sums + (long)(tile_m % DY_BN_BWD_REPLICAS) * 2 * Cd;
+      atomic_add_f64(st + n0 + tid, (double)t1);
+      atomic_add_f64(st + Cd + n0 + tid, (double)t2);
+    }
+    return;
+  }
 #pragma unroll 2
   for (int u = 0; u < ITERS; ++u) {
     const int px = PPI * (wave + NW * u) + pl;
diff --git a/dedark_yolo_amd/csrc/conv_route.h b/dedark_yolo_amd/csrc/conv_route.h
--- a/dedark_yolo_amd/csrc/conv_route.h
+++ b/dedark_yolo_amd/csrc/conv_route.h
@@ -1,6 +1,8 @@
 #pragma once
 #include "dy_common.h"
 #include "../../include/dedark_yolo.h"
+
+extern thread_local const dy_bn_reduce* dy_bnr_pending;
 
 namespace dy_route {
 
@@ -74,6 +76,11 @@
   if ((long)d->N * d->Hd * d->Wd * d->Cd * 2 > (128L << 20)) p.accumulate |= 2;
   p.M = (long)d->N * d->Hd * d->Wd;
   p.add_src = mode == 1 ? (const char*)d->add_src : nullptr; p.add_src_ld = d->add_src_ld;
+  p.bnr.z = nullptr; p.bnr.z_ld = 0; p.bnr.aff = nullptr; p.bnr.act = 0; p.bnr.sums = nullptr;
+  if (mode == 1 && dy_bnr_pending) {
+    const dy_bn_reduce* r = dy_bnr_pending;
+    p.bnr.z = (const char*)r->z; p.bnr.z_ld = r->z_ld; p.bnr.aff = r->aff; p.bnr.act = r->act; p.bnr.sums = r->sums;
+  }
   fill_dst_strides(p, d);
 }
 
@@ -137,10 +144,12 @@
 bool dy_conv_px_eligible(const dy_conv_desc* d, int mode);
 int dy_conv_px_launch(const dy_conv_desc* d, int mode, void* stream);
 bool dy_conv_v4_eligible(const dy_conv_desc* d, int mode);
+bool dy_conv_v4_fuses_bnr(const dy_conv_desc* d);
 int dy_conv_v4_launch(const dy_conv_desc* d, int mode, void* stream);
 bool dy_conv_v4_classes_eligible(const dy_conv_desc* classes, int ncls);
 int dy_conv_v4_launch_classes(const dy_conv_desc* classes, int ncls, void* stream);
 bool dy_conv_v5_eligible(const dy_conv_desc* d, int mode);
+bool dy_conv_v5_fuses_bnr(const dy_conv_desc* d);
 int dy_conv_v5_launch(const dy_conv_desc* d, int mode, void* stream);
 bool dy_conv_v5_classes_eligible(const dy_conv_desc* classes, int ncls);
 int dy_conv_v5_launch_classes(const dy_conv_desc* classes, int ncls, void* stream);
diff --git a/dedark_yolo_amd/csrc/conv_v4.hip b/dedark_yolo_amd/csrc/conv_v4.hip
--- a/dedark_yolo_amd/csrc/conv_v4.hip
+++ b/dedark_yolo_amd/csrc/conv_v4.hip
@@ -41,12 +41,13 @@
   long add_src_ld;
   int ncls;
   DyParityCls cls[4];
+  dy_epi::BnReduce bnr;
 };
 
 using dy_route::xcd_remap;
 using dy_route::dst_offset;
 
-template <int ABL, typename T, int RB>
+template <int ABL, typename T, int RB, bool BNR = false>
 __device__ __forceinline__ void conv_tile(const P& p, char* smem, const long m0, const int n0, const int tile_m) {
   constexpr int RG = 16 * RB;
   const int tid = threadIdx.x, lane = tid & 63;
@@ -324,6 +325,11 @@
     }
   __syncthreads();
   auto off_fn = [&](long m) { return dst_offset(p, m); };
+  if constexpr (BNR) {
+    dy_epi::store_rows<BM, BN, 8, T, decltype(off_fn), RG, true>(smem, lane, wave, m0, n0, p.M, p.Cd, p.accumulate, reinterpret_cast<T*>(p.dst),
+                                                                 off_fn, reinterpret_cast<const T*>(p.add_src), p.add_src_ld, &p.bnr, tile_m);
+    return;
+  }
   if (!(ABL & 64))
     dy_epi::store_rows<BM, BN, 8, T, decltype(off_fn), RG>(smem, lane, wave, m0, n0, p.M, p.Cd, p.accumulate, reinterpret_cast<T*>(p.dst), off_fn,
                                                            reinterpret_cast<const T*>(p.add_src), p.add_src_ld);
@@ -367,10 +373,10 @@
   }
 }
 
-template <int ABL, typename T = bf16_t>
+template <int ABL, typename T = bf16_t, bool BNR = false>
 __global__ __launch_bounds__(512) void conv_kernel(const P p) {
   extern __shared__ __attribute__((aligned(16))) char smem[];
-  if (p.ncls > 1) {
+  if (!BNR && p.ncls > 1) {
     const int x = blockIdx.x & 7, i = (int)blockIdx.x >> 3;
     int c = 0;
 #pragma unroll
@@ -394,12 +400,12 @@
   const int tile_m = bid / p.tiles_n, tile_n = bid - tile_m * p.tiles_n;
   const int n0 = tile_n * BN;
   if (!tail) {
-    conv_tile<ABL, T, 4>(p, smem, (long)tile_m * BM, n0, tile_m);
+    conv_tile<ABL, T, 4, BNR>(p, smem, (long)tile_m * BM, n0, tile_m);
   } else {
     const int full_m = p.n_full / p.tiles_n;
     const long m0 = (long)full_m * BM + (long)(tile_m - full_m) * 64 * p.rb_tail;
-    if (p.rb_tail == 3) conv_tile<ABL, T, 3>(p, smem, m0, n0, tile_m);
-    else conv_tile<ABL, T, 2>(p, smem, m0, n0, tile_m);
+    if (p.rb_tail == 3) conv_tile<ABL, T, 3, BNR>(p, smem, m0, n0, tile_m);
+    else conv_tile<ABL, T, 2, BNR>(p, smem, m0, n0, tile_m);
   }
 }
 
@@ -477,14 +483,25 @@
   constexpr int EPI256 = dy_epi::row_image_bytes<256, 256>();
   constexpr int SH256 = 2 * v4::BUF > EPI256 ? 2 * v4::BUF : EPI256;
   static_assert(SH256 <= 160 * 1024, "LDS budget");
+  constexpr int SHBNR = EPI256 + dy_epi::bnr_lds_bytes<256, 8>() > SH256 ? EPI256 + dy_epi::bnr_lds_bytes<256, 8>() : SH256;
+  static_assert(SHBNR <= 160 * 1024, "LDS budget");
   static bool configured = false;
   if (!configured) {
     hipError_t e = hipFuncSetAttribute(reinterpret_cast<const void*>(&v4::conv_kernel<ABL, T>), hipFuncAttributeMaxDynamicSharedMemorySize, SH256);
+    if (e == hipSuccess && ABL == 0)
+      e = hipFuncSetAttribute(reinterpret_cast<const void*>(&v4::conv_kernel<0, T, true>), hipFuncAttributeMaxDynamicSharedMemorySize, SHBNR);
     if (e != hipSuccess) {
       dy_set_error("conv_v4: hipFuncSetAttribute failed: %s", hipGetErrorString(e));
       return 3;
     }
     configured = true;
+  }
+  if (p.bnr.sums) {
+    DY_CHECK(ABL == 0 && mode == 1 && ncls <= 1 && d->Cd % 8 == 0, "conv_v4: the BatchNorm-reduce epilogue serves whole data gradients");
+    dy_note_kernel("v4::conv_kernel<bnr>");
+    v4::conv_kernel<0, T, true><<<p.nblk, 512, SHBNR, (hipStream_t)stream>>>(p);
+    DY_LAUNCH_CHECK();
+    return 0;
   }
   dy_note_kernel("v4::conv_kernel");
   v4::conv_kernel<ABL, T><<<p.nblk, 512, SH256, (hipStream_t)stream>>>(p);
@@ -493,6 +510,7 @@
 }
 
 #ifndef DY_V4_DIAG_BUILD
+bool dy_conv_v4_fuses_bnr(const dy_conv_desc* d) { return d->Cd % 8 == 0; }
 bool dy_conv_v4_eligible(const dy_conv_desc* d, int mode) {
   static const bool off = dy_env("DY_NO_CONV_V4") != nullptr;
   return !off && v4_variant(d, mode) != 0;
diff --git a/dedark_yolo_amd/csrc/conv_v5.hip b/dedark_yolo_amd/csrc/conv_v5.hip
--- a/dedark_yolo_amd/csrc/conv_v5.hip
+++ b/dedark_yolo_amd/csrc/conv_v5.hip
@@ -50,12 +50,13 @@
   int ablate;
   int ncls;
   DyParityCls cls[4];
+  dy_epi::BnReduce bnr;
 };
 
 using dy_route::xcd_remap;
 using dy_route::dst_offset;
 
-template <int BN, typename T, int MB>
+template <int BN, typename T, int MB, bool BNR = false>
 __device__ __forceinline__ void epilogue(const P& p, f32x4 (&acc)[MB][4], char* smem, int tid, int lane, int wave, int wm, int wn, long m0,
                                          int n0, int tile_m) {
   constexpr int WN = BN / 64, WM = 4 / WN;
@@ -99,8 +100,14 @@
   }
   __syncthreads();
   stamp(DY_ABLATE_OF(p), p.nblk, 3);
-  dy_epi::store_rows<BM, BN, 4>(smem, lane, wave, m0, n0, p.M, p.Cd, p.accumulate, reinterpret_cast<T*>(p.dst),
-                                [&](long m) { return dst_offset(p, m); }, reinterpret_cast<const T*>(p.add_src), p.add_src_ld);
+  auto off_fn = [&](long m) { return dst_offset(p, m); };
+  if constexpr (BNR) {
+    dy_epi::store_rows<BM, BN, 4, T, decltype(off_fn), 64, true>(smem, lane, wave, m0, n0, p.M, p.Cd, p.accumulate, reinterpret_cast<T*>(p.dst),
+                                                                 off_fn, reinterpret_cast<const T*>(p.add_src), p.add_src_ld, &p.bnr, tile_m);
+    return;
+  }
+  dy_epi::store_rows<BM, BN, 4>(smem, lane, wave, m0, n0, p.M, p.Cd, p.accumulate, reinterpret_cast<T*>(p.dst), off_fn,
+                                reinterpret_cast<const T*>(p.add_src), p.add_src_ld);
   stamp(DY_ABLATE_OF(p), p.nblk, 4);
   if (p.stats) {
     __syncthreads();
@@ -357,7 +364,7 @@
 
 constexpr int BAND_BYTES = 17 * 1024;
 
-template <int BN, typename T = bf16_t, int NBAND_ = (BN == 64 ? 3 : 2)>
+template <int BN, typename T = bf16_t, int NBAND_ = (BN == 64 ? 3 : 2), bool BNR = false>
 __global__ __launch_bounds__(256, (BN == 64 && NBAND_ == 2) ? 3 : 2) void band_kernel(const P p) {
   constexpr int WN = BN / 64, WM = 4 / WN, MB = BM / WM / 16, B_LD = BN / 64, B_BYTES = BN * 64;
   constexpr int NBAND = NBAND_, DB = 3 * (NBAND - 1), NBBUF = DB + 1;
@@ -541,7 +548,7 @@
   asm volatile("s_waitcnt vmcnt(0)" ::: "memory");
   __builtin_amdgcn_s_barrier();
   stamp(DY_ABLATE_OF(p), p.nblk, 2);
-  epilogue<BN, T, MB>(p, acc, smem, tid, lane, wave, wm, wn, m0, n0, tile_m);
+  epilogue<BN, T, MB, BNR>(p, acc, smem, tid, lane, wave, wm, wn, m0, n0, tile_m);
 #ifdef DY_DIAG
   asm volatile("s_waitcnt vmcnt(0)" ::: "memory");
 #endif
@@ -570,6 +577,17 @@
 }
 
 static int v5_launch(const dy_conv_desc* d, int mode, void* stream, const dy_conv_desc* classes, int ncls);
+
+static bool v5_band(const dy_conv_desc* d) {
+  static const bool no_band = dy_env("DY_NO_CONV_BAND") != nullptr;
+  return !no_band && d->KH == 3 && d->KW == 3 && d->stride == 1 && d->pad == 1 && d->dil == 1 && d->KHf <= 0 && d->Hs == d->Hd && d->Ws == d->Wd &&
+         d->Ws >= 16;
+}
+static int v5_band64_nband() {
+  static const int n = dy_env("DY_BAND64_NBAND") ? atoi(dy_env("DY_BAND64_NBAND")) : 2;
+  return n;
+}
+bool dy_conv_v5_fuses_bnr(const dy_conv_desc* d) { return v5_band(d) && d->Cd % 8 == 0 && (d->Cd > 64 || v5_band64_nband() == 2); }
 
 int dy_conv_v5_launch(const dy_conv_desc* d, int mode, void* stream) { return v5_launch(d, mode, stream, nullptr, 0); }
 
@@ -616,11 +634,12 @@
   constexpr int SB128 = BAND128 > EPI128 ? BAND128 : EPI128, SB64 = BAND64 > EPI64 ? BAND64 : EPI64;
   constexpr int BAND64S = 2 * v5::BAND_BYTES + 4 * 64 * 64 + 64, SB64S = BAND64S > EPI64 ? BAND64S : EPI64;
   static_assert(3 * SB64S <= 160 * 1024, "three blocks per CU");
-  static const int band64_nband = dy_env("DY_BAND64_NBAND") ? atoi(dy_env("DY_BAND64_NBAND")) : 2;
+  const int band64_nband = v5_band64_nband();
   static_assert(2 * SH128 <= 160 * 1024 && 2 * SH64 <= 160 * 1024 && 2 * SB128 <= 160 * 1024 && 2 * SB64 <= 160 * 1024, "two blocks per CU");
-  static const bool no_band = dy_env("DY_NO_CONV_BAND") != nullptr;
-  const bool band = ncls <= 1 && !no_band && d->KH == 3 && d->KW == 3 && d->stride == 1 && d->pad == 1 && d->dil == 1 && d->KHf <= 0 && d->Hs == d->Hd &&
-                    d->Ws == d->Wd && d->Ws >= 16;
+  const bool band = ncls <= 1 && v5_band(d);
+  constexpr int SBR128 = EPI128 + dy_epi::bnr_lds_bytes<128, 4>() > SB128 ? EPI128 + dy_epi::bnr_lds_bytes<128, 4>() : SB128;
+  constexpr int SBR64S = EPI64 + dy_epi::bnr_lds_bytes<64, 4>() > SB64S ? EPI64 + dy_epi::bnr_lds_bytes<64, 4>() : SB64S;
+  static_assert(2 * SBR128 <= 160 * 1024 && 3 * SBR64S <= 160 * 1024, "blocks per CU of the BNR band kernels");
   static bool configured = false;
   if (!configured) {
     hipError_t e = hipFuncSetAttribute(reinterpret_cast<const void*>(&v5::conv_kernel<128, bf16_t>), hipFuncAttributeMaxDynamicSharedMemorySize, SH128);
@@ -635,6 +654,10 @@
     if (e == hipSuccess) e = hipFuncSetAttribute(reinterpret_cast<const void*>(&v5::band_kernel<64, f16_t>), hipFuncAttributeMaxDynamicSharedMemorySize, SB64);
     if (e == hipSuccess) e = hipFuncSetAttribute(reinterpret_cast<const void*>(&v5::band_kernel<64, bf16_t, 2>), hipFuncAttributeMaxDynamicSharedMemorySize, SB64S);
     if (e == hipSuccess) e = hipFuncSetAttribute(reinterpret_cast<const void*>(&v5::band_kernel<64, f16_t, 2>), hipFuncAttributeMaxDynamicSharedMemorySize, SB64S);
+    if (e == hipSuccess) e = hipFuncSetAttribute(reinterpret_cast<const void*>(&v5::band_kernel<128, bf16_t, 2, true>), hipFuncAttributeMaxDynamicSharedMemorySize, SBR128);
+    if (e == hipSuccess) e = hipFuncSetAttribute(reinterpret_cast<const void*>(&v5::band_kernel<128, f16_t, 2, true>), hipFuncAttributeMaxDynamicSharedMemorySize, SBR128);
+    if (e == hipSuccess) e = hipFuncSetAttribute(reinterpret_cast<const void*>(&v5::band_kernel<64, bf16_t, 2, true>), hipFuncAttributeMaxDynamicSharedMemorySize, SBR64S);
+    if (e == hipSuccess) e = hipFuncSetAttribute(reinterpret_cast<const void*>(&v5::band_kernel<64, f16_t, 2, true>), hipFuncAttributeMaxDynamicSharedMemorySize, SBR64S);
     if (e != hipSuccess) {
       dy_set_error("conv_v5: hipFuncSetAttribute failed: %s", hipGetErrorString(e));
       return 3;
@@ -642,6 +665,20 @@
     configured = true;
   }
   const bool f16 = d->dtype == DY_F16;
+  if (p.bnr.sums) {
+    DY_CHECK(mode == 1 && dy_conv_v5_fuses_bnr(d), "conv_v5: the BatchNorm-reduce epilogue serves the band kernels' data gradients");
+    if (bn == 128) {
+      dy_note_kernel("v5::band_kernel<128,bnr>");
+      if (f16) v5::band_kernel<128, f16_t, 2, true><<<p.nblk, 256, SBR128, (hipStream_t)stream>>>(p);
+      else v5::band_kernel<128, bf16_t, 2, true><<<p.nblk, 256, SBR128, (hipStream_t)stream>>>(p);
+    } else {
+      dy_note_kernel("v5::band_kernel<64,bnr>");
+      if (f16) v5::band_kernel<64, f16_t, 2, true><<<p.nblk, 256, SBR64S, (hipStream_t)stream>>>(p);
+      else v5::band_kernel<64, bf16_t, 2, true><<<p.nblk, 256, SBR64S, (hipStream_t)stream>>>(p);
+    }
+    DY_LAUNCH_CHECK();
+    return 0;
+  }
   if (band && bn == 128) {
     dy_note_kernel("v5::band_kernel<128>");
     if (f16) v5::band_kernel<128, f16_t><<<p.nblk, 256, SB128, (hipStream_t)stream>>>(p);
diff --git a/dedark_yolo_amd/csrc/dy_common.h b/dedark_yolo_amd/csrc/dy_common.h
--- a/dedark_yolo_amd/csrc/dy_common.h
+++ b/dedark_yolo_amd/csrc/dy_common.h
@@ -203,6 +203,23 @@
     return s * (1.0f + u * (1.0f - s));
   }
   if (act == DY_ACT_LEAKY) return u > 0.f ? 1.0f : 0.1f;
+  return 1.0f;
+}
+
+__device__ inline float fast_sigmoid(float x) { return __builtin_amdgcn_rcpf(1.0f + __expf(-x)); }
+template <typename T, int ACT> __device__ inline float act_f(float u) {
+  if (sizeof(T) == 4) return dy_act(ACT, u);
+  if (ACT == DY_ACT_SILU) return u * fast_sigmoid(u);
+  if (ACT == DY_ACT_LEAKY) return u > 0.f ? u : 0.1f * u;
+  return u;
+}
+template <typename T, int ACT> __device__ inline float dact_f(float u) {
+  if (sizeof(T) == 4) return dy_dact(ACT, u);
+  if (ACT == DY_ACT_SILU) {
+    const float s = fast_sigmoid(u);
+    return s * (1.0f + u * (1.0f - s));
+  }
+  if (ACT == DY_ACT_LEAKY) return u > 0.f ? 1.0f : 0.1f;
   return 1.0f;
 }
 
diff --git a/dedark_yolo_amd/nn/modules.py b/dedark_yolo_amd/nn/modules.py
--- a/dedark_yolo_amd/nn/modules.py
+++ b/dedark_yolo_amd/nn/modules.py
@@ -128,11 +128,11 @@
 
     _takes_into = True
 
-    def _bwd(self, tape, dy, needs=(True,), dx_out=None, accumulate=False, add_src=None, into=None):
+    def _bwd(self, tape, dy, needs=(True,), dx_out=None, accumulate=False, add_src=None, into=None, bn_next=None):
         if into is not None and into[0] is not None:
             conv_backward(tape, dy, need_dx=True, dx_out=into[0], accumulate=True)
             return None
-        return conv_backward(tape, dy, need_dx=needs[0], dx_out=dx_out, accumulate=accumulate, add_src=add_src)
+        return conv_backward(tape, dy, need_dx=needs[0], dx_out=dx_out, accumulate=accumulate, add_src=add_src, bn_next=bn_next)
 
 
 class AddConv(nn.Module):
@@ -234,9 +234,9 @@
         t = self.cv1._fwd(tape, x)
         return self.cv2._fwd(tape, t, out=out, residual=x if self.add else None)
 
-    def _bwd(self, tape, dy, needs=(True,), dx_out=None, accumulate=False):
-        dt = self.cv2._bwd(tape, dy)
-        return self.cv1._bwd(tape, dt, dx_out=dx_out, accumulate=accumulate, add_src=dy if self.add else None)
+    def _bwd(self, tape, dy, needs=(True,), dx_out=None, accumulate=False, bn_next=None):
+        dt = self.cv2._bwd(tape, dy, bn_next=tape.stack[-2])
+        return self.cv1._bwd(tape, dt, dx_out=dx_out, accumulate=accumulate, add_src=dy if self.add else None, bn_next=bn_next)
 
 
 class C2(DyModule):
@@ -294,7 +294,8 @@
         c, n = self.c, len(self.m)
         dY = self.cv2._bwd(tape, dy)
         for i in reversed(range(n)):
-            self.m[i]._bwd(tape, dY[:, (2 + i) * c:(3 + i) * c], dx_out=dY[:, (1 + i) * c:(2 + i) * c], accumulate=True)
+            self.m[i]._bwd(tape, dY[:, (2 + i) * c:(3 + i) * c], dx_out=dY[:, (1 + i) * c:(2 + i) * c], accumulate=True,
+                           bn_next=tape.stack[-3] if i >= 1 else None)
         return self.cv1._bwd(tape, dY[:, :2 * c], needs=needs)
 
 
diff --git a/dedark_yolo_amd/ops.py b/dedark_yolo_amd/ops.py
--- a/dedark_yolo_amd/ops.py
+++ b/dedark_yolo_amd/ops.py
@@ -309,7 +309,7 @@
 
 class ConvCtx:
     __slots__ = ("x", "z", "aff", "weight", "bias", "bn", "act", "k", "stride", "pad", "dil", "cout", "cout_pad", "cin_pad",
-                 "has_bn", "y", "owner", "shared")
+                 "has_bn", "y", "owner", "shared", "sums")
 
 
 def _conv_desc(src, w, dst, N, Hs, Ws, Cs, Hd, Wd, Cd, KH, KW, stride, pad, dil, scale, shift, act, stats, accumulate, dtype):
@@ -355,6 +355,7 @@
         ctx.shared = shared
         ctx.k, ctx.stride, ctx.pad, ctx.dil = (KH, KW), stride, pad, dil
         ctx.cout, ctx.cout_pad, ctx.cin_pad, ctx.has_bn = Cout, cout_pad, cin_pad, has_bn
+        ctx.sums = None
     if batch_stats:
         z = empty_nhwc(B, cout_pad, Ho, Wo, dtype, dev)
         stats = arena.alloc(2 * cout_pad * _C.STATS_REPLICAS, dev)
@@ -527,7 +528,20 @@
     return None
 
 
-def conv_backward(tape, dy, need_dx=True, dx_out=None, accumulate=False, add_src=None):
+_bn_fusion = {"on": os.environ.get("DY_BN_FUSION", "1") != "0"}
+
+
+def enable_bn_fusion(on=True):
+    _bn_fusion["on"] = bool(on)
+
+
+def _bn_next_fusable(nxt, dtype, B, H, W, cin_pad):
+    return (_bn_fusion["on"] and isinstance(nxt, ConvCtx) and nxt.has_bn and nxt.z is not None and nxt.sums is None
+            and dtype in (torch.bfloat16, torch.float16) and _C._prof is None and _emulate_storage is None
+            and nxt.cout_pad == cin_pad and nxt.z.dtype == dtype and tuple(nxt.z.shape) == (B, cin_pad, H, W))
+
+
+def conv_backward(tape, dy, need_dx=True, dx_out=None, accumulate=False, add_src=None, bn_next=None):
     ctx = tape.pop()
     x = ctx.x
     dtype = x.dtype
@@ -553,7 +567,11 @@
         if not direct:
             dgb = torch.empty((2, Cout), dtype=torch.float32, device=dev)
             gw_, gb_ = dgb[0], dgb[1]
-        if _C._prof is None or _emulate_storage is not None:
+        if ctx.sums is not None:
+            sums, ctx.sums = ctx.sums, None
+            call("dy_bn_act_bwd_apply_valid", ptr(dy), ld_of(dy), ptr(z), ld_of(z), pa, pa + sa, pa + 2 * sa, pa + 3 * sa,
+                 ptr(bn.weight), ctx.act, 1, ptr(sums), ptr(dz), ld_of(dz), ptr(gw_), ptr(gb_), pixels, cout_pad, Cout, did, st)
+        elif _C._prof is None or _emulate_storage is not None:
             call("dy_bn_act_bwd_valid", dy.data_ptr(), ld_of(dy), z.data_ptr(), ld_of(z), pa, ptr(bn._parameters["weight"]), ctx.act,
                  sums.data_ptr(), dz.data_ptr(), ld_of(dz), gw_.data_ptr(), gb_.data_ptr(), pixels, cout_pad, Cout, did, st)
         else:
@@ -655,7 +673,13 @@
         d.add_src, d.add_src_ld = add_src.data_ptr(), ld_of(add_src)
     _C._prof is not None and _C.set_meta(kind="conv_dgrad", shape=f"{Cin}->{Cout} k{KH} s{ctx.stride} in {B}x{H}x{W}", dtype=str(dtype), flops=2.0 * pixels * Cout * KH * KW * Cin,
                 bytes=float((B * H * W * Cin * (2 if accumulate else 1) + pixels * Cout + Cout * KH * KW * Cin) * x.element_size()))
-    call("dy_conv2d_dgrad", C.byref(d), st)
+    if bn_next is not None and _bn_next_fusable(bn_next, dtype, B, H, W, cin_pad):
+        nz = bn_next.z
+        bn_next.sums = arena.alloc(2 * cin_pad * _C.BN_BWD_REPLICAS, dev)
+        r = _C.BnReduce(nz.data_ptr(), ld_of(nz), bn_next.aff.data_ptr(), bn_next.act, bn_next.sums.data_ptr())
+        call("dy_conv2d_dgrad_bnreduce", C.byref(d), C.byref(r), st)
+    else:
+        call("dy_conv2d_dgrad", C.byref(d), st)
     emu_round(dxb)
     if dx_out is not None:
         return dx_out
diff --git a/include/dedark_yolo.h b/include/dedark_yolo.h
--- a/include/dedark_yolo.h
+++ b/include/dedark_yolo.h
@@ -48,6 +48,14 @@
 
 int dy_conv2d_fwd(const dy_conv_desc* d, void* stream);
 int dy_conv2d_dgrad(const dy_conv_desc* d, void* stream);
+typedef struct {
+  const void* z;
+  int64_t z_ld;
+  const float* aff;
+  int act;
+  double* sums;
+} dy_bn_reduce;
+int dy_conv2d_dgrad_bnreduce(const dy_conv_desc* d, const dy_bn_reduce* r, void* stream);
 int dy_conv2d_wgrad(const void* x, int64_t x_ld, int N, int Hi, int Wi, int Cin_pad, const void* dz, int64_t dz_ld, int Ho,
                     int Wo, int Cout_pad, int KH, int KW, int stride, int pad, int dil, int Cout, int Cin, float* scratch,
                     int64_t scratch_elems, float* g_oihw, int dtype, void* stream);
```

New measurement: 999.7. -1.7%, worse.
